# chayanchatterjee/GW-Whisper

Measured on AMD Instinct MI355X. Metric: 1s-strain segments/sec (encoder fwd), higher is better.
Workload: dtype bf16; 1 GPU; whisper-tiny encoder fwd, batch 256 log-mel (80x3000) per GPU, 1500 tokens, random-init weights (BASELINE configs[1]); global_batch=256, parallelism=dp1, encoder=tiny, streams_per_gpu=1

## Files before the change

### gw_whisper_amd/_lib.py

```python

from __future__ import annotations

import ctypes as C
import os

_HERE = os.path.dirname(os.path.abspath(__file__))
LIB_PATH = os.environ.get("GWW_LIB") or os.path.join(_HERE, "libgww.so")

PREC_BF16 = 0
PREC_F32 = 1

EPI_BIAS, EPI_GELU, EPI_RESID = 0, 1, 2
EPI_DGELU = 5


class EncCfg(C.Structure):
    _fields_ = [("d_model", C.c_int), ("n_layers", C.c_int), ("n_heads", C.c_int),
                ("ffn", C.c_int), ("n_mels", C.c_int), ("t_in", C.c_int)]


class EncGlobals(C.Structure):
    _fields_ = [(n, C.c_void_p) for n in
                ("conv1_w", "conv1_b", "conv2_w", "conv2_b", "pos", "ln_w", "ln_b")]

# ... 2 lines not shown
    _fields_ = [(n, C.c_void_p) for n in
                ("ln1_w", "ln1_b", "q_w", "q_b", "k_w", "v_w", "v_b", "o_w", "o_b",
                 "ln2_w", "ln2_b", "fc1_w", "fc1_b", "fc2_w", "fc2_b")]


class DoraTarget(C.Structure):
    _fields_ = [("layer", C.c_int), ("proj", C.c_int), ("r", C.c_int), ("scaling", C.c_float),
                ("A", C.c_void_p), ("B", C.c_void_p), ("mag", C.c_void_p), ("nrm", C.c_void_p),
                ("dA", C.c_void_p), ("dB", C.c_void_p), ("dm", C.c_void_p)]


class EncLayerGrads(C.Structure):
    _fields_ = [(f[0], C.c_void_p) for f in EncLayer._fields_]


class EncGrads(C.Structure):
    _fields_ = [(n, C.c_void_p) for n in
                ("conv1_w", "conv1_b", "conv2_w", "conv2_b", "pos", "ln_w", "ln_b")] + \
               [("layers", C.POINTER(EncLayerGrads))]


class DoraMergeItem(C.Structure):
    _fields_ = [("w0", C.c_void_p), ("a", C.c_void_p), ("b", C.c_void_p), ("m", C.c_void_p), ("w_eff", C.c_void_p),
                ("norm_out", C.c_void_p), ("scaling", C.c_float), ("d_out", C.c_int), ("d_in", C.c_int), ("r", C.c_int)]


SIGNATURES = {
    "gww_version": (C.c_int, []),
    "gww_last_error": (C.c_char_p, []),
    "gww_frontend_create": (C.c_int, [C.POINTER(C.c_void_p)]),
    "gww_frontend_create_nmel": (C.c_int, [C.c_int, C.POINTER(C.c_void_p)]),
    "gww_frontend_destroy": (None, [C.c_void_p]),
    "gww_logmel_f32": (C.c_int, [C.c_void_p, C.c_void_p, C.c_int, C.c_int, C.c_long, C.c_void_p,
                                 C.c_void_p, C.c_void_p]),
    "gww_logmel_host_f32": (C.c_int, [C.c_void_p, C.c_int, C.c_int, C.c_long, C.c_void_p]),
    "gww_logmel_host_nmel_f32": (C.c_int, [C.c_void_p, C.c_int, C.c_int, C.c_long, C.c_int, C.c_void_p]),
    "gww_encoder_create": (C.c_int, [C.POINTER(EncCfg), C.POINTER(C.c_void_p)]),
    "gww_encoder_destroy": (None, [C.c_void_p]),
    "gww_encoder_set_weights": (C.c_int, [C.c_void_p, C.POINTER(EncGlobals), C.POINTER(EncLayer),
                                          C.c_int, C.c_void_p]),
    "gww_encoder_update_weights": (C.c_int, [C.c_void_p, C.POINTER(EncGlobals), C.POINTER(EncLayer), C.c_int,
                                             C.POINTER(C.c_uint), C.c_void_p]),
    "gww_encoder_workspace_bytes": (C.c_size_t, [C.c_void_p, C.c_int, C.c_int]),
    "gww_encoder_forward": (C.c_int, [C.c_void_p, C.c_void_p, C.c_int, C.c_int, C.c_void_p, C.c_size_t,
                                      C.c_void_p, C.c_void_p, C.c_void_p]),
    "gww_encoder_forward_outputs": (C.c_int, [C.c_void_p, C.c_void_p, C.c_int, C.c_int, C.c_void_p, C.c_size_t,
                                              C.c_void_p, C.c_void_p, C.c_void_p, C.c_void_p]),
    "gww_encoder_set_split": (C.c_int, [C.c_void_p, C.c_int]),
    "gww_encoder_set_stem_shortcut": (C.c_int, [C.c_void_p, C.c_int]),
    "gww_encoder_stem_shortcut_flags": (C.c_int, [C.c_void_p, C.c_int, C.c_int, C.c_void_p, C.POINTER(C.c_int)]),
    "gww_encoder_set_x_native": (C.c_int, [C.c_void_p, C.c_int]),
    "gww_x_native_offset": (C.c_size_t, [C.c_long, C.c_int, C.c_long]),
    "gww_x_native_bytes": (C.c_size_t, [C.c_long]),
    "gww_encoder_trace_enable": (C.c_int, [C.c_void_p, C.c_int]),
    "gww_encoder_trace_read": (C.c_int, [C.c_void_p, C.POINTER(C.c_float), C.POINTER(C.c_int)]),
    "gww_encoder_trace_classes": (C.c_int, []),
    "gww_encoder_trace_class_name": (C.c_char_p, [C.c_int]),
    "gww_train_saved_bytes": (C.c_size_t, [C.c_void_p, C.c_int]),
    "gww_train_workspace_bytes": (C.c_size_t, [C.c_void_p, C.c_int]),
    "gww_encoder_train_forward": (C.c_int, [C.c_void_p, C.c_void_p, C.c_int, C.c_void_p, C.c_size_t, C.c_void_p,
                                            C.c_size_t, C.c_void_p, C.c_int, C.c_void_p]),
    "gww_encoder_train_backward": (C.c_int, [C.c_void_p, C.c_int, C.c_void_p, C.c_size_t, C.c_void_p, C.c_size_t,
                                             C.c_void_p, C.POINTER(DoraTarget), C.c_int, C.c_void_p, C.c_void_p,
                                             C.c_int, C.c_void_p]),
    "gww_train_workspace_bytes_full": (C.c_size_t, [C.c_void_p, C.c_int]),
    "gww_train_workspace_bytes_adapters": (C.c_size_t, [C.c_void_p, C.c_int, C.c_int]),
    "gww_encoder_train_backward_full": (C.c_int, [C.c_void_p, C.c_int, C.c_void_p, C.c_size_t, C.c_void_p, C.c_size_t,
                                                  C.c_void_p, C.POINTER(DoraTarget), C.c_int, C.c_void_p, C.c_void_p,
                                                  C.c_int, C.POINTER(EncGrads), C.c_void_p]),
    "gww_train_saved_bytes_f32": (C.c_size_t, [C.c_void_p, C.c_int]),
    "gww_train_workspace_bytes_f32": (C.c_size_t, [C.c_void_p, C.c_int]),
    "gww_encoder_train_forward_f32": (C.c_int, [C.c_void_p, C.c_void_p, C.c_int, C.c_void_p, C.c_size_t, C.c_void_p,
                                                C.c_size_t, C.c_void_p, C.c_int, C.c_void_p]),
    "gww_encoder_train_backward_f32": (C.c_int, [C.c_void_p, C.c_int, C.c_void_p, C.c_size_t, C.c_void_p, C.c_size_t,
                                                 C.c_void_p, C.POINTER(DoraTarget), C.c_int, C.c_void_p, C.c_void_p,
                                                 C.c_int, C.c_void_p]),
    "gww_attention_lse_f32": (C.c_int, [C.c_void_p, C.c_void_p, C.c_void_p, C.c_int, C.c_int, C.c_int, C.c_void_p]),
    "gww_attention_bwd_f32_scratch_bytes": (C.c_size_t, [C.c_int, C.c_int, C.c_int]),
    "gww_attention_bwd_f32": (C.c_int, [C.c_void_p, C.c_void_p, C.c_void_p, C.c_void_p, C.c_void_p, C.c_void_p,
                                        C.c_int, C.c_int, C.c_int, C.c_void_p]),
    "gww_adapter_grads_f32_scratch_bytes": (C.c_size_t, [C.c_long, C.c_int, C.c_int, C.c_int]),
    "gww_adapter_grads_f32": (C.c_int, [C.c_void_p, C.c_long, C.c_void_p, C.c_void_p, C.c_long, C.c_void_p, C.c_float,
                                        C.c_float, C.c_void_p, C.c_void_p, C.c_void_p, C.c_void_p, C.c_void_p,
                                        C.c_void_p, C.c_void_p, C.c_long, C.c_int, C.c_int, C.c_int, C.c_void_p,
                                        C.c_size_t, C.c_void_p]),
    "gww_gemm_wgrad_workspace_bytes": (C.c_size_t, [C.c_long, C.c_int, C.c_int]),
    "gww_gemm_wgrad_bf16": (C.c_int, [C.c_void_p, C.c_long, C.c_void_p, C.c_long, C.c_long, C.c_int, C.c_int, C.c_float,
                                      C.c_void_p, C.c_void_p, C.c_void_p, C.c_size_t, C.c_void_p]),
    "gww_layernorm_param_grads_workspace_bytes": (C.c_size_t, [C.c_long, C.c_int]),
    "gww_layernorm_param_grads": (C.c_int, [C.c_void_p, C.c_void_p, C.c_int, C.c_long, C.c_int, C.c_void_p, C.c_void_p,
                                            C.c_void_p, C.c_size_t, C.c_void_p]),
    "gww_attention_bwd_bf16": (C.c_int, [C.c_void_p, C.c_void_p, C.c_void_p, C.c_void_p, C.c_void_p, C.c_void_p,
                                         C.c_int, C.c_int, C.c_int, C.c_void_p]),
    "gww_attention_bwd_log2q_bf16": (C.c_int, [C.c_void_p, C.c_void_p, C.c_void_p, C.c_void_p, C.c_void_p, C.c_void_p,
                                         C.c_int, C.c_int, C.c_int, C.c_void_p]),
    "gww_attention_log2q_bf16": (C.c_int, [C.c_void_p, C.c_void_p, C.c_void_p, C.c_int, C.c_int, C.c_int, C.c_void_p]),
    "gww_attention_lse_bf16": (C.c_int, [C.c_void_p, C.c_void_p, C.c_void_p, C.c_int, C.c_int, C.c_int, C.c_void_p]),
    "gww_layernorm_bwd": (C.c_int, [C.c_void_p, C.c_void_p, C.c_void_p, C.c_int, C.c_void_p, C.c_int, C.c_void_p,
                                    C.c_long, C.c_int, C.c_void_p]),
    "gww_gelu_bf16": (C.c_int, [C.c_void_p, C.c_void_p, C.c_void_p, C.c_long, C.c_void_p]),
    "gww_dora_grads": (C.c_int, [C.c_void_p, C.c_long, C.c_void_p, C.c_void_p, C.c_long, C.c_void_p, C.c_float,
                                 C.c_float, C.c_void_p, C.c_void_p, C.c_void_p, C.c_void_p, C.c_void_p, C.c_void_p,
                                 C.c_void_p, C.c_long, C.c_int, C.c_int, C.c_void_p]),
    "gww_adapter_grads_scratch_bytes": (C.c_size_t, [C.c_long, C.c_int, C.c_int, C.c_int]),
    "gww_adapter_grads": (C.c_int, [C.c_void_p, C.c_long, C.c_void_p, C.c_void_p, C.c_long, C.c_void_p, C.c_float,
                                    C.c_float, C.c_void_p, C.c_void_p, C.c_void_p, C.c_void_p, C.c_void_p, C.c_void_p,
# ... 179 lines not shown
```

### gw_whisper_amd/csrc/attention.hip

```cpp
#include "common.h"

#include <stdlib.h>
#include <type_traits>

#ifndef GWW_ATT_EPI16
#define GWW_ATT_EPI16 1
#endif
namespace gww {

#ifdef GWW_STAMP
__device__ unsigned long long g_stamp_att[8];
#define ASTAMP_DECL unsigned long long _t0 = __builtin_amdgcn_s_memtime(); unsigned long long _acc[7] = {0, 0, 0, 0, 0, 0, 0};
#define ASTAMP(i)                                                  \
  do {                                                             \
    __builtin_amdgcn_sched_barrier(0);                             \
    const unsigned long long _t1 = __builtin_amdgcn_s_memtime();   \
    _acc[i] += _t1 - _t0;                                          \
    _t0 = _t1;                                                     \
    __builtin_amdgcn_sched_barrier(0);                             \
  } while (0)
#define ASTAMP_FLUSH                                                                 \
  if (lane == 0) {                                                                   \
    for (int _q = 0; _q < 7; ++_q) atomicAdd(&g_stamp_att[_q], _acc[_q]);            \
    atomicAdd(&g_stamp_att[7], 1ull);                                                \
// ... 388 lines not shown
    __syncthreads();
  };
  using P0 = std::integral_constant<int, 0>;
  using P1 = std::integral_constant<int, 1>;
  using Yes = std::true_type;
  using No = std::false_type;

  gload(0);
  lstore(P0{});
  __syncthreads();
  const bool ragged = (T % KB) != 0;
  if (n_kt == 1) {
    if (ragged) tile(0, P0{}, Yes{}, Yes{});
    else tile(0, P0{}, Yes{}, No{});
  } else {
    tile(0, P0{}, Yes{}, No{});
    int kt = 1;
    for (; kt + 2 <= n_kt - 1; kt += 2) {
      tile(kt, P1{}, No{}, No{});
      tile(kt + 1, P0{}, No{}, No{});
    }
    if (kt == n_kt - 2) {
      tile(kt, P1{}, No{}, No{});
      if (ragged) tile(kt + 1, P0{}, No{}, Yes{});
      else tile(kt + 1, P0{}, No{}, No{});
    } else {
      if (ragged) tile(kt, P1{}, No{}, Yes{});
      else tile(kt, P1{}, No{}, No{});
    }
  }

  const float l_tot = (VAR & 2) ? l_run + __shfl_xor(l_run, 32, 64) : lt[0];
  const float inv = 1.0f / l_tot;
  if (lse && q_row < T && hh == 0)
    lse[((long)b * H + h) * T + q_row] = (m_run + __log2f(l_tot)) * 0.69314718055994530942f;
  if (q_row < T) {
    unsigned short* orow = ctx + ((long)b * T + q_row) * d + h * DH;
#pragma unroll
    for (int n = 0; n < 2; ++n)
#pragma unroll
      for (int c = 0; c < 4; ++c) {
        const int dh = 32 * n + 8 * c + 4 * hh;
        u32x2 o = {pack2bf(ot[n][4 * c] * inv, ot[n][4 * c + 1] * inv),
                   pack2bf(ot[n][4 * c + 2] * inv, ot[n][4 * c + 3] * inv)};
        *reinterpret_cast<u32x2*>(orow + dh) = o;
      }
  }
}

#endif
#ifndef GWW_ATT_NBUF
#define GWW_ATT_NBUF 2
#endif
template <int MINW, bool MSUM, bool NOMAX>
__global__ __launch_bounds__(256, MINW) void k_attention_dma_bf16(const unsigned short* __restrict__ qkv,
                                                                 unsigned short* __restrict__ ctx,
                                                                 float* __restrict__ lse, int T, int H, int q_tiles,
                                                                 int qt0) {
  constexpr int NB = GWW_ATT_NBUF;
  __shared__ __attribute__((aligned(16))) unsigned char lds[NB * 2 * KB * DH * 2];
  constexpr int TILE_BYTES = KB * DH * 2, NW = 4;
  typedef __attribute__((address_space(3))) void* lds_ptr;
  typedef const __attribute__((address_space(1))) void* g_ptr;
  const int tid = threadIdx.x, lane = tid & 63, wave = tid >> 6;
  const int wave_u = __builtin_amdgcn_readfirstlane(wave);
  const unsigned nblk = gridDim.x, per = nblk >> 3;
  const unsigned wid = blockIdx.x < 8 * per ? (blockIdx.x & 7) * per + (blockIdx.x >> 3) : blockIdx.x;
  const int qt = qt0 + wid % q_tiles;
  const int bh = wid / q_tiles;
  const int b = bh / H, h = bh - b * H;
  const int d = H * DH;
  const long row_stride = 3L * d;
  const unsigned short* base = qkv + (long)b * T * row_stride;
  const unsigned short* qp = base + h * DH;
  const unsigned short* kp = base + d + h * DH;
  const unsigned short* vp = base + 2 * d + h * DH;
  const int r = lane & 31, hh = lane >> 5;
  const int q_row = qt * (NW * 32) + wave * 32 + r;
  const int q_ld = q_row < T ? q_row : T - 1;
  const bool wave_live = qt * (NW * 32) + wave_u * 32 < T;
  bf16x8 qf[4];
#pragma unroll
  for (int s = 0; s < 4; ++s) qf[s] = *reinterpret_cast<const bf16x8*>(qp + (long)q_ld * row_stride + 16 * s + 8 * hh);

  const int n_kt = (T + KB - 1) / KB;
  const bool ragged = (T % KB) != 0;
  unsigned koff[2], voff[2];
#pragma unroll
  for (int j = 0; j < 2; ++j) {
    const int row = 8 * (2 * wave + j) + (lane >> 3), pos = lane & 7;
    koff[j] = (unsigned)(row * (int)row_stride * 2 + ((pos ^ ((row >> 1) & 7)) << 4));
    voff[j] = (unsigned)(row * (int)row_stride * 2 + ((pos ^ (((row >> 1) & 1) << 2)) << 4));
  }
  auto dma = [&](int kt, auto buf_c) {
    constexpr int BUF = decltype(buf_c)::value;
    const char* kb = reinterpret_cast<const char*>(kp + (long)kt * KB * row_stride);
    const char* vb = reinterpret_cast<const char*>(vp + (long)kt * KB * row_stride);
    unsigned char* dk = lds + BUF * TILE_BYTES + (2 * wave_u) * 1024;
    unsigned char* dv = dk + NB * TILE_BYTES;
    if constexpr (NB == 3) {
      const unsigned mk = (unsigned)(unsigned long long)(lds_ptr)dk, mv = (unsigned)(unsigned long long)(lds_ptr)dv;
      unsigned ko[2], vo[2];
      if (kt != n_kt - 1 || !ragged) {
        ko[0] = koff[0]; ko[1] = koff[1]; vo[0] = voff[0]; vo[1] = voff[1];
      } else {
        const int last_row = T - 1 - kt * KB;
#pragma unroll
// ... 176 lines not shown
    using P2 = std::integral_constant<int, 2>;
    dma(0, P0{});
    if (n_kt > 1) {
      dma(1, P1{});
      asm volatile("s_waitcnt vmcnt(4)\n\ts_barrier" ::: "memory");
    } else {
      asm volatile("s_waitcnt vmcnt(0)\n\ts_barrier" ::: "memory");
    }
#pragma unroll
    for (int s4 = 0; s4 < 4; ++s4) asm volatile("" : "+v"(qf[s4]));
    tile(0, P0{}, Yes{}, No{}, n_kt == 1 && ragged);
    for (int kt = 1; kt < n_kt; kt += 3) {
      tile(kt, P1{}, No{}, No{}, ragged && kt == n_kt - 1);
      if (kt + 1 < n_kt) tile(kt + 1, P2{}, No{}, No{}, ragged && kt + 1 == n_kt - 1);
      if (kt + 2 < n_kt) tile(kt + 2, P0{}, No{}, No{}, ragged && kt + 2 == n_kt - 1);
    }
  } else {
    dma(0, P0{});
    __syncthreads();
    if (n_kt == 1) {
      if (ragged) tile(0, P0{}, Yes{}, Yes{});
      else tile(0, P0{}, Yes{}, No{});
    } else {
      tile(0, P0{}, Yes{}, No{});
      int kt = 1;
      for (; kt + 2 <= n_kt - 1; kt += 2) {
        tile(kt, P1{}, No{}, No{});
        tile(kt + 1, P0{}, No{}, No{});
      }
      if (kt == n_kt - 2) {
        tile(kt, P1{}, No{}, No{});
        if (ragged) tile(kt + 1, P0{}, No{}, Yes{});
        else tile(kt + 1, P0{}, No{}, No{});
      } else {
        if (ragged) tile(kt, P1{}, No{}, Yes{});
        else tile(kt, P1{}, No{}, No{});
      }
    }
  }

  float l_tot;
  if constexpr (MSUM) {
    l_tot = lt[0];
  } else {
    const auto sw = __builtin_amdgcn_permlane32_swap(__float_as_uint(l_run), __float_as_uint(l_run), false, false);
    l_tot = __uint_as_float(sw[0]) + __uint_as_float(sw[1]);
  }
  const float inv = 1.0f / l_tot;
  if (lse && q_row < T && hh == 0)
    lse[((long)b * H + h) * T + q_row] = (m_run + __log2f(l_tot)) * 0.69314718055994530942f;
#if GWW_ATT_EPI16
  {
    unsigned short* orow = ctx + ((long)b * T + q_row) * d + h * DH;
#pragma unroll
    for (int n = 0; n < 2; ++n)
#pragma unroll
      for (int cp = 0; cp < 2; ++cp) {
        const int c0 = 2 * cp, c1 = 2 * cp + 1;
        const unsigned a0 = pack2bf(ot[n][4 * c0] * inv, ot[n][4 * c0 + 1] * inv), a1 = pack2bf(ot[n][4 * c0 + 2] * inv, ot[n][4 * c0 + 3] * inv);
        const unsigned b0 = pack2bf(ot[n][4 * c1] * inv, ot[n][4 * c1 + 1] * inv), b1 = pack2bf(ot[n][4 * c1 + 2] * inv, ot[n][4 * c1 + 3] * inv);
        const auto s0 = __builtin_amdgcn_permlane32_swap(a0, b0, false, false);
        const auto s1 = __builtin_amdgcn_permlane32_swap(a1, b1, false, false);
        u32x4 o = {s0[0], s1[0], s0[1], s1[1]};
        if (q_row < T) *reinterpret_cast<u32x4*>(orow + 32 * n + 8 * (hh ? c1 : c0)) = o;
      }
  }
#else
  if (q_row < T) {
    unsigned short* orow = ctx + ((long)b * T + q_row) * d + h * DH;
#pragma unroll
    for (int n = 0; n < 2; ++n)
#pragma unroll
      for (int c = 0; c < 4; ++c) {
        const int dh = 32 * n + 8 * c + 4 * hh;
        u32x2 o = {pack2bf(ot[n][4 * c] * inv, ot[n][4 * c + 1] * inv),
                   pack2bf(ot[n][4 * c + 2] * inv, ot[n][4 * c + 3] * inv)};
        *reinterpret_cast<u32x2*>(orow + dh) = o;
      }
  }
#endif
}

#ifdef GWW_LAB
constexpr int PP_SLOTS = 4;
#ifndef GWW_PP_PRIO
#define GWW_PP_PRIO 0
#endif
template <int MODE>
__global__ __launch_bounds__(MODE == 1 ? 256 : 512, 1) void k_attention_pp_bf16(const unsigned short* __restrict__ qkv,
                                                              unsigned short* __restrict__ ctx,
                                                              float* __restrict__ lse, int T, int H, int q_tiles,
                                                              int qt0) {
  constexpr int TILE_BYTES = KB * DH * 2;
  __shared__ __attribute__((aligned(16))) unsigned char lds[2 * PP_SLOTS * TILE_BYTES];
  typedef __attribute__((address_space(3))) void* lds_ptr;
  typedef const __attribute__((address_space(1))) void* g_ptr;
  const int tid = threadIdx.x, lane = tid & 63;
  const int wave = __builtin_amdgcn_readfirstlane(tid >> 6);
  const bool g1 = wave >= 4;
  constexpr int NWV = MODE == 1 ? 4 : 8, PPW = 8 / NWV;
  const unsigned nblk = gridDim.x, per = nblk >> 3;
  const unsigned wid = blockIdx.x < 8 * per ? (blockIdx.x & 7) * per + (blockIdx.x >> 3) : blockIdx.x;
  const int qt = qt0 + wid % q_tiles;
  const int bh = wid / q_tiles;
  const int b = bh / H, h = bh - b * H;
  const int d = H * DH;
  const long row_stride = 3L * d;
  const unsigned short* base = qkv + (long)b * T * row_stride;
  const unsigned short* qp = base + h * DH;
  const unsigned short* kp = base + d + h * DH;
  const unsigned short* vp = base + 2 * d + h * DH;
  const int r = lane & 31, hh = lane >> 5;
  const int q_row = qt * (NWV * 32) + wave * 32 + r;
  const int q_ld = q_row < T ? q_row : T - 1;
  bf16x8 qf[4];
#pragma unroll
  for (int s = 0; s < 4; ++s) qf[s] = *reinterpret_cast<const bf16x8*>(qp + (long)q_ld * row_stride + 16 * s + 8 * hh);

  const int n_kt = (T + KB - 1) / KB;
  const bool ragged = (T % KB) != 0;
// ... 481 lines not shown
  if (g1) __builtin_amdgcn_s_barrier();
  if (GWW_PP_PRIO == 2 && g1) __builtin_amdgcn_s_setprio(1);
  if (n_kt == 1 && ragged) tile(0, std::integral_constant<int, 0>{}, Yes{}, Yes{});
  else tile(0, std::integral_constant<int, 0>{}, Yes{}, No{});
  {
    int kt = 1;
    for (; kt + 4 <= n_kt - 1; kt += 4) {
      tile(kt, std::integral_constant<int, 1>{}, No{}, No{});
      tile(kt + 1, std::integral_constant<int, 2>{}, No{}, No{});
      tile(kt + 2, std::integral_constant<int, 3>{}, No{}, No{});
      tile(kt + 3, std::integral_constant<int, 0>{}, No{}, No{});
    }
    for (; kt < n_kt; ++kt) tile_rt(kt, ragged && kt == n_kt - 1);
  }
  pv_reads((n_kt - 1) & 3);
  pv_mfma();
  if (!g1) __builtin_amdgcn_s_barrier();
  ASTAMP(6);
  ASTAMP_FLUSH
  }

  float l_tot;
  {
    const auto sw = __builtin_amdgcn_permlane32_swap(__float_as_uint(l_run), __float_as_uint(l_run), false, false);
    l_tot = __uint_as_float(sw[0]) + __uint_as_float(sw[1]);
  }
  const float inv = 1.0f / l_tot;
  if (lse && q_row < T && hh == 0)
    lse[((long)b * H + h) * T + q_row] = (m_run + __log2f(l_tot)) * 0.69314718055994530942f;
  {
    unsigned short* orow = ctx + ((long)b * T + q_row) * d + h * DH;
#pragma unroll
    for (int n = 0; n < 2; ++n)
#pragma unroll
      for (int cp = 0; cp < 2; ++cp) {
        const int c0 = 2 * cp, c1 = 2 * cp + 1;
        const unsigned a0 = pack2bf(ot[n][4 * c0] * inv, ot[n][4 * c0 + 1] * inv), a1 = pack2bf(ot[n][4 * c0 + 2] * inv, ot[n][4 * c0 + 3] * inv);
        const unsigned b0 = pack2bf(ot[n][4 * c1] * inv, ot[n][4 * c1 + 1] * inv), b1 = pack2bf(ot[n][4 * c1 + 2] * inv, ot[n][4 * c1 + 3] * inv);
        const auto s0 = __builtin_amdgcn_permlane32_swap(a0, b0, false, false);
        const auto s1 = __builtin_amdgcn_permlane32_swap(a1, b1, false, false);
        u32x4 o = {s0[0], s1[0], s0[1], s1[1]};
        if (q_row < T) *reinterpret_cast<u32x4*>(orow + 32 * n + 8 * (hh ? c1 : c0)) = o;
      }
  }
}

#endif
bool attention_log2q_enabled() {
  static const bool off = lab_int("GWW_ATT_LOG2Q", 1) == 0;
  return !off;
}

int launch_attention_bf16(const void* qkv, void* ctx, int B, int T, int H, hipStream_t s, float* lse,
                          bool last_tile_only, bool q_log2) {
  GWW_REQUIRE(qkv && ctx, "attention_bf16: NULL operand");
  GWW_REQUIRE(B >= 0 && T > 0 && H > 0, "attention_bf16: bad shape B=%d T=%d H=%d", B, T, H);
  GWW_REQUIRE((((uintptr_t)qkv) & 15) == 0 && (((uintptr_t)ctx) & 15) == 0, "attention_bf16: 16-byte alignment");
  if (B == 0) return GWW_OK;
#ifdef GWW_LAB
  if (q_log2 && !last_tile_only && lab_int("GWW_ATT_W64", 0) != 0) return launch_attention_w64_bf16(qkv, ctx, B, T, H, s, lse);
#endif
  const unsigned short* in = (const unsigned short*)qkv;
  unsigned short* out = (unsigned short*)ctx;
#ifdef GWW_LAB
  const int nw_env = (int)lab_int("GWW_ATT_WAVES", 0);
  const int var_env = (int)lab_int("GWW_ATT_VAR", 7);
  const bool pp = q_log2 && var_env >= 8;
  const int nw = ((nw_env == 8 && !q_log2) || (pp && var_env == 8)) ? 8 : 4;
#else
  const int nw = 4;
#endif
  const int all_tiles = (T + nw * 32 - 1) / (nw * 32);
  const int q_tiles = last_tile_only ? 1 : all_tiles, qt0 = last_tile_only ? all_tiles - 1 : 0;
  const long blocks = (long)q_tiles * B * H;
  GWW_REQUIRE(blocks < 2147483647L, "attention_bf16: grid too large");
#define GWW_DMA(MW, MS, NM) hipLaunchKernelGGL((k_attention_dma_bf16<MW, MS, NM>), dim3((unsigned)blocks), dim3(256), 0, s, in, out, lse, T, H, q_tiles, qt0)
#ifdef GWW_LAB
  if (pp && var_env >= 9) {
    hipLaunchKernelGGL((k_attention_pp_bf16<1>), dim3((unsigned)blocks), dim3(256), 0, s, in, out, lse, T, H, q_tiles, qt0);
  } else if (pp) {
    hipLaunchKernelGGL((k_attention_pp_bf16<0>), dim3((unsigned)blocks), dim3(512), 0, s, in, out, lse, T, H, q_tiles, qt0);
  } else if (q_log2) {
    const int var = var_env & 7;
#define GWW_L2(VV) hipLaunchKernelGGL((k_attention_l2_bf16<4, VV>), dim3((unsigned)blocks), dim3(256), 0, s, in, out, lse, T, H, q_tiles, qt0)
    switch (var) {
      case 0: GWW_L2(0); break;
      case 1: GWW_L2(1); break;
      case 2: GWW_L2(2); break;
      case 3: GWW_L2(3); break;
      case 4: GWW_DMA(3, false, false); break;
      case 5: GWW_DMA(4, false, false); break;
      case 6: GWW_DMA(3, true, false); break;
      default: GWW_DMA(3, false, true); break;
    }
#undef GWW_L2
  } else if (nw == 8) {
    hipLaunchKernelGGL(k_attention_bf16<8>, dim3((unsigned)blocks), dim3(512), 0, s, in, out, lse, T, H, q_tiles, qt0);
  } else
#else
  if (q_log2) {
    GWW_DMA(3, false, true);
  } else
#endif
  {
    hipLaunchKernelGGL(k_attention_bf16<4>, dim3((unsigned)blocks), dim3(256), 0, s, in, out, lse, T, H, q_tiles, qt0);
  }
#undef GWW_DMA
  GWW_LAUNCH_CHECK();
  return GWW_OK;
}

constexpr int FKB = 32;
constexpr int FLDS = DH + 1;

__global__ __launch_bounds__(256) void k_attention_f32(const float* __restrict__ qkv, float* __restrict__ ctx,
                                                       int T, int H, int q_tiles) {
  __shared__ float Ks[FKB][FLDS];
  __shared__ float Vs[FKB][FLDS];
  const int tid = threadIdx.x, lane = tid & 63, wave = tid >> 6;
  const int qt = blockIdx.x % q_tiles;
  const int bh = blockIdx.x / q_tiles;
  const int b = bh / H, h = bh - b * H;
  const int d = H * DH;
  const long row_stride = 3L * d;
  const float* base = qkv + (long)b * T * row_stride;
  const float* qp = base + h * DH;
  const float* kp = base + d + h * DH;
  const float* vp = base + 2 * d + h * DH;
// ... 183 lines not shown
  GWW_REQUIRE(qkv && ctx && lse, "attention_lse_f32: NULL operand");
  GWW_REQUIRE(B >= 0 && T > 0 && H > 0, "attention_lse_f32: bad shape B=%d T=%d H=%d", B, T, H);
  GWW_REQUIRE((((uintptr_t)qkv) & 15) == 0 && (((uintptr_t)ctx) & 15) == 0, "attention_lse_f32: 16-byte alignment");
  if (B == 0) return GWW_OK;
  const int q_tiles = (T + QB - 1) / QB;
  const int qt0 = last_tile_only ? q_tiles - 1 : 0;
  const long blocks = (long)(q_tiles - qt0) * B * H;
  GWW_REQUIRE(blocks < 2147483647L, "attention_lse_f32: grid too large");
  hipLaunchKernelGGL(k_attention_lse_f32, dim3((unsigned)blocks), dim3(256), 0, s, qkv, ctx, lse, T, H, q_tiles - qt0, qt0);
  GWW_LAUNCH_CHECK();
  return GWW_OK;
}

int launch_attention_f32(const float* qkv, float* ctx, int B, int T, int H, hipStream_t s) {
  GWW_REQUIRE(qkv && ctx, "attention_f32: NULL operand");
  GWW_REQUIRE(B >= 0 && T > 0 && H > 0, "attention_f32: bad shape B=%d T=%d H=%d", B, T, H);
  GWW_REQUIRE((((uintptr_t)qkv) & 15) == 0 && (((uintptr_t)ctx) & 15) == 0, "attention_f32: 16-byte alignment");
  if (B == 0) return GWW_OK;
  const int q_tiles = (T + QB - 1) / QB;
  const long blocks = (long)q_tiles * B * H;
  GWW_REQUIRE(blocks < 2147483647L, "attention_f32: grid too large");
  hipLaunchKernelGGL(k_attention_f32, dim3((unsigned)blocks), dim3(256), 0, s, qkv, ctx, T, H, q_tiles);
  GWW_LAUNCH_CHECK();
  return GWW_OK;
}

}

using namespace gww;

#ifdef GWW_STAMP
extern "C" int gww_debug_stamps_att(unsigned long long* out8, int reset) {
  GWW_HIP(hipMemcpyFromSymbol(out8, HIP_SYMBOL(gww::g_stamp_att), sizeof(unsigned long long) * 8));
  if (reset) {
    unsigned long long z[8] = {0};
    GWW_HIP(hipMemcpyToSymbol(HIP_SYMBOL(gww::g_stamp_att), z, sizeof(z)));
  }
  return GWW_OK;
}
#endif

extern "C" int gww_attention_bf16(const void* qkv, void* ctx, int B, int T, int n_heads, void* stream) {
  return launch_attention_bf16(qkv, ctx, B, T, n_heads, (hipStream_t)stream);
}
extern "C" int gww_attention_lse_bf16(const void* qkv, void* ctx, float* lse, int B, int T, int n_heads, void* stream) {
  GWW_REQUIRE(lse != nullptr, "gww_attention_lse_bf16: lse is NULL");
  return launch_attention_bf16(qkv, ctx, B, T, n_heads, (hipStream_t)stream, lse);
}

extern "C" int gww_attention_log2q_bf16(const void* qkv, void* ctx, float* lse_or_null, int B, int T, int n_heads,
                                        void* stream) {
  return launch_attention_bf16(qkv, ctx, B, T, n_heads, (hipStream_t)stream, lse_or_null, false, true);
}
extern "C" int gww_attention_f32(const float* qkv, float* ctx, int B, int T, int n_heads, void* stream) {
  return launch_attention_f32(qkv, ctx, B, T, n_heads, (hipStream_t)stream);
}
extern "C" int gww_attention_lse_f32(const float* qkv, float* ctx, float* lse, int B, int T, int n_heads, void* stream) {
  return launch_attention_lse_f32(qkv, ctx, lse, B, T, n_heads, false, (hipStream_t)stream);
}
```

### gw_whisper_amd/csrc/common.h

```cpp
#pragma once

#include <hip/hip_runtime.h>
#include <stdarg.h>
#include <stdint.h>
#include <stdio.h>
#include <string.h>

#include "../../include/gww.h"
#include <vector>

namespace gww {

extern thread_local char g_err[512];
int fail(int code, const char* fmt, ...);

#define GWW_HIP(expr)                                                                 \
  do {                                                                                \
    hipError_t _e = (expr);                                                           \
    if (_e != hipSuccess)                                                             \
      return ::gww::fail(GWW_ERR_HIP, "%s failed: %s (%s:%d)", #expr, hipGetErrorString(_e), \
                         __FILE__, __LINE__);                                         \
  } while (0)

#define GWW_LAUNCH_CHECK() GWW_HIP(hipGetLastError())
// ... 70 lines not shown

__device__ __forceinline__ float gelu_fast(float x) {
  const float z = fabsf(x) * 0.70710678118654752440f;
  const float t = __builtin_amdgcn_rcpf(fmaf(0.3275911f, z, 1.0f));
  float p = fmaf(1.061405429f, t, -1.453152027f);
  p = fmaf(p, t, 1.421413741f);
  p = fmaf(p, t, -0.284496736f);
  p = fmaf(p, t, 0.254829592f);
  p *= t;
  const float e = __builtin_amdgcn_exp2f(-z * z * 1.44269504088896340736f);
  const float erf_abs = fmaf(-p, e, 1.0f);
  const float h = 0.5f * x;
  return fmaf(h, copysignf(erf_abs, x), h);
}

__device__ __forceinline__ float gelu_sig4(float x) {
  const float s = fminf(x * x, 64.0f);
  float q = fmaf(s, 0.0010148164f, -0.1067791331f);
  q = fmaf(s, q, -2.3011178f);
  const float e = __builtin_amdgcn_exp2f(x * q);
  return x * __builtin_amdgcn_rcpf(1.0f + e);
}
__device__ __forceinline__ float gelu_sig4_sigma(float x) {
  const float s = fminf(x * x, 64.0f);
  float q = fmaf(s, 0.0010148164f, -0.1067791331f);
  q = fmaf(s, q, -2.3011178f);
  const float e = __builtin_amdgcn_exp2f(x * q);
  return __builtin_amdgcn_rcpf(1.0f + e);
}

__device__ __forceinline__ float dgelu_fast(float z) {
  const float az = fabsf(z) * 0.70710678118654752440f;
  const float t = __builtin_amdgcn_rcpf(fmaf(0.3275911f, az, 1.0f));
  float p = fmaf(1.061405429f, t, -1.453152027f);
  p = fmaf(p, t, 1.421413741f);
  p = fmaf(p, t, -0.284496736f);
  p = fmaf(p, t, 0.254829592f);
  p *= t;
  const float e = __builtin_amdgcn_exp2f(-az * az * 1.44269504088896340736f);
  const float erf_abs = fmaf(-p, e, 1.0f);
  return fmaf(0.5f, copysignf(erf_abs, z), fmaf(z * 0.3989422804f, e, 0.5f));
}

static inline long cdiv(long a, long b) { return (a + b - 1) / b; }
static inline bool aligned(const void* p, uintptr_t a) { return (((uintptr_t)p) & (a - 1)) == 0; }

__host__ __device__ inline size_t x_native_offset(long g, int c, long M) {
  if (g > M - 1) g = M - 1;
  const size_t slice = (size_t)(g >> 5);
  const int r = (int)(g & 31), t = c >> 5, cc = (c >> 3) & 3, hh = (c >> 2) & 1, k = c & 3;
  return (slice * 48 + (size_t)(4 * t + cc)) * 1024 + (size_t)(r + 32 * hh) * 16 + (size_t)(4 * k);
}
inline size_t x_native_bytes(long M) { return (size_t)cdiv(M, 128) * 128 * 384 * 4; }

struct Arena {
  size_t off = 0;
  size_t take(size_t bytes) { const size_t o = off; off += (bytes + 255) / 256 * 256; return o; }
  size_t total() const { return off; }
};

#ifdef GWW_LAB
long lab_int(const char* name, long dflt);
#else
constexpr long lab_int(const char*, long dflt) { return dflt; }
#endif

constexpr int kStemTc = 256, kStemTt = kStemTc / 2;

enum { PREP_PACK16, PREP_PACK32, PREP_COPY, PREP_LNFOLD, PREP_TRANSPOSE, PREP_DORA };
constexpr int kPrepMaxOps = 40;
constexpr int kPrepMaxRank = 1024;
struct PrepOp {
  const void *a, *b, *c, *d;
  void *o0, *o1, *o2;
  int kind, blocks, N, K;
  int C, taps;
  float scale;
  int pad_;
};
struct PrepArgs {
  int n;
  int first[kPrepMaxOps + 1];
  PrepOp op[kPrepMaxOps];
};
struct PrepBatch {
  std::vector<PrepArgs> args;
  hipStream_t s;
  explicit PrepBatch(hipStream_t st) : s(st) {}
  int add(const PrepOp& o);
  int flush();
  int pack(const float* w, void* out, int out_bf16, int N, int C, int taps, int Kpad, float scale);
  int copy(const float* in, float* out, int n, float scale);
  int ln_fold(const float* w, const float* g, const float* bl, const float* bias, float scale, int N, int K, void* wp,
              float* u, float* cb);
  int transpose(const void* in, void* out, int R, int Cn);
  int dora(const float* w0, const float* a, const float* b, const float* m, float scaling, int d_out, int d_in, int r,
           float* w_eff, float* norm_out);
};

enum : int {
  EPI_BIAS = 0,
  EPI_GELU = 1,
  EPI_RESID = 2,
  EPI_CONV2 = 3,
};

// ... 4 lines not shown
```

### gw_whisper_amd/csrc/encoder.hip

```cpp
#include "encoder_impl.h"

namespace gww {
#ifdef GWW_LAB
long lab_int(const char* name, long dflt) {
  const char* e = getenv(name);
  return e ? atol(e) : dflt;
}
#endif
}

using namespace gww;

static size_t carve_blob(gww_encoder* e, char* blob) {
  const size_t d = e->cfg.d_model, F = e->cfg.ffn, T = e->cfg.t_in / 2, Kc1 = conv1_kpad(e->cfg.n_mels);
  const uintptr_t base = (uintptr_t)blob;
  Arena a;
  auto put = [&](auto*& p, size_t bytes) { p = (decltype(+p))(base + a.take(bytes)); };
  put(e->c1w, d * Kc1 * 2);
  put(e->c2w, (d + 255) / 256 * 256 * 3 * d * 2);
  put(e->c1w32, d * Kc1 * 4);
  put(e->c2w32, d * 3 * d * 4);
  put(e->c1wT, d * Kc1 * 2);
  put(e->c2wT, d * 3 * d * 2);
  put(e->c1b, d * 4);
// ... 228 lines not shown
};
WsLayout ws_layout(const gww_enc_cfg& c, int B, int precision) {
  const size_t es = precision == GWW_PREC_BF16 ? 2 : 4;
  const size_t d = c.d_model, F = c.ffn, Tin = c.t_in, T = c.t_in / 2, C = c.n_mels, Kc1 = conv1_kpad(c.n_mels);
  WsLayout w{};
  Arena a;
  const size_t Mp = padded_rows((size_t)B * T);
  w.melT = a.take(((size_t)B * (Tin + 2) * C + Kc1) * es);
  w.c1 = a.take((((size_t)B * (Tin + 2) + 255) / 256 * 256 + 520) * d * es);
  w.x = a.take(Mp * d * 4);
  w.x2 = a.take(Mp * d * 4);
  w.h = a.take(Mp * d * es);
  w.d2 = a.take(Mp * d * es);
  w.qkv = a.take(Mp * 3 * d * es);
  w.ctx = a.take(Mp * d * es);
  w.f1 = a.take(Mp * F * es);
  w.total = a.total();
  return w;
}

struct StemTailLayout {
  size_t c1s, xs, tr, dump, total;
};
StemTailLayout stem_tail_layout(int B, int d) {
  StemTailLayout t{};
  Arena a;
  t.c1s = a.take((((size_t)B * (kStemTc + 2) + 255) / 256 * 256 + 520) * d * 2);
  t.xs = a.take((size_t)B * kStemTt * d * 4);
  t.tr = a.take((size_t)B * d * 4);
  t.dump = a.take((size_t)d * 4);
  t.total = a.total();
  return t;
}

enum Conv1Kind { CONV1_DIRECT, CONV1_ASTAT, CONV1_GENERIC };
enum Conv2Kind { CONV2_V4, CONV2_FULLN, CONV2_GENERIC };
struct FwdWants {
  bool last_hidden, last_token, hidden_slab, attn_slab;
};
struct FwdPlan {
  Conv1Kind conv1;
  Conv2Kind conv2;
  bool shortcut;
  bool x0_layer0;
  bool astat;
  bool mlp_fused;
  bool fuse_qkv;
  bool lnqkv0;
  bool op;
  bool fuse_final;
  bool pooled;
  bool q_log2;
  bool x_native;
};
FwdPlan plan_forward(const gww_encoder* e, int batch, int precision, FwdWants want) {
  const gww_enc_cfg& c = e->cfg;
  const int m = generic_path_mask(), d = c.d_model, F = c.ffn, T = c.t_in / 2;
  const bool bf = precision == GWW_PREC_BF16;
  FwdPlan p{};
  p.conv1 = !bf || (m & GP_CONV1) ? CONV1_GENERIC
            : conv1_mel_supported(c.n_mels, d, conv1_kpad(c.n_mels)) ? CONV1_DIRECT : d % 128 == 0 ? CONV1_ASTAT : CONV1_GENERIC;
  p.conv2 = bf && d % 128 == 0 && d <= 3072 && !(m & GP_CONV2) ? CONV2_V4
            : bf && (d == 384 || d == 512) && !(m & GP_CONV2_FULLN) ? CONV2_FULLN : CONV2_GENERIC;
  const auto x2_bytes = [&] { const WsLayout w = ws_layout(c, batch, precision); return w.h - w.x2; };
  p.shortcut = p.conv1 == CONV1_DIRECT && p.conv2 == CONV2_V4 && e->stem_shortcut && batch > 0 && !(m & GP_STEM_SHORTCUT) &&
               stem_tail_supported(c.t_in, d) && stem_tail_layout(batch, d).total <= x2_bytes();
  p.astat = bf && (d == 384 || (d == 512 && (m & GP_ASTAT_512))) && F % 128 == 0 && !(m & GP_LAYER_GEMMS);
  p.mlp_fused = p.astat && mlp_fused_supported(d, F) && !(m & GP_MLP);
  p.fuse_qkv = p.mlp_fused && !(m & GP_QKV);
  p.lnqkv0 = p.fuse_qkv && !(m & GP_LNQKV0);
  p.op = p.fuse_qkv && !(m & GP_OUT_PROJ);
  p.fuse_final = p.op && want.last_hidden && !(m & GP_FINAL_LN);
  p.pooled = bf && !want.last_hidden && want.last_token && T >= 3 && !(m & GP_POOLED) && !want.hidden_slab && !want.attn_slab;
  p.x0_layer0 = p.shortcut && p.lnqkv0 && p.op && !want.hidden_slab && c.n_layers > 1;
  p.q_log2 = attention_log2q_enabled();
  p.x_native = e->x_native && p.op && p.fuse_final && !p.pooled && !want.hidden_slab && c.n_layers > 1 && d == 384 &&
               mlp_fused_x_native_supported() && !(m & GP_X_NATIVE) &&
               x_native_bytes((long)batch * T) <= padded_rows((size_t)batch * T) * d * 4;
  return p;
}
}

constexpr int kSplitMin = 32;

static bool use_split(const gww_encoder* e, int batch) { return e->split && batch >= 2 * kSplitMin; }

extern "C" size_t gww_encoder_workspace_bytes(const gww_encoder* e, int batch, int precision) {
  if (!e || batch <= 0) return 0;
  if (use_split(e, batch)) {
    const int b0 = batch / 2;
    return ws_layout(e->cfg, b0, precision).total + ws_layout(e->cfg, batch - b0, precision).total;
  }
  return ws_layout(e->cfg, batch, precision).total;
}

extern "C" int gww_encoder_set_stem_shortcut(gww_encoder* e, int on) {
  GWW_REQUIRE(e != nullptr, "gww_encoder_set_stem_shortcut: NULL handle");
  e->stem_shortcut = on != 0;
  return GWW_OK;
}

extern "C" int gww_encoder_set_x_native(gww_encoder* e, int on) {
  GWW_REQUIRE(e != nullptr, "gww_encoder_set_x_native: NULL handle");
  e->x_native = on != 0;
  return GWW_OK;
}

extern "C" size_t gww_x_native_offset(long row, int col, long M) {
  if (row < 0 || col < 0 || col >= 384 || M <= 0) return (size_t)-1;
  return x_native_offset(row, col, M);
}
extern "C" size_t gww_x_native_bytes(long M) { return M > 0 ? x_native_bytes(M) : 0; }

extern "C" int gww_encoder_stem_shortcut_flags(const gww_encoder* e, int batch, int precision, const void* workspace,
                                               int* flags) {
  GWW_REQUIRE(e && workspace && flags, "gww_encoder_stem_shortcut_flags: NULL argument");
  GWW_REQUIRE(batch > 0 && (precision == GWW_PREC_BF16 || precision == GWW_PREC_F32),
              "gww_encoder_stem_shortcut_flags: bad batch %d / precision %d", batch, precision);
  flags[0] = flags[1] = -1;
  const bool split = use_split(e, batch);
  const int b[2] = {split ? batch / 2 : batch, split ? batch - batch / 2 : 0};
  size_t off = 0;
  for (int i = 0; i < 2 && b[i] > 0; ++i) {
    const WsLayout w = ws_layout(e->cfg, b[i], precision);
    if (plan_forward(e, b[i], precision, FwdWants{}).shortcut)
      GWW_HIP(hipMemcpy(&flags[i], (const char*)workspace + off + w.melT, sizeof(int), hipMemcpyDeviceToHost));
    off += w.total;
  }
  return GWW_OK;
}

extern "C" int gww_encoder_set_split(gww_encoder* e, int on) {
  GWW_REQUIRE(e != nullptr, "gww_encoder_set_split: NULL handle");
  if (on && !e->s2[0]) {
    for (int i = 0; i < 2; ++i) {
      GWW_HIP(hipStreamCreateWithFlags(&e->s2[i], hipStreamNonBlocking));
      GWW_HIP(hipEventCreateWithFlags(&e->ev_join[i], hipEventDisableTiming));
    }
    GWW_HIP(hipEventCreateWithFlags(&e->ev_fork, hipEventDisableTiming));
    GWW_HIP(hipEventCreateWithFlags(&e->ev_skew, hipEventDisableTiming));
  }
  e->split = on ? 1 : 0;
  return GWW_OK;
}

struct Tracer {
  gww_encoder* e;
  hipStream_t s;
  int begin(int cls) {
    if (!e->trace) return GWW_OK;
    TraceSpan sp{cls, nullptr, nullptr};
    for (hipEvent_t* ev : {&sp.a, &sp.b}) {
      if (!e->pool.empty()) { *ev = e->pool.back(); e->pool.pop_back(); }
      else GWW_HIP(hipEventCreate(ev));
    }
    GWW_HIP(hipEventRecord(sp.a, s));
    e->spans.push_back(sp);
    return GWW_OK;
  }
  int end() {
    if (!e->trace) return GWW_OK;
    GWW_HIP(hipEventRecord(e->spans.back().b, s));
    return GWW_OK;
  }
};
// ... 101 lines not shown
                           hipMemcpyDeviceToDevice, s));
  TR(TR_OUT, launch_gemm_bf16((const unsigned short*)ctx + (size_t)(T - 1) * d, (long)T * d, L.wo, L.bo, xl, nullptr,
                              xm, B, d, d, EPI_RESID, 0, s, 0));
  TR(TR_LNROWS, launch_layernorm(xm, L.ln2w, L.ln2b, hb, 1, B, d, s));
  TR(TR_FC1, launch_gemm_bf16(hb, d, L.w1, L.b1, nullptr, nullptr, f1, B, F, d, EPI_GELU, 0, s, 0));
  TR(TR_FC2, launch_gemm_bf16(f1, F, L.w2, L.b2, xm, nullptr, xf, B, d, F, EPI_RESID, 0, s, 0));
  TR(TR_LNROWS, launch_layernorm_rows(xf, d, e->lnw, e->lnb, last_token, B, d, s, nullptr));
  return GWW_OK;
}

int Fwd::final_layernorm(const float* xc, const void* pending) {
  if (last_hidden) TR(TR_LN, launch_layernorm(xc, e->lnw, e->lnb, last_hidden, 0, M, d, s, pending));
  if (last_token)
    TR(TR_LNROWS, launch_layernorm_rows(xc + (long)(T - 1) * d, (long)T * d, e->lnw, e->lnb, last_token, B, d, s,
                                        pending ? (const char*)pending + (size_t)(T - 1) * d * 2 : nullptr));
  if (last_hidden) GWW_TRY(tap_final());
  return GWW_OK;
}

struct AstatState {
  float* xc;
  float* xn;
  const void* pending;
  bool qkv_ready;
  void swap() { std::swap(xc, xn); }
};

int Fwd::walk_astat() {
  AstatState st{x, x2, nullptr, false};
  void* const d1 = h;
  auto args = [&]() { MlpFusedArgs a; a.who = "gww_encoder_forward"; a.M = M; a.d = d; return a; };
  auto with_qkv = [&](MlpFusedArgs& a, const LayerW& W) { a.qkv_u = W.uqkv; a.qkv_cb = W.cbqkv; a.qkv_out = qkv; a.NQ = 3 * d; };
  for (int i = 0; i < n_layers; ++i) {
    const LayerW& L = e->layers[i];
    const bool last = i == n_layers - 1, from_x0 = i == 0 && p.x0_layer0;
    if (!st.qkv_ready) {
      if (i == 0 && p.lnqkv0) {
        MlpFusedArgs a = args();
        a.x = st.xc; a.Wt = L.wqkv_st;
        with_qkv(a, L);
        if (from_x0) a.x0 = &x0;
        TR(TR_QKV, launch_mlp_fused(a, s));
      } else {
        TR(TR_QKV, launch_gemm_astat(st.xc, d, st.pending, st.pending ? st.xn : nullptr, L.uqkv, L.cbqkv, L.wqkv_ln, nullptr, qkv,
                                     M, 3 * d, d, EPI_BIAS, 0, s));
        if (st.pending) st.swap();
        st.pending = nullptr;
      }
    }
    st.qkv_ready = false;
    GWW_TRY(tap_hidden(i, st.xc));
    if (i == 0 && skew_event) GWW_HIP(hipEventRecord(skew_event, s));
    if (p.pooled && last) return pooled_last_layer(L, st.xc, st.xn, d1);
    TR(TR_ATTN, launch_attention_bf16(qkv, ctx, B, T, H, s, nullptr, false, p.q_log2));
    GWW_TRY(tap_attn(i));
    if (!p.op)
      TR(TR_OUT, launch_gemm_astat(ctx, d, nullptr, nullptr, nullptr, nullptr, L.wo, L.bo, d1, M, d, d, EPI_BIAS, 0, s));
    MlpFusedArgs a = args();
    a.x = st.xc; a.x_new = from_x0 ? nullptr : st.xn; a.ln_u = L.u1; a.ln_cb = L.cb1; a.b2 = L.b2; a.F = F;
    a.x_native_in = p.x_native && i > (p.x0_layer0 ? 1 : 0);
    if (p.op) { a.ctx = ctx; a.bo = L.bo; a.Wt = L.wmlp_op; }
    else { a.delta = d1; a.Wt = L.wmlp; }
    if (p.fuse_qkv && !last) {
      with_qkv(a, e->layers[i + 1]);
      if (from_x0) a.x0 = &x0;
      a.x_native_out = p.x_native && !from_x0;
      TR(TR_MLPQKV, launch_mlp_fused(a, s));
      st.qkv_ready = true;
    } else if (p.fuse_final) {
      a.lnf_w = e->lnw; a.lnf_b = e->lnb; a.y = last_hidden; a.last_token = last_token; a.T = T;
      TR(TR_MLPFIN, launch_mlp_fused(a, s));
      return tap_final();
    } else if (p.mlp_fused) {
      a.C = d2; a.keep_x_new = true;
      TR(TR_MLP, launch_mlp_fused(a, s));
      st.swap();
      st.pending = d2;
    } else {
      TR(TR_FC1, launch_gemm_astat(st.xc, d, d1, st.xn, L.u1, L.cb1, L.w1_ln, nullptr, f1, M, F, d, EPI_GELU, 0, s));
      st.swap();
      TR(TR_FC2, launch_gemm_fulln(f1, F, L.w2, L.b2, nullptr, d2, M, d, F, EPI_BIAS, 0, s));
      st.pending = d2;
    }
  }
  return final_layernorm(st.xc, st.pending);
}

int Fwd::walk_generic() {
  for (int i = 0; i < n_layers; ++i) {
    const LayerW& L = e->layers[i];
    GWW_TRY(tap_hidden(i, x));
    TR(TR_LN, launch_layernorm(x, L.ln1w, L.ln1b, h, bf ? 1 : 0, M, d, s));
    TR(TR_QKV, gemm(h, d, L.wqkv, L.wqkv32, bf ? L.bqkv16 : L.bqkv, nullptr, nullptr, qkv, M, 3 * d, d, EPI_BIAS, 0));
    if (p.pooled && i == n_layers - 1) return pooled_last_layer(L, x, x2, h);
    if (bf) TR(TR_ATTN, launch_attention_bf16(qkv, ctx, B, T, H, s, nullptr, false, p.q_log2));
    else TR(TR_ATTN, launch_attention_f32((const float*)qkv, (float*)ctx, B, T, H, s));
    GWW_TRY(tap_attn(i));
    TR(TR_OUT, gemm(ctx, d, L.wo, L.wo32, L.bo, x, nullptr, x, M, d, d, EPI_RESID, 0));
    TR(TR_LN, launch_layernorm(x, L.ln2w, L.ln2b, h, bf ? 1 : 0, M, d, s));
    TR(TR_FC1, gemm(h, d, L.w1, L.w132, L.b1, nullptr, nullptr, f1, M, F, d, EPI_GELU, 0));
    TR(TR_FC2, gemm(f1, F, L.w2, L.w232, L.b2, x, nullptr, x, M, d, F, EPI_RESID, 0));
  }
  return final_layernorm(x, nullptr);
}
#undef TR

static int forward_impl(gww_encoder* e, const float* mel, int batch, int precision, void* workspace,
                        size_t workspace_bytes, float* last_hidden, float* last_token, void* stream,
                        hipEvent_t skew_event = nullptr, float* hidden_slab = nullptr, float* attn_slab = nullptr,
                        size_t hs_stride = 0, size_t as_stride = 0) {
  GWW_REQUIRE(e && mel, "gww_encoder_forward: NULL argument");
  if (!e->ready) return fail(GWW_ERR_STATE, "gww_encoder_forward: weights not set");
  GWW_REQUIRE(precision == GWW_PREC_BF16 || precision == GWW_PREC_F32, "gww_encoder_forward: bad precision %d",
              precision);
// ... 88 lines not shown
```

### gw_whisper_amd/csrc/encoder_impl.h

```cpp
#pragma once

#include "common.h"
#include "epilogue.h"

#include <stdlib.h>
#include <algorithm>
#include <vector>

namespace gww {

struct LayerW {
  unsigned short *wqkv, *wo, *w1, *w2;
  float *wqkv32, *wo32, *w132, *w232;
  float *bqkv, *bo, *b1, *b2, *ln1w, *ln1b, *ln2w, *ln2b;
  float* bqkv16;
  unsigned short *wqkv_ln, *w1_ln;
  unsigned short* wmlp;
  unsigned short* wqkv_st;
  unsigned short* wmlp_op;
  float *uqkv, *cbqkv, *u1, *cb1;
  unsigned short *wqkvT, *woT, *w1T, *w2T;
};

constexpr int conv1_kpad(int n_mels) { return (3 * n_mels + 63) / 64 * 64; }

inline size_t align_up(size_t x, size_t a = 256) { return (x + a - 1) / a * a; }

inline size_t padded_rows(size_t M) { return (M + 255) / 256 * 256 + 512; }

struct SavedArena {
  size_t layer_stride, x_in, total;
  int n_layers;
  float* x_in_at(void* saved, int l) const {
    return (float*)((char*)saved + (l < n_layers ? (size_t)l * layer_stride + x_in : (size_t)n_layers * layer_stride));
  }
  const float* x_in_at(const void* saved, int l) const { return x_in_at(const_cast<void*>(saved), l); }
};

enum : int {
  GP_LAYER_GEMMS = 1,
  GP_CONV1 = 2,
  GP_CONV2 = 4,
  GP_MLP = 8,
  GP_QKV = 16,
  GP_POOLED = 32,
  GP_LNQKV0 = 64,
  GP_OUT_PROJ = 128,
  GP_FINAL_LN = 256,
  GP_ASTAT_512 = 512,
  GP_CONV2_FULLN = 1024,
  GP_STEM_SHORTCUT = 2048,
  GP_X_NATIVE = 4096,
};
inline int generic_path_mask() {
  static const int mask = (int)lab_int("GWW_GENERIC_PATH", 0);
  return mask;
}

inline int check_targets(const char* who, const gww_dora_target* t, int n) {
  for (int i = 0; i < n; ++i) {
    GWW_REQUIRE(t[i].r >= 1 && t[i].r <= 64, "%s: target %d has rank %d: adapter gradients support ranks 1..64", who, i, t[i].r);
    GWW_REQUIRE(t[i].A && t[i].B && t[i].mag && t[i].nrm && t[i].dA && t[i].dB && t[i].dm, "%s: NULL pointer in target %d", who, i);
  }
  for (int i = 1; i < n; ++i)
    for (int j = 0; j < i; ++j)
      GWW_REQUIRE(t[i].layer != t[j].layer || t[i].proj != t[j].proj, "%s: duplicate target: %d and %d both name layer %d proj %d",
                  who, j, i, t[i].layer, t[i].proj);
  return GWW_OK;
}
inline int check_target_range(const char* who, const gww_dora_target* t, int n, int L) {
  for (int i = 0; i < n; ++i)
    GWW_REQUIRE(t[i].layer >= 0 && t[i].layer < L && t[i].proj >= 0 && t[i].proj <= 5, "%s: bad target %d", who, i);
  return GWW_OK;
}
struct TargetTable {
  std::vector<const gww_dora_target*> slot;
  TargetTable() = default;
  TargetTable(const gww_dora_target* t, int n, int L) : slot(n > 0 ? (size_t)L * 6 : 0, nullptr) {
    for (int i = 0; i < n; ++i) slot[(size_t)t[i].layer * 6 + t[i].proj] = &t[i];
  }
  const gww_dora_target* at(int layer, int proj) const { return slot.empty() ? nullptr : slot[(size_t)layer * 6 + proj]; }
};

}

enum : int { TR_MEL = 0, TR_CONV1, TR_CONV2, TR_QKV, TR_ATTN, TR_OUT, TR_FC1, TR_FC2, TR_LN, TR_MLP, TR_MLPQKV, TR_LNROWS, TR_MLPFIN, TR_COUNT };

struct TraceSpan { int cls; hipEvent_t a, b; };

struct gww_encoder {
  gww_enc_cfg cfg{};
  bool ready = false;
  bool trace = false;
  bool stem_shortcut = true;
  bool x_native = true;
  std::vector<TraceSpan> spans;
  std::vector<hipEvent_t> pool;
  int split = 0;
  hipStream_t s2[2] = {nullptr, nullptr};
  hipEvent_t ev_fork = nullptr, ev_skew = nullptr, ev_join[2] = {nullptr, nullptr};
  char* blob = nullptr;
  size_t blob_bytes = 0;
  unsigned short *c1w = nullptr, *c2w = nullptr;
  unsigned short *c1wT = nullptr, *c2wT = nullptr;
  float *c1w32 = nullptr, *c2w32 = nullptr;
  float *c1b = nullptr, *c2b = nullptr, *pos = nullptr, *lnw = nullptr, *lnb = nullptr;
  float* pos_c = nullptr;
  std::vector<gww::LayerW> layers;
};
```

### gw_whisper_amd/csrc/launchers.h

```cpp
#pragma once

namespace gww {

int launch_layernorm(const float* x, const float* w, const float* b, void* y, int out_bf16,
                     long M, int d, hipStream_t s, const void* delta_bf16 = nullptr);
int launch_layernorm_rows(const float* x, long row_stride, const float* w, const float* b, float* y,
                          long M, int d, hipStream_t s, const void* delta_bf16 = nullptr);
int launch_pack_weight(const float* w, void* out, int out_bf16, int N, int C, int taps, int Kpad,
                       float scale, hipStream_t s);

bool conv1_mel_supported(int n_mels, int d, int kpad);
int launch_conv1_mel(const float* mel, const void* W, const float* bias, void* c1, int B, int T, int d, hipStream_t s,
                     int t_stride = 0, const int* run_flag = nullptr, int run_if = 0);
bool stem_tail_supported(int t_in, int d);
int launch_stem_detect(const float* mel, int* flag, long rows, int t_in, hipStream_t s);
int launch_stem_fill(const float* xs, const float* tr, const float* pos, float* x, const int* flag, int B, int T, int d,
                     hipStream_t s, int Tt = kStemTt);
int launch_mel_to_tokens(const float* mel, void* out, int out_bf16, int B, int C, int T, hipStream_t s);

int launch_gemm_astat(const void* A, long lda, const void* delta, float* x_out, const float* ln_u,
                      const float* ln_cb, const void* W, const float* bias, void* C, long M, int N, int K,
                      int epi, int rows_per_batch, hipStream_t s, long c_panel_rows = 0);
int launch_gemm_bf16(const void* A, long lda, const void* W, const float* bias, const float* resid,
                     const float* pos, void* C, long M, int N, int K, int epi, int rows_per_batch,
                     hipStream_t s, int rows_padded_256 = 0);
int launch_gemm_bf16_v4(const void* A, long lda, const void* W, const float* bias, const float* resid, void* C, long M,
                        int N, int K, int epi, hipStream_t s, int force_split = 0, const float* pos = nullptr,
                        int rows_per_batch = 0, int n_real = 0, float* dump = nullptr, const int* run_flag = nullptr,
                        int run_if = 0, float* tmpl_r = nullptr, int tmpl_t = 0);
int launch_gemm_fulln(const void* A, long lda, const void* W, const float* bias, const float* pos, void* C,
                      long M, int N, int K, int epi, int rows_per_batch, hipStream_t s);
int launch_gemm_f32(const float* A, long lda, const float* W, const float* bias, const float* resid,
                    const float* pos, float* C, long M, int N, int K, int epi, int rows_per_batch,
                    hipStream_t s);

int launch_attention_bf16(const void* qkv, void* ctx, int B, int T, int H, hipStream_t s, float* lse = nullptr,
                          bool last_tile_only = false, bool q_log2 = false);
int launch_attention_w64_bf16(const void* qkv, void* ctx, int B, int T, int H, hipStream_t s, float* lse);
bool attention_log2q_enabled();
int launch_attention_f32(const float* qkv, float* ctx, int B, int T, int H, hipStream_t s);
int launch_attention_probs(const void* qkv, bool bf16, bool q_log2, float* probs, int B, int T, int H, hipStream_t s);
int launch_attention_bwd_bf16(const void* qkv, const void* ctx, const void* dctx, const float* lse, float* D,
                              void* dqkv, int B, int T, int H, hipStream_t s, bool q_log2);

int launch_mlp_pack(const void* w1_folded, const void* w2, const void* wqkv_folded, void* out, int d, int F, int NQ,
                    hipStream_t s, const void* wo = nullptr);
bool mlp_fused_supported(int d, int F);
bool mlp_fused_x_native_supported();
struct MfX0 {
  const float *xs, *tr, *pos;
  const int* flag;
  int T, Tt;
};
struct MlpFusedArgs {
  const char* who = "mlp_fused";
  const float* x = nullptr;
  const void* delta = nullptr;
  const void* ctx = nullptr;
  const float* bo = nullptr;
  float* x_new = nullptr;
  bool keep_x_new = false;
  const float *ln_u = nullptr, *ln_cb = nullptr;
  const void* Wt = nullptr;
  const float* b2 = nullptr;
  void* C = nullptr;
  const float *qkv_u = nullptr, *qkv_cb = nullptr;
  void* qkv_out = nullptr;
  int NQ = 0;
  float* x_next = nullptr;
  const float *lnf_w = nullptr, *lnf_b = nullptr;
  float* y = nullptr;
  float* last_token = nullptr;
  int T = 0;
  bool x_native_in = false;
  bool x_native_out = false;
  const MfX0* x0 = nullptr;
  long M = 0;
  int d = 0, F = 0;
};
int launch_mlp_fused(const MlpFusedArgs& a, hipStream_t s);

int launch_ln_bwd(const float* x, const float* gamma, const void* dy, int dy_f32, float* dx, int accumulate,
                  void* dx_bf16, long M, int d, hipStream_t s);
int launch_gelu_bf16(const void* z, const void* df, void* out, long n, hipStream_t s);
int launch_sub_f32_bf16(const float* a, const float* b, void* out, long n, hipStream_t s);
int launch_add_delta_f32(const float* x, const void* delta_bf16, float* out, long n, hipStream_t s);
int launch_stem_dz2(const void* dxb, const void* z2, void* out, int B, int T, int d, hipStream_t s);
int launch_stem_dz1(const void* col, const void* z1, void* out, int B, int T, int Tin, int d, hipStream_t s);
int launch_stem_dmel(const void* col1, float* dmel, int B, int Tin, int C, int Kp, hipStream_t s);
int launch_ln_param_grads(const float* x, const void* dy, int dy_f32, long M, int d, float* dgamma, float* dbeta,
                          void* workspace, size_t ws_bytes, hipStream_t s);
size_t ln_param_grads_workspace_bytes(long M, int d);
int launch_pos_grad(const float* dx0, float* dpos, int B, int T, int d, hipStream_t s);
int launch_dora_grads(const void* X, long ldx, const void* dY, const void* Y, long ldy, const float* bias_st,
                      float yscale, float scaling, const float* A, const float* Bm, const float* mag,
                      const float* nrm, float* dA, float* dB, float* dm, long M, int d, int r, hipStream_t s,
                      void* scratch = nullptr, size_t scratch_bytes = 0);
int launch_dora_grads_multi(const void* X, long ldx, const void* dY, const void* Y, long ldy, int np,
                            const long* col_off, const float* const* bias_st, const float* yscale,
                            const float* scaling, const float* const* A, const float* const* Bm,
                            const float* const* mag, const float* const* nrm, float* const* dA, float* const* dB,
                            float* const* dm, long M, int d, hipStream_t s, void* scratch, size_t scratch_bytes);
size_t dora_grads_scratch_bytes(int np, int d);
int launch_adapter_grads(const void* X, long ldx, const void* dY, const void* Y, long ldy, const float* bias_st,
                         float yscale, float scaling, const float* A, const float* Bm, const float* mag,
                         const float* nrm, float* dA, float* dB, float* dm, long M, int d_in, int d_out, int r,
                         hipStream_t s, void* scratch, size_t scratch_bytes);
size_t adapter_grads_scratch_bytes(long M, int d_in, int d_out, int r);
int launch_wgrad(const void* dY, long ldy, const void* X, long ldx, long M, int N, int K, float alpha, float* dW,
                 float* db, int conv_cin, void* workspace, size_t ws_bytes, hipStream_t s);
size_t wgrad_workspace_bytes(long M, int N, int K);

int launch_attention_lse_f32(const float* qkv, float* ctx, float* lse, int B, int T, int H, bool last_tile_only,
                             hipStream_t s);
int launch_attention_bwd_f32(const float* qkv, const float* ctx, const float* dctx, const float* lse, float* scratch,
                             float* dqkv, int B, int T, int H, hipStream_t s);
size_t attention_bwd_f32_scratch_words(int B, int T, int H);
int launch_gemm_f32_dx(const float* A, long lda, const float* W, float* C, long ldc, long M, int N, int K, hipStream_t s);
int launch_adapter_grads_f32(const float* X, long ldx, const float* dY, const float* Y, long ldy, const float* bias,
                             float yscale, float scaling, const float* A, const float* Bm, const float* mag,
                             const float* nrm, float* dA, float* dB, float* dm, long M, int d_in, int d_out, int r,
                             hipStream_t s, void* scratch, size_t scratch_bytes);
size_t adapter_grads_f32_scratch_bytes(long M, int d_in, int d_out, int r);
int launch_gelu_f32(const float* z, const float* g, float* out, long n, hipStream_t s);
int launch_sub_f32(const float* a, const float* b, float* out, long n, hipStream_t s);
int launch_stem_dz2_f32(const float* dx0, const float* z2, float* out, int B, int T, int d, hipStream_t s);
int launch_stem_dz1_f32(const float* col, const float* z1, float* out, int B, int T, int Tin, int d, hipStream_t s);
int launch_stem_dmel_f32(const float* col1, float* dmel, int B, int Tin, int C, int Kp, hipStream_t s);
// ... 3 lines not shown
```

### gw_whisper_amd/csrc/mlp_fused.hip

```cpp
#include "common.h"

#include <stdlib.h>

#include <type_traits>

namespace gww {

namespace {
constexpr int MF_D = 384;
constexpr int MF_KT = MF_D / 64;
constexpr int MF_OT = MF_D / 32;
constexpr int MF_WAVES = 4, MF_THREADS = 256, MF_BM = 128;
#ifndef GWW_MF_EXP
#define GWW_MF_EXP 0
#endif
#ifndef GWW_MF_ABL
#define GWW_MF_ABL 0
#endif
#ifndef GWW_MF_OLDDMA
#define GWW_MF_OLDDMA 0
#endif
#ifndef GWW_MF_AHEAD
#define GWW_MF_AHEAD 3
#endif
#ifndef GWW_MF_SCHED
#define GWW_MF_SCHED 1
#endif
#ifndef GWW_MF_VACC
#define GWW_MF_VACC 1
#endif
#ifndef GWW_MF_NTSTORE
#define GWW_MF_NTSTORE 1
#endif
#ifndef GWW_MF_NTLOAD
#define GWW_MF_NTLOAD 1
#endif
#if GWW_MF_NTLOAD
#define MF_NT " nt"
#else
#define MF_NT ""
#endif
#ifndef GWW_MF_PADNOP
#define GWW_MF_PADNOP 0
#endif
#if GWW_MF_PADNOP
#define MF_PADNOP "s_nop 1\n\t"
#else
#define MF_PADNOP ""
#endif
#ifndef GWW_MF_XLDS
#define GWW_MF_XLDS 0
#endif
#ifndef GWW_MF_XSTNT
#define GWW_MF_XSTNT 0
#endif
#ifndef GWW_MF_XNT
#define GWW_MF_XNT 0
#endif
#if GWW_MF_XNT
#define MF_XNT MF_NT
#else
#define MF_XNT ""
#endif
#ifndef GWW_MF_XN_LDNT
#define GWW_MF_XN_LDNT 1
#endif
#ifndef GWW_MF_XN_STNT
#define GWW_MF_XN_STNT 1
#endif
#if GWW_MF_XN_LDNT
#define MF_XN_LDNT " nt"
#else
#define MF_XN_LDNT ""
#endif
#if GWW_MF_XN_STNT
#define MF_XN_STNT " nt"
#else
#define MF_XN_STNT ""
#endif
#ifndef GWW_MF_DMAGAP
#define GWW_MF_DMAGAP 1
#endif
#ifndef GWW_MF_TAIL2
#define GWW_MF_TAIL2 0
#endif
#ifndef GWW_MF_NORM
#define GWW_MF_NORM 1
#endif
#ifndef GWW_MF_XACC
#define GWW_MF_XACC 1
#endif
#ifndef GWW_MF_CSPREAD
#define GWW_MF_CSPREAD 1
#endif
constexpr int MF_AHEAD = GWW_MF_AHEAD;
constexpr int MF_NST_MAX = MF_AHEAD + 1;
constexpr int MF_TILE = 128 * 64 * 2;
constexpr int MF_GL = 16 / MF_WAVES;
constexpr int MF_FMAX = 1536;
constexpr int MF_SLICE_STRIDE = 144, MF_SLICE_BYTES = 32 * MF_SLICE_STRIDE;
constexpr int MF_OFF_CB = MF_NST_MAX * MF_TILE;
constexpr int MF_OFF_U = MF_OFF_CB + MF_FMAX * 4;
constexpr int MF_OFF_B2 = MF_OFF_U + MF_FMAX * 4;
constexpr int MF_OFF_BO = MF_OFF_B2 + MF_D * 4;
constexpr int MF_OFF_QCB = MF_OFF_BO + MF_D * 4;
constexpr int MF_OFF_SLICE = MF_OFF_QCB + MF_FMAX * 4;
constexpr int MF_LDS = MF_OFF_SLICE + 2 * MF_WAVES * MF_SLICE_BYTES;
static_assert(MF_LDS <= 160 * 1024, "LDS budget");

template <int N>
using MF_FL = std::integral_constant<int, N>;

__device__ __forceinline__ float mf_sum8(float v) {
  v += __builtin_bit_cast(float, __builtin_amdgcn_update_dpp(0, __builtin_bit_cast(int, v), 0xB1, 0xF, 0xF, true));
  v += __builtin_bit_cast(float, __builtin_amdgcn_update_dpp(0, __builtin_bit_cast(int, v), 0x4E, 0xF, 0xF, true));
  v += __builtin_bit_cast(float, __builtin_amdgcn_update_dpp(0, __builtin_bit_cast(int, v), 0x141, 0xF, 0xF, true));
  return v;
}

template <int N>
__device__ __forceinline__ void mf_wait_vmcnt() {
// ... 19 lines not shown
  const unsigned long long _tb = _t0, _rb = __builtin_amdgcn_s_memrealtime();
#define MSTAMP(i)                                                  \
  do {                                                             \
    if (GWW_STAMP >= 2 && (i) != 0 && (i) != 3 && (i) != 4 && (i) != 5 && !((i) >= 100)) break; \
    __builtin_amdgcn_sched_barrier(0);                             \
    const unsigned long long _t1 = __builtin_amdgcn_s_memtime();   \
    _acc[(i) >= 100 ? (i) - 100 : (i)] += _t1 - _t0;               \
    _t0 = _t1;                                                     \
    __builtin_amdgcn_sched_barrier(0);                             \
  } while (0)
#define TSTAMP(i) do { if (GWW_STAMP == 3) MSTAMP(100 + (i)); } while (0)
#define MSTAMP_FLUSH                                                                 \
  if (lane == 0) {                                                                   \
    for (int _q = 0; _q < 20; ++_q) atomicAdd(&g_stamp_mlp[_q], _acc[_q]);           \
    atomicAdd(&g_stamp_mlp[21], __builtin_amdgcn_s_memrealtime() - _rb);             \
    atomicAdd(&g_stamp_mlp[22], __builtin_amdgcn_s_memtime() - _tb);                 \
    atomicAdd(&g_stamp_mlp[23], 1ull);                                                \
  }
#else
#define MSTAMP_DECL
#define MSTAMP(i)
#define TSTAMP(i)
#define MSTAMP_FLUSH
#endif
}

__device__ __forceinline__ const float* mf_x0_row(const MfX0& z, const float* X, long g, bool x0, bool& tail, int& seg) {
  tail = false; seg = 0;
  if (!x0) return X + g * MF_D;
  const unsigned b = (unsigned)g / (unsigned)z.T, j = (unsigned)g - b * (unsigned)z.T;
  seg = (int)b;
  tail = (int)j >= z.Tt - 2 && (int)j <= z.T - 2;
  if (tail) return z.pos + (long)j * MF_D;
  return z.xs + ((long)b * z.Tt + ((int)j == z.T - 1 ? z.Tt - 1 : (int)j)) * MF_D;
}

struct MfNoX0 {};
template <int MODE, bool OP, bool X0 = false, int XL = 0>
__global__ __launch_bounds__(MF_THREADS, 1) void k_mlp_fused(const float* X, const unsigned short* delta, float* x_out,
                                                            const float* __restrict__ ln_u,
                                                            const float* __restrict__ ln_cb,
                                                            const unsigned short* __restrict__ Wt,
                                                            const float* __restrict__ b2,
                                                            unsigned short* __restrict__ C, long M, int F,
                                                            int stagger_ticks, const float* __restrict__ q_u,
                                                            const float* __restrict__ q_cb,
                                                            unsigned short* __restrict__ q_out, int NQ,
                                                            float* x_next, const float* __restrict__ bo, int keep_x_new,
                                                            const std::conditional_t<X0, MfX0, MfNoX0> z) {
  __shared__ __attribute__((aligned(16))) unsigned char lds[MF_LDS];
  constexpr bool QKV = MODE == 1 || MODE == 2, LNQ = MODE == 2, FIN = MODE == 3;
  static_assert(!X0 || (GWW_MF_NORM && GWW_MF_XACC && (MODE == 2 || (MODE == 1 && OP))), "X0: layer 0's two launches; stages in the u table");
  constexpr bool XACC = GWW_MF_XACC && GWW_MF_NORM && GWW_MF_SCHED && OP && (MODE == 1 || MODE == 3);
  constexpr bool XIN = (XL & 1) != 0, XOUT = (XL & 2) != 0;
  constexpr bool CSP = GWW_MF_CSPREAD && XACC;
  constexpr bool XPR = CSP && !X0 && !(GWW_MF_ABL & 32);
  static_assert(XL == 0 || (XACC && !GWW_MF_XLDS && !X0 && (!XOUT || MODE == 1) && XL <= 3), "XL: the accumulator-order stream of XACC");
  constexpr int MF_NST = MF_AHEAD + 1;
  float* lds_cb = reinterpret_cast<float*>(lds + MF_OFF_CB);
  float* lds_u = reinterpret_cast<float*>(lds + MF_OFF_U);
  float* lds_b2 = reinterpret_cast<float*>(lds + MF_OFF_B2);
  float* lds_bo = reinterpret_cast<float*>(lds + MF_OFF_BO);
  float* lds_qcb = reinterpret_cast<float*>(lds + MF_OFF_QCB);
  constexpr int OP_TILES = OP ? 3 * MF_KT : 0;
  typedef __attribute__((address_space(3))) void* lds_ptr;

  const int tid = threadIdx.x, lane = tid & 63, wave = tid >> 6;
  const int r = lane & 31, hh = lane >> 5;
  const long m_base = (long)blockIdx.x * MF_BM + wave * 32;
  unsigned char* slice = lds + MF_OFF_SLICE + wave * MF_SLICE_BYTES;
  unsigned char* const slice0 = slice;
  const int crow = lane >> 3, cchunk = lane & 7;

  const int wave_u = __builtin_amdgcn_readfirstlane(wave);
  const unsigned lane_off = (unsigned)lane * 16u;
  const unsigned lds_base = (unsigned)(unsigned long long)(lds_ptr)lds;
  auto issue_piece_c = [&](int tile, int stage, auto j_c) {
    constexpr int J = decltype(j_c)::value;
    const unsigned dst = lds_base + (unsigned)(stage * MF_TILE + MF_GL * wave_u * 1024);
    if (GWW_MF_EXP & 8) tile &= 7;
    const unsigned short* src = Wt + ((long)tile * (MF_TILE / 2) + MF_GL * wave_u * 512);
    const unsigned lo = lane_off;
    asm volatile("s_mov_b32 m0, %2\n\ts_nop 0\n\tglobal_load_lds_dwordx4 %0, %1 offset:%3"
                 :
                 : "v"(lo), "s"(src), "s"(dst), "n"(J * 1024)
                 : "memory");
  };
  auto issue_piece = [&](int tile, int stage, int j) {
#if GWW_MF_OLDDMA
    const unsigned dst = lds_base + (unsigned)(stage * MF_TILE + (MF_GL * wave_u + j) * 1024);
    const unsigned short* src = Wt + ((long)tile * (MF_TILE / 2) + (MF_GL * wave_u + j) * 512);
    unsigned keep;
    asm volatile("s_mov_b32 %0, m0\n\ts_mov_b32 m0, %3\n\ts_nop 0\n\tglobal_load_lds_dwordx4 %1, %2\n\ts_mov_b32 m0, %0"
                 : "=&s"(keep) : "v"(lane_off), "s"(src), "s"(dst) : "memory");
#else
    if (j == 0) issue_piece_c(tile, stage, std::integral_constant<int, 0>{});
    else if (j == 1) issue_piece_c(tile, stage, std::integral_constant<int, 1>{});
    else if (j == 2) issue_piece_c(tile, stage, std::integral_constant<int, 2>{});
    else issue_piece_c(tile, stage, std::integral_constant<int, 3>{});
#endif
  };
  auto issue = [&](int tile, int stage) {
#pragma unroll
    for (int j = 0; j < MF_GL; ++j) issue_piece(tile, stage, j);
  };

  MSTAMP_DECL
  auto stage_tables = [&]() {
    for (int i = tid; i < F; i += MF_THREADS) {
      lds_cb[i] = GWW_MF_SCHED ? ln_cb[i] * 0.125f : ln_cb[i];
// ... 22 lines not shown
#pragma unroll
    for (int k = 0; k < TB_D; ++k) { table_piece(tb_b2[k], b2, tid + MF_THREADS * k, MF_D); table_piece(tb_bo[k], bo, tid + MF_THREADS * k, MF_D); }
    if constexpr (FIN) {
#pragma unroll
      for (int k = 0; k < TB_D; ++k) { table_piece(tb_qu[k], q_u, tid + MF_THREADS * k, MF_D); table_piece(tb_q[k], q_cb, tid + MF_THREADS * k, MF_D); }
    }
    if constexpr (QKV) {
#pragma unroll
      for (int k = 0; k < TB_CB; ++k) table_piece(tb_q[k], q_cb, tid + MF_THREADS * k, NQ);
    }
  };
  auto publish_tables = [&]() {
#pragma unroll
    for (int k = 0; k < TB_CB; ++k) {
      asm volatile("" : "+v"(tb_cb[k]));
      if (tid + MF_THREADS * k < F) lds_cb[tid + MF_THREADS * k] = tb_cb[k] * 0.125f;
    }
#pragma unroll
    for (int k = 0; k < TB_D; ++k) {
      asm volatile("" : "+v"(tb_b2[k]), "+v"(tb_bo[k]));
      if (tid + MF_THREADS * k < MF_D) {
        lds_b2[tid + MF_THREADS * k] = tb_b2[k] + tb_bo[k];
        lds_bo[tid + MF_THREADS * k] = tb_bo[k];
      }
    }
    if constexpr (FIN) {
#pragma unroll
      for (int k = 0; k < TB_D; ++k) {
        asm volatile("" : "+v"(tb_qu[k]), "+v"(tb_q[k]));
        if (tid + MF_THREADS * k < MF_D) { lds_u[tid + MF_THREADS * k] = tb_qu[k]; lds_u[MF_D + tid + MF_THREADS * k] = tb_q[k]; }
      }
    }
    if constexpr (QKV) {
#pragma unroll
      for (int k = 0; k < TB_CB; ++k) {
        asm volatile("" : "+v"(tb_q[k]));
        if (tid + MF_THREADS * k < NQ) lds_qcb[tid + MF_THREADS * k] = tb_q[k];
      }
    }
  };
  if (stagger_ticks > 0 && blockIdx.x < 256) {
    const unsigned long long t0 = __builtin_amdgcn_s_memrealtime();
    const unsigned long long wait = (unsigned long long)((blockIdx.x >> 3) & 15) * stagger_ticks;
    while (__builtin_amdgcn_s_memrealtime() - t0 < wait) __builtin_amdgcn_s_sleep(8);
  }

#pragma unroll
  for (int p = 0; p < MF_AHEAD; ++p) issue(p, p);
  if constexpr (XACC) request_tables();
  const long xrow_l = m_base + r < M ? m_base + r : M - 1;
  const unsigned xoff = (unsigned)xrow_l * (unsigned)(MF_D * 4) + 16u * (unsigned)hh;
  const unsigned xoff_n = (unsigned)(xrow_l >> 5) * (unsigned)(32 * MF_D * 4) + 16u * (((unsigned)xrow_l & 31u) + 32u * (unsigned)hh);
  const unsigned coff = (unsigned)xrow_l * (unsigned)(MF_D * 2) + 64u * (unsigned)hh;
  f32x4 xp[XACC ? MF_OT : 1][4];
  bool x0 = false;
  int x0_seg0 = 0;
  f32x4* const lds_x0 = reinterpret_cast<f32x4*>(lds + MF_OFF_U);
  const float* x0_stage[2] = {nullptr, nullptr};
  f32x4 x0_sg[2];
  bool x0_tail = false;
  int x0_seg = 0;
  if constexpr (X0) {
    x0 = __builtin_amdgcn_readfirstlane(*z.flag) != 0;
    const unsigned g0 = (unsigned)blockIdx.x * (unsigned)MF_BM;
    x0_seg0 = (int)(g0 / (unsigned)z.T);
    const int seg_last = (int)((unsigned)(M - 1) / (unsigned)z.T);
#pragma unroll
    for (int k = 0; k < 2; ++k) {
      const int q = tid + 256 * k < 4 * (MF_D / 4) ? tid + 256 * k : tid;
      const int sg = q / (2 * (MF_D / 4)), wh = (q / (MF_D / 4)) & 1, c = q % (MF_D / 4);
      const long b = x0_seg0 + sg < seg_last ? x0_seg0 + sg : seg_last;
      x0_stage[k] = (wh ? z.tr + b * MF_D : z.xs + (b * z.Tt + (z.Tt - 2)) * MF_D) + 4 * c;
    }
  }
  auto x0_publish = [&](f32x4 (&sg)[2]) {
    lds_x0[tid] = sg[0];
    if (tid + 256 < 4 * (MF_D / 4)) lds_x0[tid + 256] = sg[1];
    asm volatile("s_waitcnt lgkmcnt(0)" ::: "memory");
    __builtin_amdgcn_s_barrier();
    asm volatile("" ::: "memory");
  };
  if constexpr (XACC && X0) {
    const float* xsrc = mf_x0_row(z, X, xrow_l, x0, x0_tail, x0_seg) + 4 * hh;
#pragma unroll
    for (int t = 0; t < MF_OT; ++t)
#pragma unroll
      for (int cc = 0; cc < 4; ++cc)
        asm volatile("global_load_dwordx4 %0, %1, off offset:%2" MF_XNT : "=a"(xp[t][cc]) : "v"(xsrc), "n"((32 * t + 8 * cc) * 4) : "memory");
#pragma unroll
    for (int k = 0; k < 2; ++k) asm volatile("global_load_dwordx4 %0, %1, off" : "=v"(x0_sg[k]) : "v"(x0_stage[k]) : "memory");
  } else if constexpr (XACC) {
#pragma unroll
    for (int t = 0; t < (XPR ? 4 : MF_OT); ++t)
#pragma unroll
      for (int cc = 0; cc < 4; ++cc)
        if (GWW_MF_ABL & 32) asm volatile("v_accvgpr_write_b32 %0, 0" : "=a"(xp[t][cc][0]));
        else if constexpr (XIN)
          asm volatile("global_load_dwordx4 %0, %1, %2 offset:%3" MF_XN_LDNT : "=a"(xp[t][cc]) : "v"(xoff_n), "s"(reinterpret_cast<const char*>(X) + 4096 * t), "n"(1024 * cc) : "memory");
        else asm volatile("global_load_dwordx4 %0, %1, %2 offset:%3" MF_XNT : "=a"(xp[t][cc]) : "v"(xoff), "s"(X), "n"((32 * t + 8 * cc) * 4) : "memory");
  }
  bf16x8 af[MF_KT * 4];
  float row_rstd, row_mean;
  long grow[4];
#pragma unroll
  for (int i = 0; i < 4; ++i) {
    const long g = m_base + 8 * i + crow;
    grow[i] = g < M ? g : M - 1;
  }
  if constexpr (XACC) {
#pragma unroll
    for (int S = 0; S < (CSP ? 1 : MF_KT); ++S)
#pragma unroll
      for (int j = 0; j < 4; ++j)
        asm volatile("global_load_dwordx4 %0, %1, %2 offset:%3" : "=v"(af[4 * S + j]) : "v"(coff), "s"(delta), "n"((64 * S + 8 * j) * 2) : "memory");
    if constexpr (XPR) {
#pragma unroll
      for (int t = 4; t < MF_OT; ++t)
#pragma unroll
        for (int cc = 0; cc < 4; ++cc)
          if constexpr (XIN)
            asm volatile("global_load_dwordx4 %0, %1, %2 offset:%3" MF_XN_LDNT : "=a"(xp[t][cc]) : "v"(xoff_n), "s"(reinterpret_cast<const char*>(X) + 4096 * t), "n"(1024 * cc) : "memory");
          else asm volatile("global_load_dwordx4 %0, %1, %2 offset:%3" MF_XNT : "=a"(xp[t][cc]) : "v"(xoff), "s"(X), "n"((32 * t + 8 * cc) * 4) : "memory");
    }
    if constexpr (X0) {
      if (x0) {
        asm volatile("s_waitcnt vmcnt(%2)" : "+v"(x0_sg[0]), "+v"(x0_sg[1]) : "n"(CSP ? 4 : 4 * MF_KT) : "memory");
#pragma unroll
        for (int t = 0; t < MF_OT; ++t) asm volatile("" : "+a"(xp[t][0]), "+a"(xp[t][1]), "+a"(xp[t][2]), "+a"(xp[t][3]));
        x0_publish(x0_sg);
        if (x0_tail) {
          const f32x4* const st = lds_x0 + (x0_seg - x0_seg0) * (2 * (MF_D / 4)) + hh;
#pragma unroll
          for (int t = 0; t < MF_OT; ++t)
#pragma unroll
            for (int cc = 0; cc < 4; ++cc) {
              const f32x4 xt = st[8 * t + 2 * cc], rt = st[MF_D / 4 + 8 * t + 2 * cc];
#pragma unroll
              for (int k = 0; k < 4; ++k) xp[t][cc][k] = __builtin_fmaf(xt[k], rt[k], xp[t][cc][k]);
            }
        }
      }
    }
    asm volatile("s_waitcnt vmcnt(%0)" ::"n"(XPR ? 32 : 0) : "memory");
#pragma unroll
    for (int i = 0; i < (CSP ? 4 : MF_KT * 4); ++i) asm volatile("" : "+v"(af[i]));
    publish_tables();
    row_rstd = 1.f; row_mean = 0.f;
  } else if constexpr (OP) {
    const unsigned short* crow_p[4];
#pragma unroll
    for (int i = 0; i < 4; ++i) crow_p[i] = delta + grow[i] * MF_D + 8 * cchunk;
    u32x4 cv[MF_KT][4];
#pragma unroll
    for (int S = 0; S < MF_KT; ++S)
#pragma unroll
      for (int i = 0; i < 4; ++i) {
        if (GWW_MF_ABL & 64) { cv[S][i] = u32x4{0x3f803f80u, 0x3f803f80u, 0x3f803f80u, 0x3f803f80u}; continue; }
        asm volatile("global_load_dwordx4 %0, %1, off offset:%2" MF_NT : "=v"(cv[S][i]) : "v"(crow_p[i]), "n"(64 * S * 2) : "memory");
      }
#pragma unroll
    for (int S = 0; S < MF_KT; ++S) {
#pragma unroll
      for (int i = 0; i < 4; ++i) {
        if (!(GWW_MF_ABL & 64)) asm volatile("s_waitcnt vmcnt(%1)" : "+v"(cv[S][i]) : "n"(23 - (4 * S + i)));
        *reinterpret_cast<u32x4*>(slice + (8 * i + crow) * MF_SLICE_STRIDE + cchunk * 16) = cv[S][i];
      }
// ... 450 lines not shown
            xn4[np % 3][h2][i] = v;
            if (np == 0 && h2 == 0) {
              float t = (v[0] + v[1]) + (v[2] + v[3]);
              t = mf_sum8(t);
              cshift[i] = t * (1.0f / 32.0f);
            }
            v[0] -= cshift[i]; v[1] -= cshift[i]; v[2] -= cshift[i]; v[3] -= cshift[i];
            s1[i] += (v[0] + v[1]) + (v[2] + v[3]);
            s2[i] += (v[0] * v[0] + v[1] * v[1]) + (v[2] * v[2] + v[3] * v[3]);
            u32x2 o = {pack2bf(v[0], v[1]), pack2bf(v[2], v[3])};
            *reinterpret_cast<u32x2*>(slice + (8 * i + crow) * MF_SLICE_STRIDE + h2 * 64 + cchunk * 8) = o;
          }
#pragma unroll
        for (int j = 0; j < 4; ++j) {
          u32x4 u = *reinterpret_cast<const u32x4*>(slice + r * MF_SLICE_STRIDE + (4 * hh + j) * 16);
          asm volatile("" : "+v"(u)::"memory");
          af[4 * np + j] = __builtin_bit_cast(bf16x8, u);
        }
        if (np == 2) request(3);
        store_chunk(np);
      }
      float* stat = reinterpret_cast<float*>(slice0);
#pragma unroll
      for (int i = 0; i < 4; ++i) {
        float a = s1[i], b = s2[i];
        a = mf_sum8(a); b = mf_sum8(b);
        const float mean = a * (1.0f / MF_D);
        const float var = fmaxf(b * (1.0f / MF_D) - mean * mean, 0.f);
        if (cchunk == 0) {
          stat[8 * i + crow] = rsqrtf(var + 1e-5f);
          stat[32 + 8 * i + crow] = mean;
        }
      }
      row_rstd = stat[r];
      row_mean = stat[32 + r];
      asm volatile("" : "+v"(row_rstd), "+v"(row_mean)::"memory");
      };
  auto seam_x = [&](const float* sb, float* dst, auto native_c, const unsigned xst_n) {
    constexpr bool NAT = decltype(native_c)::value;
    if constexpr (XACC) {
    float s1 = 0.f, s2 = 0.f, csh = 0.f;
#pragma unroll
    for (int t = 0; t < MF_OT; ++t)
#pragma unroll
      for (int cc = 0; cc < 4; ++cc) {
        const float4 bv = *reinterpret_cast<const float4*>(sb + 32 * t + 8 * cc + 4 * hh);
        f32x4 v = {oacc[t][4 * cc] + bv.x, oacc[t][4 * cc + 1] + bv.y, oacc[t][4 * cc + 2] + bv.z, oacc[t][4 * cc + 3] + bv.w};
        if (dst && !(GWW_MF_ABL & 16)) {
          if (GWW_MF_XLDS) {
            *reinterpret_cast<f32x4*>(slice0 + (t & 1) * (MF_WAVES * MF_SLICE_BYTES) + r * MF_SLICE_STRIDE + (8 * cc + 4 * hh) * 4) = v;
          } else if constexpr (NAT) {
            asm volatile("global_store_dwordx4 %0, %1, %2 offset:%3" MF_XN_STNT "\n\ts_nop 1" : : "v"(xst_n), "v"(v), "s"(reinterpret_cast<char*>(dst) + 4096 * t), "n"(1024 * cc) : "memory");
          } else {
            f32x4* const sp = reinterpret_cast<f32x4*>(reinterpret_cast<char*>(dst) + (XL != 0 && MODE == 1 ? xst_n : xoff) + (32 * t + 8 * cc) * 4);
            if (GWW_MF_XSTNT) __builtin_nontemporal_store(v, sp);
            else *sp = v;
          }
        }
        if (GWW_MF_XLDS && dst && !(GWW_MF_ABL & 16) && cc == 3) {
#pragma unroll
          for (int i = 0; i < 4; ++i) {
            const f32x4 u = *reinterpret_cast<const f32x4*>(slice0 + (t & 1) * (MF_WAVES * MF_SLICE_BYTES) + (8 * i + crow) * MF_SLICE_STRIDE + cchunk * 16);
            *reinterpret_cast<f32x4*>(reinterpret_cast<char*>(dst) + (unsigned)grow[i] * (unsigned)(MF_D * 4) + 16u * (unsigned)cchunk + t * 128) = u;
          }
        }
        if (t == 0 && cc == 0) {
          const auto sw = __builtin_amdgcn_permlane32_swap(__float_as_uint(v[0]), __float_as_uint(v[0]), false, false);
          csh = hh ? __uint_as_float(sw[0]) : v[0];
        }
        v[0] -= csh; v[1] -= csh; v[2] -= csh; v[3] -= csh;
        s1 += (v[0] + v[1]) + (v[2] + v[3]);
        s2 += (v[0] * v[0] + v[1] * v[1]) + (v[2] * v[2] + v[3] * v[3]);
      }
    {
      const auto a = __builtin_amdgcn_permlane32_swap(__float_as_uint(s1), __float_as_uint(s1), false, false);
      const auto b = __builtin_amdgcn_permlane32_swap(__float_as_uint(s2), __float_as_uint(s2), false, false);
      s1 = __uint_as_float(a[0]) + __uint_as_float(a[1]);
      s2 = __uint_as_float(b[0]) + __uint_as_float(b[1]);
    }
    const float mean_s = s1 * (1.0f / MF_D);
    row_rstd = rsqrtf(fmaxf(s2 * (1.0f / MF_D) - mean_s * mean_s, 0.f) + 1e-5f);
    row_mean = csh + mean_s;
    const float nm = -mean_s * row_rstd;
    asm volatile("" : "+a"(oacc[0]), "+a"(oacc[1]), "+a"(oacc[2]), "+a"(oacc[3]), "+a"(oacc[4]), "+a"(oacc[5]), "+a"(oacc[6]),
                      "+a"(oacc[7]), "+a"(oacc[8]), "+a"(oacc[9]), "+a"(oacc[10]), "+a"(oacc[11]));
#pragma unroll
    for (int S = 0; S < MF_KT; ++S)
#pragma unroll
      for (int cc = 0; cc < 4; ++cc) {
        const float4 be = *reinterpret_cast<const float4*>(sb + 64 * S + 8 * cc + 4 * hh);
        const float4 bo_ = *reinterpret_cast<const float4*>(sb + 64 * S + 32 + 8 * cc + 4 * hh);
        const f32x16& E = oacc[2 * S];
        const f32x16& O = oacc[2 * S + 1];
        const unsigned e0 = pack2bf(fmaf(E[4 * cc] + be.x - csh, row_rstd, nm), fmaf(E[4 * cc + 1] + be.y - csh, row_rstd, nm));
        const unsigned e1 = pack2bf(fmaf(E[4 * cc + 2] + be.z - csh, row_rstd, nm), fmaf(E[4 * cc + 3] + be.w - csh, row_rstd, nm));
        const unsigned o0 = pack2bf(fmaf(O[4 * cc] + bo_.x - csh, row_rstd, nm), fmaf(O[4 * cc + 1] + bo_.y - csh, row_rstd, nm));
        const unsigned o1 = pack2bf(fmaf(O[4 * cc + 2] + bo_.z - csh, row_rstd, nm), fmaf(O[4 * cc + 3] + bo_.w - csh, row_rstd, nm));
        const auto w0 = __builtin_amdgcn_permlane32_swap(e0, o0, false, false);
        const auto w1 = __builtin_amdgcn_permlane32_swap(e1, o1, false, false);
        const u32x4 f = {w0[0], w1[0], w0[1], w1[1]};
        af[4 * S + cc] = __builtin_bit_cast(bf16x8, f);
      }
      }
  };
  if constexpr (OP) {
    static_assert(12 % MF_NST == 0, "OP mode relies on a ring whose depth divides the 12-tile body (4 or 6 stages)");
    static_assert(!CSP || (MF_AHEAD == 3 && MF_GL == 4), "CSP: the riders' schedule is derived for a four-stage ring of four pieces per wave");
#pragma unroll
    for (int kt = 0; kt < MF_KT; ++kt) {
#pragma unroll
      for (int nt = 0; nt < 3; ++nt) {
        const int itile = kt * 3 + nt;
        const int rid_prev = !CSP || itile < 1 || itile > 13 ? 0 : itile == 1 ? 4 : (itile - 2) % 3 == 2 ? 2 : 1;
        const int ring_wait = XPR && itile == 0 ? 32 : XPR && itile == 1 ? 16 + MF_GL + 4 : MF_GL * (MF_AHEAD - 2) + rid_prev + (CSP && itile == 2 ? 1 : 0);
        if (!(GWW_MF_ABL & 128)) asm volatile("s_waitcnt vmcnt(%0)" ::"n"(ring_wait) : "memory");
        if constexpr (XPR) {
          if (kt == 0 && nt > 0) {
#pragma unroll
            for (int t = 4 * nt; t < 4 * nt + 4; ++t) {
              asm volatile("" : "+a"(xp[t][0]), "+a"(xp[t][1]), "+a"(xp[t][2]), "+a"(xp[t][3]));
              const auto lo = __builtin_shufflevector(xp[t][0], xp[t][1], 0, 1, 2, 3, 4, 5, 6, 7);
              const auto hi = __builtin_shufflevector(xp[t][2], xp[t][3], 0, 1, 2, 3, 4, 5, 6, 7);
              oacc[t] = __builtin_shufflevector(lo, hi, 0, 1, 2, 3, 4, 5, 6, 7, 8, 9, 10, 11, 12, 13, 14, 15);
            }
          }
        }
        if (CSP && nt == 0 && kt > 0) asm volatile("" : "+v"(af[4 * kt]), "+v"(af[4 * kt + 1]), "+v"(af[4 * kt + 2]), "+v"(af[4 * kt + 3]));
        __builtin_amdgcn_s_barrier();
        const int st = itile % MF_NST, st_next = (itile + 1) % MF_NST, dma_st = (itile + MF_AHEAD) % MF_NST;
        const int dma_tile = itile + MF_AHEAD < total ? itile + MF_AHEAD : total - 1;
        const bool last = itile == OP_TILES - 1;
#pragma unroll
        for (int sub = 0; sub < 4; ++sub) {
          const int q = 4 * kt + sub;
          bf16x8(&cur)[4] = wf[q & 1];
          bf16x8(&nxt)[4] = wf[(q + 1) & 1];
          const unsigned char* Wn = lds + (sub == 3 ? st_next : st) * MF_TILE;
          if (!(GWW_MF_ABL & 128)) issue_piece(dma_tile, dma_st, sub);
          if constexpr (CSP) {
            const int rm = (itile + 2) % 3, rS = (itile + 5) / 3;
            const int cp = itile == 0 ? 4 + sub : itile > 12 ? -1 : sub == 1 ? 4 * rS + rm : sub == 2 && rm == 2 ? 4 * rS + 3 : -1;
            if (cp >= 0)
              asm volatile("global_load_dwordx4 %0, %1, %2 offset:%3" : "=v"(af[cp >= 0 ? cp : 0]) : "v"(coff), "s"(delta), "n"((64 * (cp / 4) + 8 * (cp % 4)) * 2) : "memory");
          }
#pragma unroll
          for (int u = 0; u < 4; ++u) {
            asm volatile(MF_PADNOP "v_mfma_f32_32x32x16_bf16 %0, %1, %2, %0" : "+a"(oacc[4 * nt + u]) : "v"(cur[u]), "v"(af[4 * kt + sub]));
            const int off = (last && sub == 3) ? (u & 1) * 8192 + off1[u >> 1] : u * 4096 + offq[(sub + 1) & 3];
            nxt[u] = *reinterpret_cast<const bf16x8*>(Wn + off);
          }
        }
      }
    }
    it = OP_TILES;
    stage = OP_TILES % MF_NST;
    TSTAMP(14);
    asm volatile("s_nop 15\n\ts_nop 15"
                 : "+a"(oacc[0]), "+a"(oacc[1]), "+a"(oacc[2]), "+a"(oacc[3]), "+a"(oacc[4]), "+a"(oacc[5]), "+a"(oacc[6]),
                   "+a"(oacc[7]), "+a"(oacc[8]), "+a"(oacc[9]), "+a"(oacc[10]), "+a"(oacc[11]));
    if constexpr (XACC) {
      if constexpr (XL != 0 && MODE == 1) {
        unsigned lo = lane_off;
        asm volatile("" : "+v"(lo));
        const long g = m_base + (long)((lo >> 4) & 31u);
        const unsigned gc = (unsigned)(g < M ? g : M - 1);
        seam_x(lds_bo, (keep_x_new && !(GWW_MF_ABL & 256)) ? x_out : nullptr, std::false_type{}, gc * (unsigned)(MF_D * 4) + ((lo >> 9) << 4));
      } else
      seam_x(lds_bo, (keep_x_new && !(GWW_MF_ABL & 256)) ? x_out : nullptr, std::false_type{}, 0u);
    } else {
    seam(X, x_out, lds_bo, [] {});
#if GWW_MF_NORM
    normalise_af();
#endif
#pragma unroll
    for (int t = 0; t < MF_OT; ++t)
#pragma unroll
      for (int j = 0; j < 16; ++j) oacc[t][j] = 0.f;
    }
    TSTAMP(15);
  }
  if constexpr (!LNQ) {
  if (GWW_MF_SCHED) {
#pragma unroll
    for (int t = 0; t < 4; ++t)
#pragma unroll
      for (int q = 0; q < 4; ++q) preload_bias(t, t >> 1, q);
  }
  using IW = std::conditional_t<OP && !XACC && !(GWW_MF_ABL & 32), I2, I1>;
  run_tile(MF_FL<0>{}, I0{}, I0{}, I0{}, IM{}, 0, 0, IM{}, 0, IW{});
  run_tile(MF_FL<1>{}, I0{}, I0{}, I1{}, IM{}, 0, 0, IM{}, 0, IW{});
  run_tile(MF_FL<2>{}, I0{}, I0{}, I2{}, IM{}, 0, 0, IM{}, 0, I1{});
  TSTAMP(12);
  if (GWW_MF_SCHED) asm volatile("s_nop 15\n\ts_nop 15" : "+v"(sacc[0]), "+v"(sacc[1]), "+v"(sacc[2]), "+v"(sacc[3]));
  act_piece(0, 0, 0); act_piece(0, 0, 1); act_piece(0, 0, 2); act_piece(0, 0, 3);
  TSTAMP(13);
  int b = 0;
  for (; b + 2 < nck; b += 2) {
    run_tile(MF_FL<3>{}, I0{}, I1{}, I0{}, I1{}, b >> 1, 0, IM{}, 0, I0{});
    run_tile(MF_FL<4>{}, I0{}, I1{}, I1{}, I1{}, b >> 1, 0, IM{}, 0, I0{});
    run_tile(MF_FL<5>{}, I0{}, I1{}, I2{}, I1{}, b >> 1, 1, IM{}, 0, I0{});
    run_tile(MF_FL<6>{}, I1{}, I0{}, I0{}, I2{}, b >> 1, 1, I0{}, b + 2, I0{});
    run_tile(MF_FL<7>{}, I1{}, I0{}, I1{}, I2{}, b >> 1, 1, IM{}, 0, I0{});
    run_tile(MF_FL<8>{}, I1{}, I0{}, I2{}, I2{}, b >> 1, 0, IM{}, 0, I0{});
    run_tile(MF_FL<9>{}, I0{}, I0{}, I0{}, I3{}, b >> 1, 0, IM{}, 0, I0{});
    run_tile(MF_FL<10>{}, I0{}, I0{}, I1{}, I3{}, b >> 1, 0, IM{}, 0, I0{});
    run_tile(MF_FL<11>{}, I0{}, I0{}, I2{}, I3{}, b >> 1, 1, IM{}, 0, I0{});
    run_tile(MF_FL<12>{}, I1{}, I1{}, I0{}, I0{}, (b >> 1) + 1, 1, I1{}, b + 3, I0{});
    run_tile(MF_FL<13>{}, I1{}, I1{}, I1{}, I0{}, (b >> 1) + 1, 1, IM{}, 0, I0{});
    run_tile(MF_FL<14>{}, I1{}, I1{}, I2{}, I0{}, (b >> 1) + 1, 0, IM{}, 0, I0{});
  }
  run_tile(MF_FL<3>{}, I0{}, I1{}, I0{}, I1{}, b >> 1, 0, IM{}, 0, I1{});
  run_tile(MF_FL<4>{}, I0{}, I1{}, I1{}, I1{}, b >> 1, 0, IM{}, 0, I1{});
  run_tile(MF_FL<5>{}, I0{}, I1{}, I2{}, I1{}, b >> 1, 1, IM{}, 0, I1{});
  run_tile(MF_FL<6>{}, I1{}, I0{}, I0{}, I2{}, b >> 1, 1, IM{}, 0, I1{});
// ... 509 lines not shown
      const int row2 = within >> 4, ch = (within & 15) ^ (row2 & 15);
      v = *reinterpret_cast<const u32x4*>(wq + (long)(64 * cq + row2) * MF_D + 128 * k3 + 8 * ch);
#else
      const int it2 = tile - mlp_tiles, nt = it2 / MF_KT, kt = it2 - nt * MF_KT;
      v = *reinterpret_cast<const u32x4*>(wq + (long)(128 * nt + row) * MF_D + 64 * kt + 8 * chunk);
#endif
    } else {
      int kind, cp, idx3;
      if (tile < 3) { kind = 0; cp = 0; idx3 = tile; }
      else {
        const int k = tile - 3, blk = k / 6, w = k - 6 * blk;
        if (blk == nck - 1) { kind = 1; cp = blk; idx3 = w; }
        else if (w < 3) { kind = 0; cp = blk + 1; idx3 = w; }
        else { kind = 1; cp = blk; idx3 = w - 3; }
      }
      if (kind == 0) {
        const int row2 = within >> 4, ch = (within & 15) ^ (row2 & 15);
        v = *reinterpret_cast<const u32x4*>(w1 + (long)(64 * cp + row2) * MF_D + 128 * idx3 + 8 * ch);
        if (GWW_MF_SCHED) v = mf_scale_bf16x8(v, 0.125f);
      } else {
        const unsigned short* src = w2 + (long)(128 * idx3 + row) * F + 64 * cp;
        unsigned short e[8];
#pragma unroll
        for (int j = 0; j < 8; ++j) {
          const int p = 8 * chunk + j;
          e[j] = src[(p & ~12) | ((p & 4) << 1) | ((p & 8) >> 1)];
        }
        v = u32x4{(unsigned)e[0] | ((unsigned)e[1] << 16), (unsigned)e[2] | ((unsigned)e[3] << 16),
                  (unsigned)e[4] | ((unsigned)e[5] << 16), (unsigned)e[6] | ((unsigned)e[7] << 16)};
        if (GWW_MF_SCHED) v = mf_scale_bf16x8(v, 8.0f);
      }
    }
    reinterpret_cast<u32x4*>(out)[g] = v;
  }
}

int launch_mlp_pack(const void* w1_folded, const void* w2, const void* wqkv_folded, void* out, int d, int F, int NQ,
                    hipStream_t s, const void* wo) {
  GWW_REQUIRE(d == MF_D && F % 128 == 0 && F >= 0 && (F > 0 || wqkv_folded),
              "mlp_pack: d must be 384 and ffn a multiple of 128 (0: only the q / k / v panel, for LayerNorm 1 + q / k / v alone)");
  GWW_REQUIRE(!wqkv_folded || (NQ > 0 && NQ % 128 == 0), "mlp_pack: the q / k / v panel needs NQ %% 128 == 0");
  GWW_REQUIRE(!wo || F > 0, "mlp_pack: an out_proj panel goes in front of an MLP stream");
  const long n16 = ((wo ? (long)MF_D * MF_D : 0) + 2L * MF_D * F + (wqkv_folded ? (long)NQ * MF_D : 0)) / 8;
  hipLaunchKernelGGL(k_mlp_pack, dim3((unsigned)cdiv(n16, 256)), dim3(256), 0, s, (const unsigned short*)w1_folded,
                     (const unsigned short*)w2, (const unsigned short*)wqkv_folded, (unsigned short*)out, F, n16,
                     (const unsigned short*)wo);
  GWW_LAUNCH_CHECK();
  return GWW_OK;
}

bool mlp_fused_supported(int d, int F) { return d == MF_D && F > 0 && F % 128 == 0 && F <= MF_FMAX; }
constexpr bool MF_XL_BUILT = GWW_MF_XACC && GWW_MF_NORM && GWW_MF_SCHED && !GWW_MF_XLDS;
bool mlp_fused_x_native_supported() { return MF_XL_BUILT; }

int launch_mlp_fused(const MlpFusedArgs& a, hipStream_t s) {
  const char* who = a.who;
  const void* const A = a.ctx ? a.ctx : a.delta;
  const bool op = a.ctx != nullptr, lnq = !A, fin = a.y != nullptr, qkv = a.qkv_out != nullptr, x0 = a.x0 != nullptr;
  GWW_REQUIRE(!(a.ctx && a.delta) && op == (a.bo != nullptr), "%s: a pending delta, or ctx with the out_proj bias", who);
  GWW_REQUIRE(!fin || (op && !qkv && !a.C && a.lnf_w && a.lnf_b), "%s: the final LayerNorm takes ctx, bo, lnf_w, lnf_b and no other output", who);
  GWW_REQUIRE(!a.last_token || (fin && a.T > 0 && a.M % a.T == 0 && (((uintptr_t)a.last_token) & 15) == 0 && a.last_token != a.y),
              "%s: last_token comes with y, T rows per segment and M %% T == 0", who);
  const int xl = (a.x_native_in ? 1 : 0) | (a.x_native_out ? 2 : 0);
  GWW_REQUIRE(!xl || (MF_XL_BUILT && op && !a.keep_x_new && !x0 && (!a.x_native_out || (qkv && !a.x_next))),
              "%s: the accumulator-order residual stream runs between ctx blocks that keep no x_new, in place", who);
  GWW_REQUIRE(!xl || (long)x_native_bytes(a.M) < (1L << 32), "%s: M = %ld rows exceed the 32-bit offsets of the accumulator-order stream", who, a.M);
  GWW_REQUIRE(!lnq || (!a.x_new && !a.ln_u && !a.ln_cb && !a.b2 && !a.C && a.F == 0), "%s: LayerNorm 1 + q / k / v alone takes no block operand", who);
  GWW_REQUIRE(fin || qkv || (!lnq && a.C), "%s: no output", who);
  GWW_REQUIRE(!x0 || (!a.x_new && !a.keep_x_new && (lnq || (op && qkv))), "%s: x0 runs LN1 + q / k / v alone or ctx + block + q / k / v, without x_new", who);
  GWW_REQUIRE(a.Wt && (x0 || a.x) && (lnq || (a.ln_u && a.ln_cb && a.b2 && (x0 || a.x_new))) && (!a.keep_x_new || a.x_new), "%s: NULL operand", who);
  GWW_REQUIRE(a.d == MF_D && (lnq || mlp_fused_supported(a.d, a.F)),
              "%s: built for d_model = 384 and ffn a multiple of 128, <= 1536 (got %d, %d)", who, a.d, a.F);
  GWW_REQUIRE(!qkv || (a.qkv_u && a.qkv_cb && a.NQ > 0 && a.NQ % 128 == 0 && a.NQ <= MF_FMAX),
              "%s: the q / k / v projection needs u, cb and NQ %% 128 == 0, NQ <= 1536", who);
  GWW_REQUIRE(x0 || lnq || ((const void*)a.x_new != (const void*)a.x && (const void*)a.y != (const void*)a.x_new),
              "%s: x_new must alias neither x nor y", who);
  GWW_REQUIRE((lnq && !x0) || a.M * (long)(MF_D * 4) < (1L << 32), "%s: M = %ld rows exceed the 32-bit row offsets of the seams", who, a.M);
  GWW_REQUIRE((((x0 ? 0 : (uintptr_t)a.x) | ((uintptr_t)A) | ((uintptr_t)a.x_new) | ((uintptr_t)a.Wt) | ((uintptr_t)a.C) |
                ((uintptr_t)a.qkv_out) | ((uintptr_t)a.y)) & 15) == 0, "%s: operands must be 16-byte aligned", who);
  if (a.M == 0) return GWW_OK;
  if (x0) {
    const MfX0& z = *a.x0;
    GWW_REQUIRE(z.xs && z.tr && z.pos && z.flag && a.x, "%s: NULL operand", who);
    GWW_REQUIRE(z.T >= MF_BM && z.Tt >= 3 && z.Tt < z.T && a.M % z.T == 0, "%s: bad shape M=%ld T=%d Tt=%d", who, a.M, z.T, z.Tt);
    GWW_REQUIRE(((((uintptr_t)z.xs) | ((uintptr_t)z.tr) | ((uintptr_t)z.pos) | ((uintptr_t)a.x)) & 15) == 0 && (((uintptr_t)z.flag) & 3) == 0,
                "%s: operands must be 16-byte aligned", who);
  }
  float* const x_next = !qkv || lnq ? nullptr : a.x_next ? a.x_next : const_cast<float*>(a.x);
  GWW_REQUIRE(!x_next || ((((uintptr_t)x_next) & 15) == 0 && x_next != a.x_new), "%s: x_next must not alias x_new", who);
  const long panels = cdiv(a.M, MF_BM);
  static const int stagger_env = (int)lab_int("GWW_MLP_STAGGER", 0);
  const int stagger = !lnq && !fin && !x0 && panels >= 512 ? stagger_env : 0;
  auto launch = [&](auto kernel, auto z) {
    hipLaunchKernelGGL(kernel, dim3((unsigned)panels), dim3(MF_THREADS), 0, s, a.x, (const unsigned short*)A, a.x_new, a.ln_u, a.ln_cb,
                       (const unsigned short*)a.Wt, a.b2, fin ? reinterpret_cast<unsigned short*>(a.y) : (unsigned short*)a.C, a.M, a.F,
                       stagger, fin ? a.lnf_w : qkv ? a.qkv_u : nullptr, fin ? a.lnf_b : qkv ? a.qkv_cb : nullptr,
                       fin ? reinterpret_cast<unsigned short*>(a.last_token) : (unsigned short*)a.qkv_out,
                       fin ? (a.last_token ? a.T : 0) : qkv ? a.NQ : 0, x_next, a.bo, a.keep_x_new ? 1 : 0, z);
  };
  if constexpr (MF_XL_BUILT) {
    if (xl) {
      const int mode = fin ? 3 : 1;
      if (mode == 1 && !x0 && xl == 2) launch(k_mlp_fused<1, true, false, 2>, MfNoX0{});
      else if (mode == 1 && xl == 3) launch(k_mlp_fused<1, true, false, 3>, MfNoX0{});
      else if (mode == 3 && xl == 1) launch(k_mlp_fused<3, true, false, 1>, MfNoX0{});
      else return fail(GWW_ERR_ARG, "%s: no such instantiation of k_mlp_fused", who);
      GWW_LAUNCH_CHECK();
      return GWW_OK;
    }
  }
  switch ((lnq ? 2 : fin ? 3 : qkv ? 1 : 0) | (op ? 4 : 0) | (x0 ? 8 : 0)) {
    case 5: launch(k_mlp_fused<1, true>, MfNoX0{}); break;
    case 1: launch(k_mlp_fused<1, false>, MfNoX0{}); break;
    case 4: launch(k_mlp_fused<0, true>, MfNoX0{}); break;
    case 0: launch(k_mlp_fused<0, false>, MfNoX0{}); break;
    case 7: launch(k_mlp_fused<3, true>, MfNoX0{}); break;
    case 2: launch(k_mlp_fused<2, false>, MfNoX0{}); break;
    case 10: launch(k_mlp_fused<2, false, true>, *a.x0); break;
    case 13: launch(k_mlp_fused<1, true, true>, *a.x0); break;
    default: return fail(GWW_ERR_ARG, "%s: no such instantiation of k_mlp_fused", who);
  }
  GWW_LAUNCH_CHECK();
  return GWW_OK;
}

}

using namespace gww;

#ifdef GWW_STAMP
extern "C" int gww_debug_stamps_mlp(unsigned long long* out8, int reset) {
  GWW_HIP(hipMemcpyFromSymbol(out8, HIP_SYMBOL(gww::g_stamp_mlp), sizeof(unsigned long long) * 24));
  if (reset) {
    unsigned long long z[24] = {0};
    GWW_HIP(hipMemcpyToSymbol(HIP_SYMBOL(gww::g_stamp_mlp), z, sizeof(z)));
  }
  return GWW_OK;
}
#endif

extern "C" int gww_mlp_pack_bf16(const void* w1_folded, const void* w2, const void* wqkv_folded_or_null, void* out, int d,
                                 int F, int NQ, void* stream) {
  GWW_REQUIRE(out && ((w1_folded && w2) || (F == 0 && wqkv_folded_or_null)), "gww_mlp_pack_bf16: NULL argument");
  return launch_mlp_pack(w1_folded, w2, wqkv_folded_or_null, out, d, F, NQ, (hipStream_t)stream, nullptr);
}

extern "C" int gww_mlp_pack_op_bf16(const void* wo, const void* w1_folded, const void* w2, const void* wqkv_folded_or_null,
                                    void* out, int d, int F, int NQ, void* stream) {
  GWW_REQUIRE(wo && w1_folded && w2 && out, "gww_mlp_pack_op_bf16: NULL argument");
  return launch_mlp_pack(w1_folded, w2, wqkv_folded_or_null, out, d, F, NQ, (hipStream_t)stream, wo);
}

static MlpFusedArgs mf_block_args(const char* who, const float* x, float* x_new, const float* ln_u, const float* ln_cb, const void* Wt,
                                  const float* b2, long M, int d, int F) {
  MlpFusedArgs a;
  a.who = who; a.x = x; a.x_new = x_new; a.keep_x_new = x_new != nullptr; a.ln_u = ln_u; a.ln_cb = ln_cb; a.Wt = Wt; a.b2 = b2;
  a.M = M; a.d = d; a.F = F;
  return a;
}
static void mf_qkv_args(MlpFusedArgs& a, const float* qkv_u, const float* qkv_cb, void* qkv_out, int NQ) {
  a.qkv_u = qkv_u; a.qkv_cb = qkv_cb; a.qkv_out = qkv_out; a.NQ = NQ;
}

extern "C" int gww_attn_out_mlp_fused_bf16(float* x, const void* ctx, const float* bo, float* x_out, const float* ln_u,
                                           const float* ln_cb, const void* Wt, const float* b2, void* C, long M, int d,
                                           int F, const float* qkv_u, const float* qkv_cb, void* qkv_out, int NQ,
                                           void* stream) {
  GWW_REQUIRE(ctx && bo, "gww_attn_out_mlp_fused_bf16: NULL ctx or out_proj bias");
  MlpFusedArgs a = mf_block_args("gww_attn_out_mlp_fused_bf16", x, x_out, ln_u, ln_cb, Wt, b2, M, d, F);
  a.ctx = ctx; a.bo = bo; a.C = C;
  mf_qkv_args(a, qkv_u, qkv_cb, qkv_out, NQ);
  return launch_mlp_fused(a, (hipStream_t)stream);
}

extern "C" int gww_attn_out_mlp_final_bf16(const float* x, const void* ctx, const float* bo, float* x_mid, const float* ln_u,
                                          const float* ln_cb, const void* Wt, const float* b2, const float* lnf_w,
                                          const float* lnf_b, float* y, long M, int d, int F, void* stream) {
  MlpFusedArgs a = mf_block_args("gww_attn_out_mlp_final_bf16", x, x_mid, ln_u, ln_cb, Wt, b2, M, d, F);
  a.ctx = ctx; a.bo = bo; a.lnf_w = lnf_w; a.lnf_b = lnf_b; a.y = y;
  return launch_mlp_fused(a, (hipStream_t)stream);
}

extern "C" int gww_lnqkv_fused_bf16(const float* x, const float* qkv_u, const float* qkv_cb, const void* Wt, void* qkv_out,
                                    long M, int d, int NQ, void* stream) {
  MlpFusedArgs a;
  a.who = "gww_lnqkv_fused_bf16"; a.x = x; a.Wt = Wt; a.M = M; a.d = d;
  mf_qkv_args(a, qkv_u, qkv_cb, qkv_out, NQ);
  return launch_mlp_fused(a, (hipStream_t)stream);
}

extern "C" int gww_mlp_fused_bf16(float* x, const void* delta, float* x_out, const float* ln_u,
                                  const float* ln_cb, const void* Wt, const float* b2, void* C, long M, int d,
                                  int F, const float* qkv_u, const float* qkv_cb, void* qkv_out, int NQ,
                                  void* stream) {
  GWW_REQUIRE(delta, "gww_mlp_fused_bf16: NULL operand");
  MlpFusedArgs a = mf_block_args("gww_mlp_fused_bf16", x, x_out, ln_u, ln_cb, Wt, b2, M, d, F);
  a.delta = delta; a.C = C;
  mf_qkv_args(a, qkv_u, qkv_cb, qkv_out, NQ);
  return launch_mlp_fused(a, (hipStream_t)stream);
}

extern "C" int gww_lnqkv_fused_x0_bf16(const float* xs, const float* tr, const float* pos, const int* flag, const float* x, int T,
                                       int Tt, const float* qkv_u, const float* qkv_cb, const void* Wt, void* qkv_out, long M,
                                       int d, int NQ, void* stream) {
  const MfX0 z{xs, tr, pos, flag, T, Tt};
  MlpFusedArgs a;
  a.who = "gww_lnqkv_fused_x0_bf16"; a.x = x; a.x0 = &z; a.Wt = Wt; a.M = M; a.d = d;
  mf_qkv_args(a, qkv_u, qkv_cb, qkv_out, NQ);
  return launch_mlp_fused(a, (hipStream_t)stream);
}

extern "C" int gww_attn_out_mlp_fused_x0_bf16(const float* xs, const float* tr, const float* pos, const int* flag, float* x, int T,
                                              int Tt, const void* ctx, const float* bo, const float* ln_u, const float* ln_cb,
                                              const void* Wt, const float* b2, long M, int d, int F, const float* qkv_u,
                                              const float* qkv_cb, void* qkv_out, int NQ, void* stream) {
  GWW_REQUIRE(ctx, "gww_attn_out_mlp_fused_x0_bf16: NULL operand");
  const MfX0 z{xs, tr, pos, flag, T, Tt};
  MlpFusedArgs a = mf_block_args("gww_attn_out_mlp_fused_x0_bf16", x, nullptr, ln_u, ln_cb, Wt, b2, M, d, F);
  a.ctx = ctx; a.bo = bo; a.x0 = &z;
  mf_qkv_args(a, qkv_u, qkv_cb, qkv_out, NQ);
  return launch_mlp_fused(a, (hipStream_t)stream);
}
```

### gw_whisper_amd/encoder.py

```python

from __future__ import annotations

import ctypes as C
import operator
import sys
import weakref
from dataclasses import dataclass

import torch
import torch.nn as nn

from . import _lib, synth
from ._lib import check, lib


@dataclass
class WhisperConfig:
    d_model: int = 384
    encoder_layers: int = 4
    encoder_attention_heads: int = 6
    encoder_ffn_dim: int = 1536
    num_mel_bins: int = 80
    max_source_positions: int = 1500
    dropout: float = 0.0
# ... 330 lines not shown
                             f"{x.shape[-1]}. Make sure to pad the input mel features to {t_in}.")
        if c.named[0][1].device != x.device:
            raise _lib.GwwError("encoder parameters and input are on different devices")
        return c

    def forward_raw(self, input_features: torch.Tensor, want_hidden: bool = True, want_last: bool = False, cache=None):
        c = self._enter(input_features) if cache is None else cache
        x, prec = input_features.to(torch.float32).contiguous(), self._prec
        cfg = self.config
        B = x.shape[0]
        with torch.cuda.device(x.device):
            self._sync_weights(c)
            ws = self._workspace(B, prec, x.device)
            hidden = torch.empty((B, cfg.max_source_positions, cfg.d_model), dtype=torch.float32,
                                 device=x.device) if want_hidden else None
            last = torch.empty((B, cfg.d_model), dtype=torch.float32, device=x.device) if want_last else None
            check(lib().gww_encoder_forward(self._handle, x.data_ptr(), B, prec, ws.data_ptr(), ws.numel(),
                                            hidden.data_ptr() if want_hidden else None,
                                            last.data_ptr() if want_last else None,
                                            torch.cuda.current_stream().cuda_stream), "gww_encoder_forward")
        return hidden, last

    def forward_outputs_raw(self, input_features: torch.Tensor, want_hidden_states: bool, want_attentions: bool,
                            cache=None):
        c = self._enter(input_features) if cache is None else cache
        x, prec = input_features.to(torch.float32).contiguous(), self._prec
        cfg = self.config
        B, T, d, L, H = x.shape[0], cfg.max_source_positions, cfg.d_model, cfg.encoder_layers, cfg.encoder_attention_heads
        f32 = dict(dtype=torch.float32, device=x.device)
        with torch.cuda.device(x.device):
            self._sync_weights(c)
            ws = self._workspace(B, prec, x.device)
            hs = torch.empty((L + 1, B, T, d), **f32) if want_hidden_states else None
            last = hs[L] if want_hidden_states else torch.empty((B, T, d), **f32)
            at = torch.empty((L, B, H, T, T), **f32) if want_attentions else None
            check(lib().gww_encoder_forward_outputs(self._handle, x.data_ptr(), B, prec, ws.data_ptr(), ws.numel(),
                                                    last.data_ptr(), hs.data_ptr() if hs is not None else None,
                                                    at.data_ptr() if at is not None else None,
                                                    torch.cuda.current_stream().cuda_stream), "gww_encoder_forward_outputs")
        hidden_states = tuple(hs[:L].unbind(0)) + (last,) if hs is not None else None
        attentions = tuple(at.unbind(0)) if at is not None else None
        return last, hidden_states, attentions

    def set_split(self, on: bool = True):
        check(lib().gww_encoder_set_split(self._ensure_handle(), int(on)), "gww_encoder_set_split")
        self._ws = None

    def set_stem_shortcut(self, on: bool = True):
        check(lib().gww_encoder_set_stem_shortcut(self._ensure_handle(), int(on)), "gww_encoder_set_stem_shortcut")

    def set_x_native(self, on: bool = True):
        check(lib().gww_encoder_set_x_native(self._ensure_handle(), int(on)), "gww_encoder_set_x_native")

    def stem_shortcut_flags(self, batch: int) -> tuple:
        if self._ws is None:
            raise _lib.GwwError("stem_shortcut_flags: no forward has run yet")
        flags = (C.c_int * 2)()
        with torch.cuda.device(self._ws.device):
            torch.cuda.synchronize()
            check(lib().gww_encoder_stem_shortcut_flags(self._ensure_handle(), int(batch), self._prec, self._ws.data_ptr(), flags),
                  "gww_encoder_stem_shortcut_flags")
        return int(flags[0]), int(flags[1])

    def trace_enable(self, on: bool = True):
        check(lib().gww_encoder_trace_enable(self._ensure_handle(), int(on)), "gww_encoder_trace_enable")

    def trace_read(self) -> dict:
        n = lib().gww_encoder_trace_classes()
        ms = (C.c_float * n)()
        cnt = (C.c_int * n)()
        check(lib().gww_encoder_trace_read(self._ensure_handle(), ms, cnt), "gww_encoder_trace_read")
        return {lib().gww_encoder_trace_class_name(i).decode(): (float(ms[i]), int(cnt[i])) for i in range(n)}

    def forward(self, input_features, attention_mask=None, output_hidden_states=None, output_attentions=None,
                return_dict=None, **kwargs):
        c = self.config
        want_h = c.output_hidden_states if output_hidden_states is None else bool(output_hidden_states)
        want_a = c.output_attentions if output_attentions is None else bool(output_attentions)
        as_dict = c.return_dict if return_dict is None else bool(return_dict)
        cache = self._enter(input_features)
        if self._wants_grad(input_features, cache):
            if want_h or want_a:
                raise _lib.GwwError("WhisperEncoder: output_hidden_states / output_attentions are inference only (no "
                                    "gradient flows through them): run under torch.no_grad() or freeze the adapters")
            from .training import encoder_train_forward
            out = BaseModelOutput(last_hidden_state=encoder_train_forward(self, input_features, cache=cache))
        elif want_h or want_a:
            last, hs, at = self.forward_outputs_raw(input_features, want_h, want_a, cache=cache)
            out = BaseModelOutput(last_hidden_state=last, hidden_states=hs, attentions=at)
        else:
            hidden, _ = self.forward_raw(input_features, want_hidden=True, want_last=False, cache=cache)
            out = BaseModelOutput(last_hidden_state=hidden)
        return out if as_dict else out.to_tuple()

    def _wants_grad(self, input_features, c=None) -> bool:
        if not torch.is_grad_enabled():
            return False
        c = self._param_cache() if c is None else c
        input_grad = torch.is_tensor(input_features) and input_features.requires_grad
        base_trainable = [n for n, p in c.base if p.requires_grad]
        if not base_trainable and not any(p.requires_grad for p in c.adapters):
            return input_grad
        if self.full_finetune:
            if c.adapters:
                raise _lib.GwwError("WhisperEncoder: full fine-tuning is enabled and DoRA / LoRA adapters are attached: "
                                    "the two do not combine")
# ... 18 lines not shown
```

### gw_whisper_amd/ops.py

```python

from __future__ import annotations

import torch

from . import _lib
from ._lib import check, lib


def _stream() -> int:
    return torch.cuda.current_stream().cuda_stream


def _dev(t: torch.Tensor, dtype=None, name="tensor") -> torch.Tensor:
    if not t.is_cuda:
        raise _lib.GwwError(f"{name} must live on the GPU (got {t.device}); gw_whisper_amd has no CPU path")
    if dtype is not None and t.dtype != dtype:
        raise _lib.GwwError(f"{name} must be {dtype}, got {t.dtype}")
    return t.contiguous()


_frontend = {}


def _fe(device, n_mels: int = 80) -> int:
# ... 132 lines not shown
        if c.dtype != torch.bfloat16 or not c.is_cuda or not c.is_contiguous() or c.dim() != 2 or c.shape[0] < Mp \
                or c.shape[1] != N:
            raise _lib.GwwError(f"gemm_astat: out must be a contiguous bf16 GPU tensor of [>= {Mp}, {N}]")
    if dgelu and (delta is None or tuple(delta.shape[1:]) != (N,) or delta.shape[0] < M or not delta.is_contiguous()):
        raise _lib.GwwError(f"gemm_astat: the gelu-backward epilogue needs a contiguous delta of [>= {M}, {N}]")
    dl = _dev(delta, torch.bfloat16, "delta") if delta is not None else None
    x_out = torch.empty_like(a) if (fused and return_x and dl is not None) else None
    with torch.cuda.device(a.device):
        check(lib().gww_gemm_astat_bf16(
            a.data_ptr(), dl.data_ptr() if (dl is not None and (x_out is not None or dgelu)) else None,
            x_out.data_ptr() if x_out is not None else None,
            _dev(ln[0], torch.float32).data_ptr() if fused else None,
            _dev(ln[1], torch.float32).data_ptr() if fused else None, w.data_ptr(),
            _dev(bias, torch.float32).data_ptr() if bias is not None else None, c.data_ptr(), M, N, K,
            epilogue, _stream()), "gww_gemm_astat_bf16")
    return (c[:M], x_out if x_out is not None else a) if return_x else c[:M]


def gemm_fulln(a: torch.Tensor, w: torch.Tensor, bias=None, epilogue: int = 0) -> torch.Tensor:
    a = _dev(a, torch.bfloat16, "A")
    w = _dev(w, torch.bfloat16, "W")
    M, K = a.shape
    N = w.shape[0]
    Mp = (M + 127) // 128 * 128
    c = torch.empty((Mp, N), dtype=torch.bfloat16, device=a.device)
    with torch.cuda.device(a.device):
        check(lib().gww_gemm_fulln_bf16(a.data_ptr(), w.data_ptr(),
                                        _dev(bias, torch.float32).data_ptr() if bias is not None else None,
                                        c.data_ptr(), M, N, K, epilogue, _stream()), "gww_gemm_fulln_bf16")
    return c[:M]


def mlp_pack(w1_folded: torch.Tensor, w2: torch.Tensor, wqkv_folded: torch.Tensor | None = None) -> torch.Tensor:
    wq = _dev(wqkv_folded, torch.bfloat16, "Wqkv") if wqkv_folded is not None else None
    if w1_folded is None:
        if wq is None:
            raise _lib.GwwError("mlp_pack: nothing to pack")
        w1 = w2 = None
        F, d = 0, wq.shape[1]
    else:
        w1 = _dev(w1_folded, torch.bfloat16, "W1")
        w2 = _dev(w2, torch.bfloat16, "W2")
        F, d = w1.shape
    NQ = wq.shape[0] if wq is not None else 0
    dev = wq.device if w1 is None else w1.device
    out = torch.empty((2 * d * F + NQ * d,), dtype=torch.bfloat16, device=dev)
    with torch.cuda.device(dev):
        check(lib().gww_mlp_pack_bf16(w1.data_ptr() if w1 is not None else None, w2.data_ptr() if w2 is not None else None,
                                      wq.data_ptr() if wq is not None else None, out.data_ptr(), d, F, NQ, _stream()),
              "gww_mlp_pack_bf16")
    return out


def attn_out_mlp_fused(x, ctx, wo, bo, w1_folded, w2, ln_u, ln_cb, b2, qkv=None):
    x = _dev(x, torch.float32, "x")
    ctx = _dev(ctx, torch.bfloat16, "ctx")
    wo = _dev(wo, torch.bfloat16, "Wo")
    w1 = _dev(w1_folded, torch.bfloat16, "W1")
    w2 = _dev(w2, torch.bfloat16, "W2")
    wq = _dev(qkv[0], torch.bfloat16, "Wqkv") if qkv is not None else None
    F, d = w1.shape
    NQ = wq.shape[0] if wq is not None else 0
    M = x.shape[0]
    Mp = (M + 127) // 128 * 128
    f = lambda t: _dev(t, torch.float32)
    bo, u, cb, b2 = f(bo), f(ln_u), f(ln_cb), f(b2)
    wt = torch.empty((d * d + 2 * d * F + NQ * d,), dtype=torch.bfloat16, device=x.device)
    if qkv is not None:
        x = x.clone()
    x_out = torch.empty_like(x)
    with torch.cuda.device(x.device):
        check(lib().gww_mlp_pack_op_bf16(wo.data_ptr(), w1.data_ptr(), w2.data_ptr(), wq.data_ptr() if wq is not None else None,
                                         wt.data_ptr(), d, F, NQ, _stream()), "gww_mlp_pack_op_bf16")
        if qkv is None:
            out = torch.empty((Mp, d), dtype=torch.bfloat16, device=x.device)
            qu = qc = None
        else:
            qu, qc = f(qkv[1]), f(qkv[2])
            out = torch.empty((Mp, NQ), dtype=torch.bfloat16, device=x.device)
        check(lib().gww_attn_out_mlp_fused_bf16(x.data_ptr(), ctx.data_ptr(), bo.data_ptr(), x_out.data_ptr(), u.data_ptr(),
                                                cb.data_ptr(), wt.data_ptr(), b2.data_ptr(),
                                                out.data_ptr() if qkv is None else None, M, d, F,
                                                qu.data_ptr() if qu is not None else None,
                                                qc.data_ptr() if qc is not None else None,
                                                out.data_ptr() if qkv is not None else None, NQ, _stream()),
              "gww_attn_out_mlp_fused_bf16")
    return out[:M], (x_out if qkv is None else x)


def attn_out_mlp_final(x, ctx, wo, bo, w1_folded, w2, ln_u, ln_cb, b2, lnf_w, lnf_b):
    x = _dev(x, torch.float32, "x")
    ctx = _dev(ctx, torch.bfloat16, "ctx")
    wo, w1, w2 = _dev(wo, torch.bfloat16, "Wo"), _dev(w1_folded, torch.bfloat16, "W1"), _dev(w2, torch.bfloat16, "W2")
    F, d = w1.shape
    M = x.shape[0]
    f = lambda t: _dev(t, torch.float32)
    bo, u, cb, b2, lw, lb = f(bo), f(ln_u), f(ln_cb), f(b2), f(lnf_w), f(lnf_b)
    wt = torch.empty((d * d + 2 * d * F,), dtype=torch.bfloat16, device=x.device)
    x_mid, y = torch.empty_like(x), torch.empty_like(x)
    with torch.cuda.device(x.device):
        check(lib().gww_mlp_pack_op_bf16(wo.data_ptr(), w1.data_ptr(), w2.data_ptr(), None, wt.data_ptr(), d, F, 0, _stream()),
              "gww_mlp_pack_op_bf16")
        check(lib().gww_attn_out_mlp_final_bf16(x.data_ptr(), ctx.data_ptr(), bo.data_ptr(), x_mid.data_ptr(), u.data_ptr(),
                                                cb.data_ptr(), wt.data_ptr(), b2.data_ptr(), lw.data_ptr(), lb.data_ptr(),
                                                y.data_ptr(), M, d, F, _stream()), "gww_attn_out_mlp_final_bf16")
    return y, x_mid


def lnqkv_fused(x, wt, qkv_u, qkv_cb):
    x = _dev(x, torch.float32, "x")
    wt = _dev(wt, torch.bfloat16, "Wt")
    M, d = x.shape
    qu, qc = _dev(qkv_u, torch.float32), _dev(qkv_cb, torch.float32)
    NQ = qu.numel()
    qo = torch.empty(((M + 127) // 128 * 128, NQ), dtype=torch.bfloat16, device=x.device)
    with torch.cuda.device(x.device):
        check(lib().gww_lnqkv_fused_bf16(x.data_ptr(), qu.data_ptr(), qc.data_ptr(), wt.data_ptr(), qo.data_ptr(), M, d, NQ,
                                         _stream()), "gww_lnqkv_fused_bf16")
    return qo[:M]


def _x0_operands(xs, tr, pos, flag, x=None):
    xs, tr, pos = _dev(xs, torch.float32, "xs"), _dev(tr, torch.float32, "tr"), _dev(pos, torch.float32, "pos")
    if flag.dtype != torch.int32 or not flag.is_cuda or flag.numel() != 1:
        raise _lib.GwwError("flag must be one int32 on the device")
    B, Tt, d = xs.shape
    T = pos.shape[0]
    if tr.shape != (B, d) or pos.shape[1] != d:
        raise _lib.GwwError("tr must be [B, d] and pos [T, d]")
    if x is None:
        x = torch.empty((B * T, d), dtype=torch.float32, device=xs.device)
    else:
        x = _dev(x, torch.float32, "x")
        if x.numel() != B * T * d:
            raise _lib.GwwError("x must hold B * T rows")
    return xs, tr, pos, flag, x, B, T, Tt, d


def stem_fill(xs, tr, pos, flag, x=None):
    xs, tr, pos, flag, x, B, T, Tt, d = _x0_operands(xs, tr, pos, flag, x)
    with torch.cuda.device(xs.device):
        check(lib().gww_stem_fill_f32(xs.data_ptr(), tr.data_ptr(), pos.data_ptr(), flag.data_ptr(), x.data_ptr(), B, T, Tt, d,
                                      _stream()), "gww_stem_fill_f32")
    return x


def lnqkv_fused_x0(xs, tr, pos, flag, wt, qkv_u, qkv_cb, x=None):
    xs, tr, pos, flag, x, B, T, Tt, d = _x0_operands(xs, tr, pos, flag, x)
    wt = _dev(wt, torch.bfloat16, "Wt")
    qu, qc = _dev(qkv_u, torch.float32), _dev(qkv_cb, torch.float32)
    NQ, M = qu.numel(), B * T
    qo = torch.empty(((M + 127) // 128 * 128, NQ), dtype=torch.bfloat16, device=xs.device)
    with torch.cuda.device(xs.device):
        check(lib().gww_lnqkv_fused_x0_bf16(xs.data_ptr(), tr.data_ptr(), pos.data_ptr(), flag.data_ptr(), x.data_ptr(), T, Tt,
                                            qu.data_ptr(), qc.data_ptr(), wt.data_ptr(), qo.data_ptr(), M, d, NQ, _stream()),
              "gww_lnqkv_fused_x0_bf16")
    return qo[:M]


def attn_out_mlp_fused_x0(xs, tr, pos, flag, ctx, wo, bo, w1_folded, w2, ln_u, ln_cb, b2, qkv, x=None):
    xs, tr, pos, flag, x, B, T, Tt, d = _x0_operands(xs, tr, pos, flag, x)
    x = x.clone().view(B * T, d)
    ctx = _dev(ctx, torch.bfloat16, "ctx")
    wo, w1, w2 = _dev(wo, torch.bfloat16, "Wo"), _dev(w1_folded, torch.bfloat16, "W1"), _dev(w2, torch.bfloat16, "W2")
    wq = _dev(qkv[0], torch.bfloat16, "Wqkv")
    F, NQ, M = w1.shape[0], wq.shape[0], B * T
    f = lambda t: _dev(t, torch.float32)
    bo, u, cb, b2, qu, qc = f(bo), f(ln_u), f(ln_cb), f(b2), f(qkv[1]), f(qkv[2])
    wt = torch.empty((d * d + 2 * d * F + NQ * d,), dtype=torch.bfloat16, device=x.device)
    out = torch.empty(((M + 127) // 128 * 128, NQ), dtype=torch.bfloat16, device=x.device)
    with torch.cuda.device(x.device):
        check(lib().gww_mlp_pack_op_bf16(wo.data_ptr(), w1.data_ptr(), w2.data_ptr(), wq.data_ptr(), wt.data_ptr(), d, F, NQ,
                                         _stream()), "gww_mlp_pack_op_bf16")
        check(lib().gww_attn_out_mlp_fused_x0_bf16(xs.data_ptr(), tr.data_ptr(), pos.data_ptr(), flag.data_ptr(), x.data_ptr(), T, Tt,
                                                   ctx.data_ptr(), bo.data_ptr(), u.data_ptr(), cb.data_ptr(), wt.data_ptr(),
                                                   b2.data_ptr(), M, d, F, qu.data_ptr(), qc.data_ptr(), out.data_ptr(), NQ,
                                                   _stream()), "gww_attn_out_mlp_fused_x0_bf16")
    return out[:M], x


def mlp_fused(x, delta, wt, ln_u, ln_cb, b2, qkv=None):
    x = _dev(x, torch.float32, "x")
    delta = _dev(delta, torch.bfloat16, "delta")
    wt = _dev(wt, torch.bfloat16, "Wt")
    M, d = x.shape
    F = ln_u.numel()
    Mp = (M + 127) // 128 * 128
    if qkv is not None:
        x = x.clone()
    x_out = torch.empty_like(x)
    f = lambda t: _dev(t, torch.float32)
    u, cb, b2 = f(ln_u), f(ln_cb), f(b2)
    if qkv is None:
        c = torch.empty((Mp, d), dtype=torch.bfloat16, device=x.device)
        qu = qc = qo = None
        NQ = 0
    else:
        qu, qc = f(qkv[0]), f(qkv[1])
        NQ = qu.numel()
        qo = torch.empty((Mp, NQ), dtype=torch.bfloat16, device=x.device)
        c = None
    with torch.cuda.device(x.device):
        check(lib().gww_mlp_fused_bf16(x.data_ptr(), delta.data_ptr(), x_out.data_ptr(), u.data_ptr(), cb.data_ptr(),
                                       wt.data_ptr(), b2.data_ptr(), c.data_ptr() if c is not None else None, M, d, F,
                                       qu.data_ptr() if qu is not None else None,
                                       qc.data_ptr() if qc is not None else None,
                                       qo.data_ptr() if qo is not None else None, NQ, _stream()),
              "gww_mlp_fused_bf16")
    return ((c if qkv is None else qo)[:M], x_out if qkv is None else x)


def attention(qkv: torch.Tensor, n_heads: int) -> torch.Tensor:
    bf = qkv.dtype == torch.bfloat16
    qkv = _dev(qkv, torch.bfloat16 if bf else torch.float32, "qkv")
    B, T, d3 = qkv.shape
    d = d3 // 3
    if d != n_heads * 64:
        raise _lib.GwwError(f"attention: d={d} != n_heads*64")
    ctx = torch.empty((B, T, d), dtype=qkv.dtype, device=qkv.device)
    fn = lib().gww_attention_bf16 if bf else lib().gww_attention_f32
    with torch.cuda.device(qkv.device):
        check(fn(qkv.data_ptr(), ctx.data_ptr(), B, T, n_heads, _stream()), "gww_attention")
    return ctx


def attention_log2q(qkv: torch.Tensor, n_heads: int, want_lse: bool = False):
    qkv = _dev(qkv, torch.bfloat16, "qkv")
    B, T, d3 = qkv.shape
    if d3 != 3 * n_heads * 64:
        raise _lib.GwwError(f"attention: d={d3 // 3} != n_heads*64")
    ctx = torch.empty((B, T, d3 // 3), dtype=torch.bfloat16, device=qkv.device)
    lse = torch.empty((B, n_heads, T), dtype=torch.float32, device=qkv.device) if want_lse else None
    with torch.cuda.device(qkv.device):
        check(lib().gww_attention_log2q_bf16(qkv.data_ptr(), ctx.data_ptr(), lse.data_ptr() if want_lse else None, B, T,
                                             n_heads, _stream()), "gww_attention_log2q_bf16")
    return (ctx, lse) if want_lse else ctx


def attention_probs(qkv: torch.Tensor, n_heads: int, q_log2: bool = False) -> torch.Tensor:
    bf = qkv.dtype == torch.bfloat16
    qkv = _dev(qkv, torch.bfloat16 if bf else torch.float32, "qkv")
    B, T, d3 = qkv.shape
    if d3 != 3 * n_heads * 64:
        raise _lib.GwwError(f"attention_probs: d={d3 // 3} != n_heads*64")
    probs = torch.empty((B, n_heads, T, T), dtype=torch.float32, device=qkv.device)
    with torch.cuda.device(qkv.device):
        if bf:
            check(lib().gww_attention_probs_bf16(qkv.data_ptr(), int(bool(q_log2)), probs.data_ptr(), B, T, n_heads,
                                                 _stream()), "gww_attention_probs_bf16")
        elif q_log2:
            raise _lib.GwwError("attention_probs: q in log2 units is a bf16-path convention")
        else:
            check(lib().gww_attention_probs_f32(qkv.data_ptr(), probs.data_ptr(), B, T, n_heads, _stream()),
                  "gww_attention_probs_f32")
    return probs


def dora_merge(w0: torch.Tensor, a: torch.Tensor, b: torch.Tensor, m: torch.Tensor, scaling: float,
               return_norm: bool = False):
    w0 = _dev(w0, torch.float32, "w0")
    d_out, d_in = w0.shape
    r = a.shape[0]
    out = torch.empty_like(w0)
    nrm = torch.empty((d_out,), dtype=torch.float32, device=w0.device)
    with torch.cuda.device(w0.device):
        check(lib().gww_dora_merge_f32(w0.data_ptr(), _dev(a, torch.float32).data_ptr(),
                                       _dev(b, torch.float32).data_ptr(), _dev(m, torch.float32).data_ptr(),
                                       float(scaling), d_out, d_in, r, out.data_ptr(), nrm.data_ptr(), _stream()),
              "gww_dora_merge_f32")
    return (out, nrm) if return_norm else out


def conv1_gelu(mel: torch.Tensor, weight: torch.Tensor, bias: torch.Tensor) -> torch.Tensor:
    mel = _dev(mel, torch.float32, "mel")
    weight, bias = _dev(weight, torch.float32, "weight"), _dev(bias, torch.float32, "bias")
    B, C_, T = mel.shape
    d = weight.shape[0]
    if C_ != 80 or tuple(weight.shape) != (d, 80, 3) or tuple(bias.shape) != (d,):
        raise _lib.GwwError(f"conv1_gelu: mel {tuple(mel.shape)}, weight {tuple(weight.shape)}, bias {tuple(bias.shape)}")
    scratch = torch.empty((d, 256), dtype=torch.bfloat16, device=mel.device)
    out = torch.empty((B, T + 2, d), dtype=torch.bfloat16, device=mel.device)
    with torch.cuda.device(mel.device):
        check(lib().gww_conv1_gelu_bf16(mel.data_ptr(), weight.data_ptr(), bias.data_ptr(), scratch.data_ptr(), out.data_ptr(),
                                        B, T, d, _stream()), "gww_conv1_gelu_bf16")
    return out


def dora_merge_batch(items, return_norm: bool = True):
# ... 992 lines not shown
```

### include/gww.h

```cpp
#ifndef GWW_H
#define GWW_H

#include <stddef.h>
#include <stdint.h>

#ifdef __cplusplus
extern "C" {
#endif

#define GWW_VERSION 107

#define GWW_OK 0
#define GWW_ERR_ARG (-1)
#define GWW_ERR_HIP (-2)
#define GWW_ERR_WORKSPACE (-3)
#define GWW_ERR_STATE (-4)

#define GWW_PREC_BF16 0
#define GWW_PREC_F32 1

int gww_version(void);
const char* gww_last_error(void);

typedef struct gww_frontend gww_frontend;
// ... 7 lines not shown

typedef struct {
  int d_model;
  int n_layers;
  int n_heads;
  int ffn;
  int n_mels;
  int t_in;
} gww_enc_cfg;

typedef struct {
  const float* conv1_w; const float* conv1_b;
  const float* conv2_w; const float* conv2_b;
  const float* pos;
  const float* ln_w; const float* ln_b;
} gww_enc_globals;

typedef struct {
  const float* ln1_w; const float* ln1_b;
  const float* q_w; const float* q_b;
  const float* k_w;
  const float* v_w; const float* v_b;
  const float* o_w; const float* o_b;
  const float* ln2_w; const float* ln2_b;
  const float* fc1_w; const float* fc1_b;
  const float* fc2_w; const float* fc2_b;
} gww_enc_layer;

typedef struct gww_encoder gww_encoder;

int gww_encoder_create(const gww_enc_cfg* cfg, gww_encoder** out);
void gww_encoder_destroy(gww_encoder* enc);
int gww_encoder_set_weights(gww_encoder* enc, const gww_enc_globals* g,
                            const gww_enc_layer* layers, int n_layers, void* stream);
int gww_encoder_update_weights(gww_encoder* enc, const gww_enc_globals* globals_or_null,
                               const gww_enc_layer* layers, int n_layers, const unsigned* layer_dirty,
                               void* stream);
size_t gww_encoder_workspace_bytes(const gww_encoder* enc, int batch, int precision);
int gww_encoder_forward(gww_encoder* enc, const float* mel, int batch, int precision,
                        void* workspace, size_t workspace_bytes,
                        float* last_hidden, float* last_token, void* stream);
int gww_encoder_forward_outputs(gww_encoder* enc, const float* mel, int batch, int precision,
                                void* workspace, size_t workspace_bytes, float* last_hidden,
                                float* hidden_slab, float* attn_slab, void* stream);

int gww_encoder_set_split(gww_encoder* enc, int on);

int gww_encoder_set_stem_shortcut(gww_encoder* enc, int on);
int gww_encoder_stem_shortcut_flags(const gww_encoder* enc, int batch, int precision, const void* workspace, int* flags);

int gww_encoder_set_x_native(gww_encoder* enc, int on);
size_t gww_x_native_offset(long row, int col, long M);
size_t gww_x_native_bytes(long M);

int gww_encoder_trace_enable(gww_encoder* enc, int on);
int gww_encoder_trace_read(gww_encoder* enc, float* ms, int* counts);
int gww_encoder_trace_classes(void);
const char* gww_encoder_trace_class_name(int i);

int gww_dora_merge_f32(const float* w0, const float* a, const float* b, const float* m,
                       float scaling, int d_out, int d_in, int r,
                       float* w_eff, float* norm_out, void* stream);

int gww_conv1_gelu_bf16(const float* mel, const float* conv1_w, const float* conv1_b, void* w_scratch_bf16,
                        void* c1_out, int B, int T, int d, void* stream);

typedef struct {
  const float* w0;
  const float* a;
  const float* b;
  const float* m;
  float* w_eff;
  float* norm_out;
  float scaling;
  int d_out, d_in, r;
} gww_dora_merge_item;
int gww_dora_merge_batch_f32(const gww_dora_merge_item* items, int n, void* stream);

typedef struct {
  int layer;
  int proj;
  int r;
  float scaling;
  const float* A;
  const float* B;
  const float* mag;
  const float* nrm;
  float* dA;
  float* dB;
  float* dm;
} gww_dora_target;

size_t gww_train_saved_bytes(const gww_encoder* enc, int batch);
size_t gww_train_workspace_bytes(const gww_encoder* enc, int batch);
size_t gww_train_workspace_bytes_adapters(const gww_encoder* enc, int batch, int max_r);
int gww_encoder_train_forward(gww_encoder* enc, const float* mel, int batch, void* workspace,
                              size_t workspace_bytes, void* saved, size_t saved_bytes,
                              float* last_hidden, int pooled, void* stream);
int gww_encoder_train_backward(gww_encoder* enc, int batch, void* workspace, size_t workspace_bytes,
                               const void* saved, size_t saved_bytes, const float* d_last_hidden,
                               const gww_dora_target* targets, int n_targets, float* d_x0, float* d_mel,
                               int pooled, void* stream);

typedef struct {
  float* ln1_w; float* ln1_b;
  float* q_w; float* q_b;
// ... 269 lines not shown
```

Measured before the change: 26520 segments/s.

## Store attention ctx in MFMA operand order for the fused out-proj/MLP kernel

Adds a 'ctx native' layout in which the attention kernel writes its bf16 context output in the tiled operand order that the fused attention-output/MLP kernel loads directly. The consumer then reads ctx with 1 KB-strided dwordx4 loads (non-temporal by default) instead of row-major gathers. The aim is better coalescing of the ctx handoff between the two kernels. It adds a new template specialization, layout helpers, plan gating (on by default), and C and Python entry points, but is restricted to d=384 and the log2-q attention path.

After: 26630 segments/s (median of 6 runs). About the same (+0.4%).

```diff
diff --git a/gw_whisper_amd/_lib.py b/gw_whisper_amd/_lib.py
--- a/gw_whisper_amd/_lib.py
+++ b/gw_whisper_amd/_lib.py
@@ -78,6 +78,15 @@
     "gww_encoder_set_x_native": (C.c_int, [C.c_void_p, C.c_int]),
     "gww_x_native_offset": (C.c_size_t, [C.c_long, C.c_int, C.c_long]),
     "gww_x_native_bytes": (C.c_size_t, [C.c_long]),
+    "gww_encoder_set_ctx_native": (C.c_int, [C.c_void_p, C.c_int]),
+    "gww_ctx_native_offset": (C.c_size_t, [C.c_long, C.c_int, C.c_long]),
+    "gww_ctx_native_bytes": (C.c_size_t, [C.c_long]),
+    "gww_attention_log2q_ctxn_bf16": (C.c_int, [C.c_void_p, C.c_void_p, C.c_void_p, C.c_int, C.c_int, C.c_int, C.c_int, C.c_void_p]),
+    "gww_attn_out_mlp_fused_ctxn_bf16": (C.c_int, [C.c_void_p] * 9 + [C.c_long, C.c_int, C.c_int, C.c_void_p, C.c_void_p, C.c_void_p,
+                                                   C.c_int, C.c_int, C.c_void_p]),
+    "gww_attn_out_mlp_final_ctxn_bf16": (C.c_int, [C.c_void_p] * 11 + [C.c_long, C.c_int, C.c_int, C.c_int, C.c_void_p]),
+    "gww_attn_out_mlp_fused_x0_ctxn_bf16": (C.c_int, [C.c_void_p] * 5 + [C.c_int, C.c_int] + [C.c_void_p] * 6 + [C.c_long, C.c_int, C.c_int,
+                                                      C.c_void_p, C.c_void_p, C.c_void_p, C.c_int, C.c_int, C.c_void_p]),
     "gww_encoder_trace_enable": (C.c_int, [C.c_void_p, C.c_int]),
     "gww_encoder_trace_read": (C.c_int, [C.c_void_p, C.POINTER(C.c_float), C.POINTER(C.c_int)]),
     "gww_encoder_trace_classes": (C.c_int, []),
diff --git a/gw_whisper_amd/csrc/attention.hip b/gw_whisper_amd/csrc/attention.hip
--- a/gw_whisper_amd/csrc/attention.hip
+++ b/gw_whisper_amd/csrc/attention.hip
@@ -464,7 +464,10 @@
 #ifndef GWW_ATT_NBUF
 #define GWW_ATT_NBUF 2
 #endif
-template <int MINW, bool MSUM, bool NOMAX>
+#ifndef GWW_ATT_CN_STNT
+#define GWW_ATT_CN_STNT 0
+#endif
+template <int MINW, bool MSUM, bool NOMAX, bool CN = false>
 __global__ __launch_bounds__(256, MINW) void k_attention_dma_bf16(const unsigned short* __restrict__ qkv,
                                                                  unsigned short* __restrict__ ctx,
                                                                  float* __restrict__ lse, int T, int H, int q_tiles,
@@ -747,6 +750,12 @@
 #if GWW_ATT_EPI16
   {
     unsigned short* orow = ctx + ((long)b * T + q_row) * d + h * DH;
+    if constexpr (CN) {
+      int qr = q_row;
+      asm volatile("" : "+v"(qr));
+      const long g = (long)b * T + (qr < T ? qr : T - 1);
+      orow = reinterpret_cast<unsigned short*>(reinterpret_cast<char*>(ctx) + ((g >> 5) * 24 + 4 * h + hh) * 1024 + (g & 31) * 16);
+    }
 #pragma unroll
     for (int n = 0; n < 2; ++n)
 #pragma unroll
@@ -757,10 +766,18 @@
         const auto s0 = __builtin_amdgcn_permlane32_swap(a0, b0, false, false);
         const auto s1 = __builtin_amdgcn_permlane32_swap(a1, b1, false, false);
         u32x4 o = {s0[0], s1[0], s0[1], s1[1]};
+        if constexpr (CN) {
+#if GWW_ATT_CN_STNT
+          if (q_row < T) __builtin_nontemporal_store(o, reinterpret_cast<u32x4*>(orow + 1024 * cp + 256 * n));
+#else
+          if (q_row < T) *reinterpret_cast<u32x4*>(orow + 1024 * cp + 256 * n) = o;
+#endif
+        } else
         if (q_row < T) *reinterpret_cast<u32x4*>(orow + 32 * n + 8 * (hh ? c1 : c0)) = o;
       }
   }
 #else
+  static_assert(!CN, "the operand-order epilogue is the 16-byte one");
   if (q_row < T) {
     unsigned short* orow = ctx + ((long)b * T + q_row) * d + h * DH;
 #pragma unroll
@@ -1348,13 +1365,13 @@
 }
 
 int launch_attention_bf16(const void* qkv, void* ctx, int B, int T, int H, hipStream_t s, float* lse,
-                          bool last_tile_only, bool q_log2) {
+                          bool last_tile_only, bool q_log2, bool ctx_native) {
   GWW_REQUIRE(qkv && ctx, "attention_bf16: NULL operand");
   GWW_REQUIRE(B >= 0 && T > 0 && H > 0, "attention_bf16: bad shape B=%d T=%d H=%d", B, T, H);
   GWW_REQUIRE((((uintptr_t)qkv) & 15) == 0 && (((uintptr_t)ctx) & 15) == 0, "attention_bf16: 16-byte alignment");
   if (B == 0) return GWW_OK;
 #ifdef GWW_LAB
-  if (q_log2 && !last_tile_only && lab_int("GWW_ATT_W64", 0) != 0) return launch_attention_w64_bf16(qkv, ctx, B, T, H, s, lse);
+  if (q_log2 && !last_tile_only && !ctx_native && lab_int("GWW_ATT_W64", 0) != 0) return launch_attention_w64_bf16(qkv, ctx, B, T, H, s, lse);
 #endif
   const unsigned short* in = (const unsigned short*)qkv;
   unsigned short* out = (unsigned short*)ctx;
@@ -1370,6 +1387,14 @@
   const int q_tiles = last_tile_only ? 1 : all_tiles, qt0 = last_tile_only ? all_tiles - 1 : 0;
   const long blocks = (long)q_tiles * B * H;
   GWW_REQUIRE(blocks < 2147483647L, "attention_bf16: grid too large");
+  if (ctx_native) {
+    GWW_REQUIRE(q_log2 && !last_tile_only && H * DH == 384 && nw == 4,
+                "attention_bf16: ctx in operand order comes from the log2-unit kernel, on all rows, at d = 384");
+    hipLaunchKernelGGL((k_attention_dma_bf16<3, false, true, true>), dim3((unsigned)blocks), dim3(256), 0, s, in, out, lse, T, H,
+                       q_tiles, qt0);
+    GWW_LAUNCH_CHECK();
+    return GWW_OK;
+  }
 #define GWW_DMA(MW, MS, NM) hipLaunchKernelGGL((k_attention_dma_bf16<MW, MS, NM>), dim3((unsigned)blocks), dim3(256), 0, s, in, out, lse, T, H, q_tiles, qt0)
 #ifdef GWW_LAB
   if (pp && var_env >= 9) {
@@ -1659,6 +1684,10 @@
                                         void* stream) {
   return launch_attention_bf16(qkv, ctx, B, T, n_heads, (hipStream_t)stream, lse_or_null, false, true);
 }
+extern "C" int gww_attention_log2q_ctxn_bf16(const void* qkv, void* ctx, float* lse_or_null, int B, int T, int n_heads,
+                                             int ctx_native, void* stream) {
+  return launch_attention_bf16(qkv, ctx, B, T, n_heads, (hipStream_t)stream, lse_or_null, false, true, ctx_native != 0);
+}
 extern "C" int gww_attention_f32(const float* qkv, float* ctx, int B, int T, int n_heads, void* stream) {
   return launch_attention_f32(qkv, ctx, B, T, n_heads, (hipStream_t)stream);
 }
diff --git a/gw_whisper_amd/csrc/common.h b/gw_whisper_amd/csrc/common.h
--- a/gw_whisper_amd/csrc/common.h
+++ b/gw_whisper_amd/csrc/common.h
@@ -146,6 +146,14 @@
   return (slice * 48 + (size_t)(4 * t + cc)) * 1024 + (size_t)(r + 32 * hh) * 16 + (size_t)(4 * k);
 }
 inline size_t x_native_bytes(long M) { return (size_t)cdiv(M, 128) * 128 * 384 * 4; }
+
+__host__ __device__ inline size_t ctx_native_offset(long g, int c, long M) {
+  if (g > M - 1) g = M - 1;
+  const size_t slice = (size_t)(g >> 5);
+  const int r = (int)(g & 31), h = c >> 6, hh = (c >> 5) & 1, j = (c >> 3) & 3, k = c & 7;
+  return (slice * 24 + (size_t)(4 * h + j)) * 1024 + (size_t)(r + 32 * hh) * 16 + (size_t)(2 * k);
+}
+inline size_t ctx_native_bytes(long M) { return (size_t)cdiv(M, 32) * 32 * 384 * 2; }
 
 struct Arena {
   size_t off = 0;
diff --git a/gw_whisper_amd/csrc/encoder.hip b/gw_whisper_amd/csrc/encoder.hip
--- a/gw_whisper_amd/csrc/encoder.hip
+++ b/gw_whisper_amd/csrc/encoder.hip
@@ -304,6 +304,13 @@
   bool pooled;
   bool q_log2;
   bool x_native;
+  bool ctx_native;
+  bool ctx_native_x0;
+  bool ctx_native_layer(int i, int n_layers) const {
+    const bool last = i == n_layers - 1;
+    if (!ctx_native || !(last ? fuse_final : fuse_qkv)) return false;
+    return !(i == 0 && x0_layer0 && !last) || ctx_native_x0;
+  }
 };
 FwdPlan plan_forward(const gww_encoder* e, int batch, int precision, FwdWants want) {
   const gww_enc_cfg& c = e->cfg;
@@ -329,6 +336,10 @@
   p.x_native = e->x_native && p.op && p.fuse_final && !p.pooled && !want.hidden_slab && c.n_layers > 1 && d == 384 &&
                mlp_fused_x_native_supported() && !(m & GP_X_NATIVE) &&
                x_native_bytes((long)batch * T) <= padded_rows((size_t)batch * T) * d * 4;
+  p.ctx_native = e->ctx_native && bf && d == 384 && c.n_heads * 64 == d && p.op && p.q_log2 && !p.pooled && !want.hidden_slab &&
+                 !want.attn_slab && mlp_fused_ctx_native_supported(false) && !(m & GP_CTX_NATIVE) &&
+                 ctx_native_bytes((long)batch * T) <= padded_rows((size_t)batch * T) * d * 2;
+  p.ctx_native_x0 = p.ctx_native && mlp_fused_ctx_native_supported(true);
   return p;
 }
 }
@@ -363,6 +374,17 @@
   return x_native_offset(row, col, M);
 }
 extern "C" size_t gww_x_native_bytes(long M) { return M > 0 ? x_native_bytes(M) : 0; }
+
+extern "C" int gww_encoder_set_ctx_native(gww_encoder* e, int on) {
+  GWW_REQUIRE(e != nullptr, "gww_encoder_set_ctx_native: NULL handle");
+  e->ctx_native = on != 0;
+  return GWW_OK;
+}
+extern "C" size_t gww_ctx_native_offset(long row, int col, long M) {
+  if (row < 0 || col < 0 || col >= 384 || M <= 0) return (size_t)-1;
+  return ctx_native_offset(row, col, M);
+}
+extern "C" size_t gww_ctx_native_bytes(long M) { return M > 0 ? ctx_native_bytes(M) : 0; }
 
 extern "C" int gww_encoder_stem_shortcut_flags(const gww_encoder* e, int batch, int precision, const void* workspace,
                                                int* flags) {
@@ -570,14 +592,15 @@
     GWW_TRY(tap_hidden(i, st.xc));
     if (i == 0 && skew_event) GWW_HIP(hipEventRecord(skew_event, s));
     if (p.pooled && last) return pooled_last_layer(L, st.xc, st.xn, d1);
-    TR(TR_ATTN, launch_attention_bf16(qkv, ctx, B, T, H, s, nullptr, false, p.q_log2));
+    const bool ctx_n = p.ctx_native_layer(i, n_layers);
+    TR(TR_ATTN, launch_attention_bf16(qkv, ctx, B, T, H, s, nullptr, false, p.q_log2, ctx_n));
     GWW_TRY(tap_attn(i));
     if (!p.op)
       TR(TR_OUT, launch_gemm_astat(ctx, d, nullptr, nullptr, nullptr, nullptr, L.wo, L.bo, d1, M, d, d, EPI_BIAS, 0, s));
     MlpFusedArgs a = args();
     a.x = st.xc; a.x_new = from_x0 ? nullptr : st.xn; a.ln_u = L.u1; a.ln_cb = L.cb1; a.b2 = L.b2; a.F = F;
     a.x_native_in = p.x_native && i > (p.x0_layer0 ? 1 : 0);
-    if (p.op) { a.ctx = ctx; a.bo = L.bo; a.Wt = L.wmlp_op; }
+    if (p.op) { a.ctx = ctx; a.bo = L.bo; a.Wt = L.wmlp_op; a.ctx_native = ctx_n; }
     else { a.delta = d1; a.Wt = L.wmlp; }
     if (p.fuse_qkv && !last) {
       with_qkv(a, e->layers[i + 1]);
diff --git a/gw_whisper_amd/csrc/encoder_impl.h b/gw_whisper_amd/csrc/encoder_impl.h
--- a/gw_whisper_amd/csrc/encoder_impl.h
+++ b/gw_whisper_amd/csrc/encoder_impl.h
@@ -51,6 +51,7 @@
   GP_CONV2_FULLN = 1024,
   GP_STEM_SHORTCUT = 2048,
   GP_X_NATIVE = 4096,
+  GP_CTX_NATIVE = 8192,
 };
 inline int generic_path_mask() {
   static const int mask = (int)lab_int("GWW_GENERIC_PATH", 0);
@@ -94,6 +95,7 @@
   bool trace = false;
   bool stem_shortcut = true;
   bool x_native = true;
+  bool ctx_native = true;
   std::vector<TraceSpan> spans;
   std::vector<hipEvent_t> pool;
   int split = 0;
diff --git a/gw_whisper_amd/csrc/launchers.h b/gw_whisper_amd/csrc/launchers.h
--- a/gw_whisper_amd/csrc/launchers.h
+++ b/gw_whisper_amd/csrc/launchers.h
@@ -35,7 +35,7 @@
                     hipStream_t s);
 
 int launch_attention_bf16(const void* qkv, void* ctx, int B, int T, int H, hipStream_t s, float* lse = nullptr,
-                          bool last_tile_only = false, bool q_log2 = false);
+                          bool last_tile_only = false, bool q_log2 = false, bool ctx_native = false);
 int launch_attention_w64_bf16(const void* qkv, void* ctx, int B, int T, int H, hipStream_t s, float* lse);
 bool attention_log2q_enabled();
 int launch_attention_f32(const float* qkv, float* ctx, int B, int T, int H, hipStream_t s);
@@ -47,6 +47,7 @@
                     hipStream_t s, const void* wo = nullptr);
 bool mlp_fused_supported(int d, int F);
 bool mlp_fused_x_native_supported();
+bool mlp_fused_ctx_native_supported(bool x0);
 struct MfX0 {
   const float *xs, *tr, *pos;
   const int* flag;
@@ -74,6 +75,7 @@
   int T = 0;
   bool x_native_in = false;
   bool x_native_out = false;
+  bool ctx_native = false;
   const MfX0* x0 = nullptr;
   long M = 0;
   int d = 0, F = 0;
diff --git a/gw_whisper_amd/csrc/mlp_fused.hip b/gw_whisper_amd/csrc/mlp_fused.hip
--- a/gw_whisper_amd/csrc/mlp_fused.hip
+++ b/gw_whisper_amd/csrc/mlp_fused.hip
@@ -67,6 +67,14 @@
 #endif
 #ifndef GWW_MF_XN_STNT
 #define GWW_MF_XN_STNT 1
+#endif
+#ifndef GWW_MF_CN_LDNT
+#define GWW_MF_CN_LDNT 1
+#endif
+#if GWW_MF_CN_LDNT
+#define MF_CN_LDNT " nt"
+#else
+#define MF_CN_LDNT ""
 #endif
 #if GWW_MF_XN_LDNT
 #define MF_XN_LDNT " nt"
@@ -192,10 +200,12 @@
   constexpr bool QKV = MODE == 1 || MODE == 2, LNQ = MODE == 2, FIN = MODE == 3;
   static_assert(!X0 || (GWW_MF_NORM && GWW_MF_XACC && (MODE == 2 || (MODE == 1 && OP))), "X0: layer 0's two launches; stages in the u table");
   constexpr bool XACC = GWW_MF_XACC && GWW_MF_NORM && GWW_MF_SCHED && OP && (MODE == 1 || MODE == 3);
-  constexpr bool XIN = (XL & 1) != 0, XOUT = (XL & 2) != 0;
+  constexpr bool XIN = (XL & 1) != 0, XOUT = (XL & 2) != 0, CN = (XL & 4) != 0;
+  constexpr int XS = XL & 3;
   constexpr bool CSP = GWW_MF_CSPREAD && XACC;
   constexpr bool XPR = CSP && !X0 && !(GWW_MF_ABL & 32);
-  static_assert(XL == 0 || (XACC && !GWW_MF_XLDS && !X0 && (!XOUT || MODE == 1) && XL <= 3), "XL: the accumulator-order stream of XACC");
+  static_assert(XS == 0 || (XACC && !GWW_MF_XLDS && !X0 && (!XOUT || MODE == 1)), "XL: the accumulator-order stream of XACC");
+  static_assert(XL >= 0 && XL <= 7 && (!CN || XACC), "XL bit 2: the ctx requests of XACC in operand order");
   constexpr int MF_NST = MF_AHEAD + 1;
   float* lds_cb = reinterpret_cast<float*>(lds + MF_OFF_CB);
   float* lds_u = reinterpret_cast<float*>(lds + MF_OFF_U);
@@ -324,6 +334,7 @@
   const unsigned xoff = (unsigned)xrow_l * (unsigned)(MF_D * 4) + 16u * (unsigned)hh;
   const unsigned xoff_n = (unsigned)(xrow_l >> 5) * (unsigned)(32 * MF_D * 4) + 16u * (((unsigned)xrow_l & 31u) + 32u * (unsigned)hh);
   const unsigned coff = (unsigned)xrow_l * (unsigned)(MF_D * 2) + 64u * (unsigned)hh;
+  const unsigned coff_n = (unsigned)(xrow_l >> 5) * (unsigned)(32 * MF_D * 2) + 16u * (((unsigned)xrow_l & 31u) + 32u * (unsigned)hh);
   f32x4 xp[XACC ? MF_OT : 1][4];
   bool x0 = false;
   int x0_seg0 = 0;
@@ -384,6 +395,9 @@
     for (int S = 0; S < (CSP ? 1 : MF_KT); ++S)
 #pragma unroll
       for (int j = 0; j < 4; ++j)
+        if constexpr (CN)
+          asm volatile("global_load_dwordx4 %0, %1, %2 offset:%3" MF_CN_LDNT : "=v"(af[4 * S + j]) : "v"(coff_n), "s"(reinterpret_cast<const char*>(delta) + 4096 * S), "n"(1024 * j) : "memory");
+        else
         asm volatile("global_load_dwordx4 %0, %1, %2 offset:%3" : "=v"(af[4 * S + j]) : "v"(coff), "s"(delta), "n"((64 * S + 8 * j) * 2) : "memory");
     if constexpr (XPR) {
 #pragma unroll
@@ -940,7 +954,7 @@
           } else if constexpr (NAT) {
             asm volatile("global_store_dwordx4 %0, %1, %2 offset:%3" MF_XN_STNT "\n\ts_nop 1" : : "v"(xst_n), "v"(v), "s"(reinterpret_cast<char*>(dst) + 4096 * t), "n"(1024 * cc) : "memory");
           } else {
-            f32x4* const sp = reinterpret_cast<f32x4*>(reinterpret_cast<char*>(dst) + (XL != 0 && MODE == 1 ? xst_n : xoff) + (32 * t + 8 * cc) * 4);
+            f32x4* const sp = reinterpret_cast<f32x4*>(reinterpret_cast<char*>(dst) + (XS != 0 && MODE == 1 ? xst_n : xoff) + (32 * t + 8 * cc) * 4);
             if (GWW_MF_XSTNT) __builtin_nontemporal_store(v, sp);
             else *sp = v;
           }
@@ -1028,6 +1042,10 @@
           if constexpr (CSP) {
             const int rm = (itile + 2) % 3, rS = (itile + 5) / 3;
             const int cp = itile == 0 ? 4 + sub : itile > 12 ? -1 : sub == 1 ? 4 * rS + rm : sub == 2 && rm == 2 ? 4 * rS + 3 : -1;
+            if constexpr (CN) {
+              if (cp >= 0)
+                asm volatile("global_load_dwordx4 %0, %1, %2 offset:%3" MF_CN_LDNT : "=v"(af[cp >= 0 ? cp : 0]) : "v"(coff_n), "s"(reinterpret_cast<const char*>(delta) + 4096 * (cp >= 0 ? cp / 4 : 0)), "n"(1024 * (cp >= 0 ? cp % 4 : 0)) : "memory");
+            } else
             if (cp >= 0)
               asm volatile("global_load_dwordx4 %0, %1, %2 offset:%3" : "=v"(af[cp >= 0 ? cp : 0]) : "v"(coff), "s"(delta), "n"((64 * (cp / 4) + 8 * (cp % 4)) * 2) : "memory");
           }
@@ -1047,7 +1065,7 @@
                  : "+a"(oacc[0]), "+a"(oacc[1]), "+a"(oacc[2]), "+a"(oacc[3]), "+a"(oacc[4]), "+a"(oacc[5]), "+a"(oacc[6]),
                    "+a"(oacc[7]), "+a"(oacc[8]), "+a"(oacc[9]), "+a"(oacc[10]), "+a"(oacc[11]));
     if constexpr (XACC) {
-      if constexpr (XL != 0 && MODE == 1) {
+      if constexpr (XS != 0 && MODE == 1) {
         unsigned lo = lane_off;
         asm volatile("" : "+v"(lo));
         const long g = m_base + (long)((lo >> 4) & 31u);
@@ -1663,6 +1681,11 @@
 bool mlp_fused_supported(int d, int F) { return d == MF_D && F > 0 && F % 128 == 0 && F <= MF_FMAX; }
 constexpr bool MF_XL_BUILT = GWW_MF_XACC && GWW_MF_NORM && GWW_MF_SCHED && !GWW_MF_XLDS;
 bool mlp_fused_x_native_supported() { return MF_XL_BUILT; }
+#ifndef GWW_MF_CN_X0
+#define GWW_MF_CN_X0 1
+#endif
+constexpr bool MF_CN_X0_BUILT = MF_XL_BUILT && GWW_MF_CN_X0;
+bool mlp_fused_ctx_native_supported(bool x0) { return x0 ? MF_CN_X0_BUILT : MF_XL_BUILT; }
 
 int launch_mlp_fused(const MlpFusedArgs& a, hipStream_t s) {
   const char* who = a.who;
@@ -1676,6 +1699,9 @@
   GWW_REQUIRE(!xl || (MF_XL_BUILT && op && !a.keep_x_new && !x0 && (!a.x_native_out || (qkv && !a.x_next))),
               "%s: the accumulator-order residual stream runs between ctx blocks that keep no x_new, in place", who);
   GWW_REQUIRE(!xl || (long)x_native_bytes(a.M) < (1L << 32), "%s: M = %ld rows exceed the 32-bit offsets of the accumulator-order stream", who, a.M);
+  GWW_REQUIRE(!a.ctx_native || (MF_XL_BUILT && op && (qkv || fin) && (!x0 || MF_CN_X0_BUILT)),
+              "%s: ctx in operand order is read by the ctx blocks with a q / k / v tail or the final LayerNorm", who);
+  GWW_REQUIRE(!a.ctx_native || (long)ctx_native_bytes(a.M) < (1L << 32), "%s: M = %ld rows exceed the 32-bit offsets of ctx in operand order", who, a.M);
   GWW_REQUIRE(!lnq || (!a.x_new && !a.ln_u && !a.ln_cb && !a.b2 && !a.C && a.F == 0), "%s: LayerNorm 1 + q / k / v alone takes no block operand", who);
   GWW_REQUIRE(fin || qkv || (!lnq && a.C), "%s: no output", who);
   GWW_REQUIRE(!x0 || (!a.x_new && !a.keep_x_new && (lnq || (op && qkv))), "%s: x0 runs LN1 + q / k / v alone or ctx + block + q / k / v, without x_new", who);
@@ -1710,6 +1736,20 @@
                        fin ? (a.last_token ? a.T : 0) : qkv ? a.NQ : 0, x_next, a.bo, a.keep_x_new ? 1 : 0, z);
   };
   if constexpr (MF_XL_BUILT) {
+    if (a.ctx_native) {
+      const int mode = fin ? 3 : 1;
+      if (x0) {
+        if constexpr (MF_CN_X0_BUILT) launch(k_mlp_fused<1, true, true, 4>, *a.x0);
+      }
+      else if (mode == 1 && xl == 0) launch(k_mlp_fused<1, true, false, 4>, MfNoX0{});
+      else if (mode == 1 && xl == 2) launch(k_mlp_fused<1, true, false, 6>, MfNoX0{});
+      else if (mode == 1 && xl == 3) launch(k_mlp_fused<1, true, false, 7>, MfNoX0{});
+      else if (mode == 3 && xl == 0) launch(k_mlp_fused<3, true, false, 4>, MfNoX0{});
+      else if (mode == 3 && xl == 1) launch(k_mlp_fused<3, true, false, 5>, MfNoX0{});
+      else return fail(GWW_ERR_ARG, "%s: no such instantiation of k_mlp_fused", who);
+      GWW_LAUNCH_CHECK();
+      return GWW_OK;
+    }
     if (xl) {
       const int mode = fin ? 3 : 1;
       if (mode == 1 && !x0 && xl == 2) launch(k_mlp_fused<1, true, false, 2>, MfNoX0{});
@@ -1773,23 +1813,34 @@
   a.qkv_u = qkv_u; a.qkv_cb = qkv_cb; a.qkv_out = qkv_out; a.NQ = NQ;
 }
 
+extern "C" int gww_attn_out_mlp_fused_ctxn_bf16(float* x, const void* ctx, const float* bo, float* x_out, const float* ln_u,
+                                                const float* ln_cb, const void* Wt, const float* b2, void* C, long M, int d,
+                                                int F, const float* qkv_u, const float* qkv_cb, void* qkv_out, int NQ,
+                                                int ctx_native, void* stream) {
+  GWW_REQUIRE(ctx && bo, "gww_attn_out_mlp_fused_bf16: NULL ctx or out_proj bias");
+  MlpFusedArgs a = mf_block_args("gww_attn_out_mlp_fused_bf16", x, x_out, ln_u, ln_cb, Wt, b2, M, d, F);
+  a.ctx = ctx; a.bo = bo; a.C = C; a.ctx_native = ctx_native != 0;
+  mf_qkv_args(a, qkv_u, qkv_cb, qkv_out, NQ);
+  return launch_mlp_fused(a, (hipStream_t)stream);
+}
 extern "C" int gww_attn_out_mlp_fused_bf16(float* x, const void* ctx, const float* bo, float* x_out, const float* ln_u,
                                            const float* ln_cb, const void* Wt, const float* b2, void* C, long M, int d,
                                            int F, const float* qkv_u, const float* qkv_cb, void* qkv_out, int NQ,
                                            void* stream) {
-  GWW_REQUIRE(ctx && bo, "gww_attn_out_mlp_fused_bf16: NULL ctx or out_proj bias");
-  MlpFusedArgs a = mf_block_args("gww_attn_out_mlp_fused_bf16", x, x_out, ln_u, ln_cb, Wt, b2, M, d, F);
-  a.ctx = ctx; a.bo = bo; a.C = C;
-  mf_qkv_args(a, qkv_u, qkv_cb, qkv_out, NQ);
+  return gww_attn_out_mlp_fused_ctxn_bf16(x, ctx, bo, x_out, ln_u, ln_cb, Wt, b2, C, M, d, F, qkv_u, qkv_cb, qkv_out, NQ, 0, stream);
+}
+
+extern "C" int gww_attn_out_mlp_final_ctxn_bf16(const float* x, const void* ctx, const float* bo, float* x_mid, const float* ln_u,
+                                               const float* ln_cb, const void* Wt, const float* b2, const float* lnf_w,
+                                               const float* lnf_b, float* y, long M, int d, int F, int ctx_native, void* stream) {
+  MlpFusedArgs a = mf_block_args("gww_attn_out_mlp_final_bf16", x, x_mid, ln_u, ln_cb, Wt, b2, M, d, F);
+  a.ctx = ctx; a.bo = bo; a.lnf_w = lnf_w; a.lnf_b = lnf_b; a.y = y; a.ctx_native = ctx_native != 0;
   return launch_mlp_fused(a, (hipStream_t)stream);
 }
-
 extern "C" int gww_attn_out_mlp_final_bf16(const float* x, const void* ctx, const float* bo, float* x_mid, const float* ln_u,
                                           const float* ln_cb, const void* Wt, const float* b2, const float* lnf_w,
                                           const float* lnf_b, float* y, long M, int d, int F, void* stream) {
-  MlpFusedArgs a = mf_block_args("gww_attn_out_mlp_final_bf16", x, x_mid, ln_u, ln_cb, Wt, b2, M, d, F);
-  a.ctx = ctx; a.bo = bo; a.lnf_w = lnf_w; a.lnf_b = lnf_b; a.y = y;
-  return launch_mlp_fused(a, (hipStream_t)stream);
+  return gww_attn_out_mlp_final_ctxn_bf16(x, ctx, bo, x_mid, ln_u, ln_cb, Wt, b2, lnf_w, lnf_b, y, M, d, F, 0, stream);
 }
 
 extern "C" int gww_lnqkv_fused_bf16(const float* x, const float* qkv_u, const float* qkv_cb, const void* Wt, void* qkv_out,
@@ -1821,14 +1872,22 @@
   return launch_mlp_fused(a, (hipStream_t)stream);
 }
 
+extern "C" int gww_attn_out_mlp_fused_x0_ctxn_bf16(const float* xs, const float* tr, const float* pos, const int* flag, float* x,
+                                                   int T, int Tt, const void* ctx, const float* bo, const float* ln_u,
+                                                   const float* ln_cb, const void* Wt, const float* b2, long M, int d, int F,
+                                                   const float* qkv_u, const float* qkv_cb, void* qkv_out, int NQ,
+                                                   int ctx_native, void* stream) {
+  GWW_REQUIRE(ctx, "gww_attn_out_mlp_fused_x0_bf16: NULL operand");
+  const MfX0 z{xs, tr, pos, flag, T, Tt};
+  MlpFusedArgs a = mf_block_args("gww_attn_out_mlp_fused_x0_bf16", x, nullptr, ln_u, ln_cb, Wt, b2, M, d, F);
+  a.ctx = ctx; a.bo = bo; a.x0 = &z; a.ctx_native = ctx_native != 0;
+  mf_qkv_args(a, qkv_u, qkv_cb, qkv_out, NQ);
+  return launch_mlp_fused(a, (hipStream_t)stream);
+}
 extern "C" int gww_attn_out_mlp_fused_x0_bf16(const float* xs, const float* tr, const float* pos, const int* flag, float* x, int T,
                                               int Tt, const void* ctx, const float* bo, const float* ln_u, const float* ln_cb,
                                               const void* Wt, const float* b2, long M, int d, int F, const float* qkv_u,
                                               const float* qkv_cb, void* qkv_out, int NQ, void* stream) {
-  GWW_REQUIRE(ctx, "gww_attn_out_mlp_fused_x0_bf16: NULL operand");
-  const MfX0 z{xs, tr, pos, flag, T, Tt};
-  MlpFusedArgs a = mf_block_args("gww_attn_out_mlp_fused_x0_bf16", x, nullptr, ln_u, ln_cb, Wt, b2, M, d, F);
-  a.ctx = ctx; a.bo = bo; a.x0 = &z;
-  mf_qkv_args(a, qkv_u, qkv_cb, qkv_out, NQ);
-  return launch_mlp_fused(a, (hipStream_t)stream);
-}
+  return gww_attn_out_mlp_fused_x0_ctxn_bf16(xs, tr, pos, flag, x, T, Tt, ctx, bo, ln_u, ln_cb, Wt, b2, M, d, F, qkv_u, qkv_cb,
+                                             qkv_out, NQ, 0, stream);
+}
diff --git a/gw_whisper_amd/encoder.py b/gw_whisper_amd/encoder.py
--- a/gw_whisper_amd/encoder.py
+++ b/gw_whisper_amd/encoder.py
@@ -406,6 +406,9 @@
     def set_x_native(self, on: bool = True):
         check(lib().gww_encoder_set_x_native(self._ensure_handle(), int(on)), "gww_encoder_set_x_native")
 
+    def set_ctx_native(self, on: bool = True):
+        check(lib().gww_encoder_set_ctx_native(self._ensure_handle(), int(on)), "gww_encoder_set_ctx_native")
+
     def stem_shortcut_flags(self, batch: int) -> tuple:
         if self._ws is None:
             raise _lib.GwwError("stem_shortcut_flags: no forward has run yet")
diff --git a/gw_whisper_amd/ops.py b/gw_whisper_amd/ops.py
--- a/gw_whisper_amd/ops.py
+++ b/gw_whisper_amd/ops.py
@@ -208,9 +208,16 @@
     return out
 
 
-def attn_out_mlp_fused(x, ctx, wo, bo, w1_folded, w2, ln_u, ln_cb, b2, qkv=None):
+def _ctx_operand(ctx, M: int, ctx_native: bool):
+    ctx = _dev(ctx, torch.bfloat16, "ctx")
+    if ctx_native and ctx.numel() * 2 < lib().gww_ctx_native_bytes(M):
+        raise _lib.GwwError(f"ctx in operand order must hold {lib().gww_ctx_native_bytes(M)} bytes for M = {M}")
+    return ctx
+
+
+def attn_out_mlp_fused(x, ctx, wo, bo, w1_folded, w2, ln_u, ln_cb, b2, qkv=None, ctx_native=False):
     x = _dev(x, torch.float32, "x")
-    ctx = _dev(ctx, torch.bfloat16, "ctx")
+    ctx = _ctx_operand(ctx, x.shape[0], ctx_native)
     wo = _dev(wo, torch.bfloat16, "Wo")
     w1 = _dev(w1_folded, torch.bfloat16, "W1")
     w2 = _dev(w2, torch.bfloat16, "W2")
@@ -234,19 +241,19 @@
         else:
             qu, qc = f(qkv[1]), f(qkv[2])
             out = torch.empty((Mp, NQ), dtype=torch.bfloat16, device=x.device)
-        check(lib().gww_attn_out_mlp_fused_bf16(x.data_ptr(), ctx.data_ptr(), bo.data_ptr(), x_out.data_ptr(), u.data_ptr(),
-                                                cb.data_ptr(), wt.data_ptr(), b2.data_ptr(),
-                                                out.data_ptr() if qkv is None else None, M, d, F,
-                                                qu.data_ptr() if qu is not None else None,
-                                                qc.data_ptr() if qc is not None else None,
-                                                out.data_ptr() if qkv is not None else None, NQ, _stream()),
-              "gww_attn_out_mlp_fused_bf16")
+        check(lib().gww_attn_out_mlp_fused_ctxn_bf16(x.data_ptr(), ctx.data_ptr(), bo.data_ptr(), x_out.data_ptr(), u.data_ptr(),
+                                                     cb.data_ptr(), wt.data_ptr(), b2.data_ptr(),
+                                                     out.data_ptr() if qkv is None else None, M, d, F,
+                                                     qu.data_ptr() if qu is not None else None,
+                                                     qc.data_ptr() if qc is not None else None,
+                                                     out.data_ptr() if qkv is not None else None, NQ, int(bool(ctx_native)),
+                                                     _stream()), "gww_attn_out_mlp_fused_bf16")
     return out[:M], (x_out if qkv is None else x)
 
 
-def attn_out_mlp_final(x, ctx, wo, bo, w1_folded, w2, ln_u, ln_cb, b2, lnf_w, lnf_b):
+def attn_out_mlp_final(x, ctx, wo, bo, w1_folded, w2, ln_u, ln_cb, b2, lnf_w, lnf_b, ctx_native=False):
     x = _dev(x, torch.float32, "x")
-    ctx = _dev(ctx, torch.bfloat16, "ctx")
+    ctx = _ctx_operand(ctx, x.shape[0], ctx_native)
     wo, w1, w2 = _dev(wo, torch.bfloat16, "Wo"), _dev(w1_folded, torch.bfloat16, "W1"), _dev(w2, torch.bfloat16, "W2")
     F, d = w1.shape
     M = x.shape[0]
@@ -257,9 +264,10 @@
     with torch.cuda.device(x.device):
         check(lib().gww_mlp_pack_op_bf16(wo.data_ptr(), w1.data_ptr(), w2.data_ptr(), None, wt.data_ptr(), d, F, 0, _stream()),
               "gww_mlp_pack_op_bf16")
-        check(lib().gww_attn_out_mlp_final_bf16(x.data_ptr(), ctx.data_ptr(), bo.data_ptr(), x_mid.data_ptr(), u.data_ptr(),
-                                                cb.data_ptr(), wt.data_ptr(), b2.data_ptr(), lw.data_ptr(), lb.data_ptr(),
-                                                y.data_ptr(), M, d, F, _stream()), "gww_attn_out_mlp_final_bf16")
+        check(lib().gww_attn_out_mlp_final_ctxn_bf16(x.data_ptr(), ctx.data_ptr(), bo.data_ptr(), x_mid.data_ptr(), u.data_ptr(),
+                                                     cb.data_ptr(), wt.data_ptr(), b2.data_ptr(), lw.data_ptr(), lb.data_ptr(),
+                                                     y.data_ptr(), M, d, F, int(bool(ctx_native)), _stream()),
+              "gww_attn_out_mlp_final_bf16")
     return y, x_mid
 
 
@@ -314,10 +322,10 @@
     return qo[:M]
 
 
-def attn_out_mlp_fused_x0(xs, tr, pos, flag, ctx, wo, bo, w1_folded, w2, ln_u, ln_cb, b2, qkv, x=None):
+def attn_out_mlp_fused_x0(xs, tr, pos, flag, ctx, wo, bo, w1_folded, w2, ln_u, ln_cb, b2, qkv, x=None, ctx_native=False):
     xs, tr, pos, flag, x, B, T, Tt, d = _x0_operands(xs, tr, pos, flag, x)
     x = x.clone().view(B * T, d)
-    ctx = _dev(ctx, torch.bfloat16, "ctx")
+    ctx = _ctx_operand(ctx, B * T, ctx_native)
     wo, w1, w2 = _dev(wo, torch.bfloat16, "Wo"), _dev(w1_folded, torch.bfloat16, "W1"), _dev(w2, torch.bfloat16, "W2")
     wq = _dev(qkv[0], torch.bfloat16, "Wqkv")
     F, NQ, M = w1.shape[0], wq.shape[0], B * T
@@ -328,10 +336,10 @@
     with torch.cuda.device(x.device):
         check(lib().gww_mlp_pack_op_bf16(wo.data_ptr(), w1.data_ptr(), w2.data_ptr(), wq.data_ptr(), wt.data_ptr(), d, F, NQ,
                                          _stream()), "gww_mlp_pack_op_bf16")
-        check(lib().gww_attn_out_mlp_fused_x0_bf16(xs.data_ptr(), tr.data_ptr(), pos.data_ptr(), flag.data_ptr(), x.data_ptr(), T, Tt,
-                                                   ctx.data_ptr(), bo.data_ptr(), u.data_ptr(), cb.data_ptr(), wt.data_ptr(),
-                                                   b2.data_ptr(), M, d, F, qu.data_ptr(), qc.data_ptr(), out.data_ptr(), NQ,
-                                                   _stream()), "gww_attn_out_mlp_fused_x0_bf16")
+        check(lib().gww_attn_out_mlp_fused_x0_ctxn_bf16(xs.data_ptr(), tr.data_ptr(), pos.data_ptr(), flag.data_ptr(), x.data_ptr(), T,
+                                                        Tt, ctx.data_ptr(), bo.data_ptr(), u.data_ptr(), cb.data_ptr(), wt.data_ptr(),
+                                                        b2.data_ptr(), M, d, F, qu.data_ptr(), qc.data_ptr(), out.data_ptr(), NQ,
+                                                        int(bool(ctx_native)), _stream()), "gww_attn_out_mlp_fused_x0_bf16")
     return out[:M], x
 
 
@@ -380,16 +388,19 @@
     return ctx
 
 
-def attention_log2q(qkv: torch.Tensor, n_heads: int, want_lse: bool = False):
+def attention_log2q(qkv: torch.Tensor, n_heads: int, want_lse: bool = False, ctx_native: bool = False):
     qkv = _dev(qkv, torch.bfloat16, "qkv")
     B, T, d3 = qkv.shape
     if d3 != 3 * n_heads * 64:
         raise _lib.GwwError(f"attention: d={d3 // 3} != n_heads*64")
-    ctx = torch.empty((B, T, d3 // 3), dtype=torch.bfloat16, device=qkv.device)
+    if ctx_native:
+        ctx = torch.empty(((B * T + 31) // 32 * 32, d3 // 3), dtype=torch.bfloat16, device=qkv.device)
+    else:
+        ctx = torch.empty((B, T, d3 // 3), dtype=torch.bfloat16, device=qkv.device)
     lse = torch.empty((B, n_heads, T), dtype=torch.float32, device=qkv.device) if want_lse else None
     with torch.cuda.device(qkv.device):
-        check(lib().gww_attention_log2q_bf16(qkv.data_ptr(), ctx.data_ptr(), lse.data_ptr() if want_lse else None, B, T,
-                                             n_heads, _stream()), "gww_attention_log2q_bf16")
+        check(lib().gww_attention_log2q_ctxn_bf16(qkv.data_ptr(), ctx.data_ptr(), lse.data_ptr() if want_lse else None, B, T,
+                                                  n_heads, int(bool(ctx_native)), _stream()), "gww_attention_log2q_bf16")
     return (ctx, lse) if want_lse else ctx
 
 
diff --git a/include/gww.h b/include/gww.h
--- a/include/gww.h
+++ b/include/gww.h
@@ -83,6 +83,22 @@
 int gww_encoder_set_x_native(gww_encoder* enc, int on);
 size_t gww_x_native_offset(long row, int col, long M);
 size_t gww_x_native_bytes(long M);
+
+int gww_encoder_set_ctx_native(gww_encoder* enc, int on);
+size_t gww_ctx_native_offset(long row, int col, long M);
+size_t gww_ctx_native_bytes(long M);
+int gww_attention_log2q_ctxn_bf16(const void* qkv, void* ctx, float* lse_or_null, int B, int T, int n_heads, int ctx_native,
+                                  void* stream);
+int gww_attn_out_mlp_fused_ctxn_bf16(float* x, const void* ctx, const float* bo, float* x_out, const float* ln_u,
+                                     const float* ln_cb, const void* Wt, const float* b2, void* C, long M, int d, int F,
+                                     const float* qkv_u, const float* qkv_cb, void* qkv_out, int NQ, int ctx_native, void* stream);
+int gww_attn_out_mlp_final_ctxn_bf16(const float* x, const void* ctx, const float* bo, float* x_mid, const float* ln_u,
+                                     const float* ln_cb, const void* Wt, const float* b2, const float* lnf_w, const float* lnf_b,
+                                     float* y, long M, int d, int F, int ctx_native, void* stream);
+int gww_attn_out_mlp_fused_x0_ctxn_bf16(const float* xs, const float* tr, const float* pos, const int* flag, float* x, int T, int Tt,
+                                        const void* ctx, const float* bo, const float* ln_u, const float* ln_cb, const void* Wt,
+                                        const float* b2, long M, int d, int F, const float* qkv_u, const float* qkv_cb,
+                                        void* qkv_out, int NQ, int ctx_native, void* stream);
 
 int gww_encoder_trace_enable(gww_encoder* enc, int on);
 int gww_encoder_trace_read(gww_encoder* enc, float* ms, int* counts);
```
